# SymbolicML/DynamicExpressions.jl

Hardware: AMD Instinct MI355X
Metric: node-evals/sec (higher is better)
Workload: dtype f32

## Files before the change

dynamicexpressions.jl_amd/api.py:

```python
from __future__ import annotations

import ctypes as C
import os
from dataclasses import dataclass
from typing import Optional, Sequence, Tuple, Union

import numpy as np

from .node import Node, TAPE_DTYPE, count_constant_nodes, flatten_graph, flatten_population, max_feature, preserve_sharing
from .operators import OperatorEnum

_HERE = os.path.dirname(os.path.abspath(__file__))
LIB_PATH = os.environ.get("DE_HIP_LIB") or os.path.join(_HERE, "csrc", "libde_hip.so")

DE_F32, DE_F64, DE_F16, DE_CF32, DE_CF64 = 0, 1, 2, 3, 4
COMPLEX_DTYPES = (np.dtype(np.complex64), np.dtype(np.complex128))
GRAD_VARIABLE, GRAD_CONSTANT, GRAD_BOTH = 0, 1, 2
ABI_VERSION = 3
OPT_EARLY_EXIT, OPT_FUSE_DEG1, OPT_FUSE_DEG2, OPT_BUMPER_CHECKS, OPT_TURBO, OPT_FULL_EVAL, OPT_FORWARD_GRAD, OPT_REVERSE_GRAD = 1, 2, 4, 8, 16, 32, 64, 128

EXPORTS = [
    "de_abi_version", "de_opcode_table_version", "de_opcode_by_name", "de_opcode_name",
    "de_opcode_degree", "de_status_string", "de_ctx_create", "de_ctx_destroy", "de_ctx_set_stream",
    "de_ctx_synchronize", "de_ctx_declare_dataset", "de_ctx_stream", "de_last_error", "de_program_create", "de_program_create_cse",
    "de_program_set_consts", "de_program_update", "de_program_destroy", "de_program_n_trees", "de_program_n_nodes",
    "de_program_n_grad", "de_program_dump", "de_program_verify", "de_program_stream_hash", "de_host_pool_selftest", "de_lower_tape", "de_lower_tape_stage", "de_lower_tape_complex", "de_lower_tape_stage_complex", "de_lower_tape_grad", "de_eval", "de_eval_grad", "de_eval_diff", "de_eval_loss", "de_eval_loss_grad", "de_eval_loss_grad_by_class",
    "de_loss_spec_check", "de_eval_loss_ex", "de_eval_fit_stats", "de_eval_loss_gn", "de_gn_max_rows", "de_eval_loss_grad_ex", "de_eval_loss_grad_by_class_ex",
    "de_eval_pullback_dX", "de_eval_tree_array", "de_eval_plan", "de_prio_tiles_wanted", "de_program_last_live_trees", "de_dist_unique_id", "de_dist_init", "de_dist_destroy", "de_dist_shard_size", "de_dist_world_size",
    "de_dist_broadcast", "de_dist_gather_flags", "de_dist_last_error", "de_ctx_last_kernel_ms", "de_ctx_last_kernel_name",
    "de_ctx_device", "de_ctx_timing_ring", "de_ctx_timing_read", "de_dist_reorder_selftest", "de_eval_sum_certificate",
    "de_dist_set_timeout", "de_ctx_trim", "de_program_set_consts_device", "de_program_get_consts", "de_program_consts_device_path",
]


class DeviceError(RuntimeError):
    """The HIP library/GPU is unavailable or a de_* call failed.  Never swallowed."""


class UncertifiedFlag(DeviceError):
    """EvalContext(strict_flags=True): the device's element-wise validity flag of this tree is not PROVABLY the reference's
    `isfinite(sum(x))` flag (a finite array whose sum may overflow): the caller keeps the CPU path for it."""


class ParamArgs(C.Structure):
    _fields_ = [("params", C.c_void_p), ("ld_params", C.c_int64), ("n_classes", C.c_int64),
                ("classes", C.c_void_p), ("classes_is_i64", C.c_int32), ("class_base", C.c_int32)]


class LossSpec(C.Structure):
    _fields_ = [("kind", C.c_int32), ("reserved", C.c_int32), ("param", C.c_double)]


LOSS_KINDS = {"L2": 0, "L1": 1, "pullback": 2, "huber": 16, "logcosh": 17, "l1_eps": 18, "l2_eps": 19, "quantile": 20, "lp": 21,
              "logit_dist": 22, "logit_margin": 23, "l1_hinge": 24}


def loss_spec(loss: str, loss_param: float = 0.0, with_gradient: bool = True) -> LossSpec:
    if loss == "pullback" and not with_gradient:
        raise KeyError(loss)
    spec = LossSpec(LOSS_KINDS[loss], 0, float(loss_param))
    if library().de_loss_spec_check(C.byref(spec), int(with_gradient)) != 0:
        raise ValueError(f"loss {loss!r}: parameter {loss_param!r} is not finite or outside the kind's range (include/de_hip.h de_loss_kind_t)")
    return spec


class FitStats:

    def __init__(self, mean_p, m2_p, cov, W, mean_y, m2_y):
        self.mean_p, self.m2_p, self.cov = (np.array(v, dtype=np.float64) for v in (mean_p, m2_p, cov))
        if self.mean_p.ndim != 1 or self.m2_p.shape != self.mean_p.shape or self.cov.shape != self.mean_p.shape:
            raise ValueError("mean_p, m2_p and cov are one-dimensional arrays of one length (one entry per tree)")
        self.W, self.mean_y, self.m2_y = float(W), float(mean_y), float(m2_y)

    def __len__(self) -> int:
        return self.mean_p.shape[0]

    def _flat(self):
        return self.m2_p == 0.0

    @property
    def pearson_r(self):
        with np.errstate(divide="ignore", invalid="ignore"):
            r = self.cov / np.sqrt(self.m2_p * self.m2_y)
        return np.where(self._flat(), np.nan, r)
# ... 114 lines not shown
            pass
        lib = C.CDLL(LIB_PATH)
    except OSError as e:
        raise DeviceError(f"cannot load {LIB_PATH}: {e}") from e
    vp, i32, i64, u32 = C.c_void_p, C.c_int32, C.c_int64, C.c_uint32
    lib.de_abi_version.restype = C.c_int
    if lib.de_abi_version() != ABI_VERSION:
        raise DeviceError(f"{LIB_PATH} has ABI version {lib.de_abi_version()}, this module was written for {ABI_VERSION}: rebuild (csrc/build.sh)")
    lib.de_opcode_table_version.restype = C.c_int
    lib.de_opcode_by_name.argtypes = [C.c_char_p, C.c_int]
    lib.de_opcode_name.restype = C.c_char_p
    lib.de_opcode_name.argtypes = [C.c_int]
    lib.de_opcode_degree.argtypes = [C.c_int]
    lib.de_status_string.restype = C.c_char_p
    lib.de_status_string.argtypes = [C.c_int]
    lib.de_ctx_create.argtypes = [C.c_int, vp, C.POINTER(vp)]
    lib.de_ctx_destroy.argtypes = [vp]
    lib.de_ctx_set_stream.argtypes = [vp, vp]
    lib.de_ctx_synchronize.argtypes = [vp]
    lib.de_ctx_declare_dataset.argtypes = [vp, C.c_int, vp, i64, i64, i32]
    lib.de_ctx_stream.restype = vp
    lib.de_ctx_stream.argtypes = [vp]
    lib.de_last_error.restype = C.c_char_p
    lib.de_last_error.argtypes = [vp]
    lib.de_program_create.argtypes = [vp, C.c_int, vp, vp, i64, vp, vp, i32, i32, u32, C.POINTER(vp)]
    lib.de_program_create_cse.argtypes = [vp, C.c_int, vp, vp, vp, vp, i64, vp, vp, i32, i32, u32, C.POINTER(vp)]
    lib.de_program_set_consts.argtypes = [vp, vp]
    lib.de_program_set_consts_device.argtypes = [vp, vp]
    lib.de_program_get_consts.argtypes = [vp, vp]
    lib.de_program_consts_device_path.argtypes = [vp]
    lib.de_program_update.argtypes = [vp, vp, i64, vp, vp, vp, vp, vp, vp]
    lib.de_program_destroy.argtypes = [vp]
    lib.de_program_n_trees.restype = i64
    lib.de_program_n_trees.argtypes = [vp]
    lib.de_program_n_nodes.restype = i64
    lib.de_program_n_nodes.argtypes = [vp]
    lib.de_program_n_grad.restype = i64
    lib.de_program_n_grad.argtypes = [vp, i64, C.c_int]
    lib.de_program_verify.argtypes = [vp]
    lib.de_host_pool_selftest.restype = C.c_int64
    lib.de_host_pool_selftest.argtypes = [C.c_int64, C.POINTER(C.c_int32)]
    lib.de_program_stream_hash.restype = C.c_uint64
    lib.de_program_stream_hash.argtypes = [vp]
    lib.de_program_dump.restype = i64
    lib.de_program_dump.argtypes = [vp, i64, vp, i64, C.c_int]
    lib.de_lower_tape.restype = i64
    lib.de_lower_tape.argtypes = [C.c_int, vp, i64, vp, i64, i32, i32, u32, vp, i64, vp]
    lib.de_lower_tape_stage.restype = i64
    lib.de_lower_tape_stage.argtypes = [C.c_int, vp, i64, vp, i64, i32, i32, u32, C.c_int, vp, i64]
    for fn in (lib.de_lower_tape_complex, lib.de_lower_tape_stage_complex):
        fn.restype = i64
    lib.de_lower_tape_complex.argtypes = lib.de_lower_tape.argtypes
    lib.de_lower_tape_stage_complex.argtypes = lib.de_lower_tape_stage.argtypes
    lib.de_lower_tape_grad.restype = i64
    lib.de_lower_tape_grad.argtypes = [C.c_int, vp, i64, vp, i64, i32, i32, u32, C.c_int, C.c_int, vp, i64, vp]
    lib.de_eval.argtypes = [vp, vp, vp, i64, i64, C.POINTER(ParamArgs), vp, i64, vp]
    lib.de_eval_loss.argtypes = [vp, vp, vp, i64, i64, C.POINTER(ParamArgs), vp, vp, C.c_int32, vp, vp]
    lib.de_eval_loss_grad.argtypes = [vp, vp, vp, i64, i64, C.POINTER(ParamArgs), C.c_int, vp, vp, C.c_int32, vp, vp, vp, vp]
    lib.de_eval_loss_grad_by_class.argtypes = [vp, vp, vp, i64, i64, C.POINTER(ParamArgs), C.c_int, vp, vp, C.c_int32, vp, vp, vp, vp, vp, vp]
    lib.de_loss_spec_check.argtypes = [C.POINTER(LossSpec), C.c_int]
    lib.de_eval_loss_ex.argtypes = [vp, vp, vp, i64, i64, C.POINTER(ParamArgs), vp, vp, C.POINTER(LossSpec), vp, vp]
    lib.de_eval_fit_stats.argtypes = [vp, vp, vp, i64, i64, C.POINTER(ParamArgs), vp, vp, vp, vp, vp]
    lib.de_eval_loss_gn.argtypes = [vp, vp, vp, i64, i64, C.POINTER(ParamArgs), C.c_int, vp, vp, vp, vp, vp, vp, vp, vp]
    lib.de_gn_max_rows.argtypes = []
    lib.de_eval_loss_grad_ex.argtypes = [vp, vp, vp, i64, i64, C.POINTER(ParamArgs), C.c_int, vp, vp, C.POINTER(LossSpec), vp, vp, vp, vp]
    lib.de_eval_loss_grad_by_class_ex.argtypes = [vp, vp, vp, i64, i64, C.POINTER(ParamArgs), C.c_int, vp, vp, C.POINTER(LossSpec), vp, vp, vp, vp, vp, vp]
    lib.de_eval_grad.argtypes = [vp, vp, vp, i64, i64, C.POINTER(ParamArgs), C.c_int, vp, i64, vp, vp, vp]
    lib.de_eval_diff.argtypes = [vp, vp, vp, i64, i64, i32, vp, vp, i64, vp]
    lib.de_eval_pullback_dX.argtypes = [vp, vp, vp, i64, i64, C.POINTER(ParamArgs), vp, vp, vp, vp]
    lib.de_eval_tree_array.argtypes = [vp, C.c_int, vp, i64, vp, i64, vp, i32, i64, u32, vp, vp]
    lib.de_eval_plan.argtypes = [vp, i64, vp]
    lib.de_prio_tiles_wanted.argtypes = [i64, i32, i64]
    lib.de_program_last_live_trees.argtypes = [vp, C.POINTER(i64)]
    lib.de_dist_unique_id.argtypes = [vp]
    lib.de_dist_init.argtypes = [vp, C.c_int, C.c_int, vp, C.POINTER(vp)]
    lib.de_dist_destroy.argtypes = [vp]
    lib.de_dist_set_timeout.argtypes = [vp, i64]
    lib.de_dist_world_size.argtypes = [vp]
    lib.de_dist_shard_size.restype = i64
    lib.de_dist_shard_size.argtypes = [i64, C.c_int, C.c_int]
    lib.de_dist_broadcast.argtypes = [vp, vp, C.c_size_t, C.c_int]
    lib.de_dist_gather_flags.argtypes = [vp, vp, i64, vp]
    lib.de_dist_last_error.restype = C.c_char_p
    lib.de_dist_last_error.argtypes = [vp]
    lib.de_ctx_last_kernel_ms.argtypes = [vp, C.POINTER(C.c_float)]
    lib.de_ctx_last_kernel_name.restype = C.c_char_p
    lib.de_ctx_last_kernel_name.argtypes = [vp]
    lib.de_ctx_device.argtypes = [vp]
    lib.de_ctx_timing_ring.argtypes = [vp, i32]
    lib.de_ctx_timing_read.argtypes = [vp, vp, i32, C.POINTER(i32)]
    lib.de_dist_reorder_selftest.argtypes = [vp, vp, i64, C.c_int, vp, C.POINTER(C.c_float)]
    lib.de_eval_sum_certificate.argtypes = [vp, vp, vp, i64, i64, C.POINTER(ParamArgs), vp, vp, vp]
    _lib = lib
    return lib


def _dtype_code(dtype) -> int:
    dtype = np.dtype(dtype)
    if dtype == np.float32:
        return DE_F32
    if dtype == np.float64:
        return DE_F64
    if dtype == np.float16:
        return DE_F16
    if dtype == np.complex64:
        return DE_CF32
# ... 148 lines not shown
            X = X.to(tdt)
        F, N = X.shape
        if not (X.stride(0) == 1 and (N <= 1 or X.stride(1) >= F)) and X.numel() > 0:
            X = X.t().contiguous().t()
        ld = X.stride(1) if N > 1 else max(F, 1)
        return X.data_ptr(), F, N, ld, X, True
    X = np.asarray(X)
    if X.ndim == 1:
        X = X.reshape(-1, 1)
    Xf = np.asfortranarray(X, dtype=dtype)
    F, N = Xf.shape
    return Xf.ctypes.data, F, N, max(F, 1), Xf, False


def lower_tape(tape, consts, n_features: int, n_params: int = 0, options: int = 7, dtype=np.float32):
    lib = library()
    dtype = np.dtype(dtype)
    tape = np.ascontiguousarray(tape)
    consts = np.ascontiguousarray(consts, dtype=dtype)
    meta = np.zeros(4, dtype=np.int32)
    cp = consts.ctypes.data if consts.size else None
    lower = lib.de_lower_tape_complex if dtype in COMPLEX_DTYPES else lib.de_lower_tape
    n = lower(_dtype_code(dtype), tape.ctypes.data, len(tape), cp, consts.size, n_features,
              n_params, options, None, 0, meta.ctypes.data)
    if n < 0:
        code = int(-n)
        name = lib.de_status_string(code).decode()
        if code == 3:
            from .operators import UnsupportedOperatorError
            raise UnsupportedOperatorError(name)
        raise ValueError(name)
    w = np.zeros(max(int(n), 1), dtype=np.uint32)
    lower(_dtype_code(dtype), tape.ctypes.data, len(tape), cp, consts.size, n_features,
          n_params, options, w.ctypes.data, w.size, meta.ctypes.data)
    return w[:int(n)].reshape(-1, 4), dict(n_slots=int(meta[0]), host_ok_eval=bool(meta[1]),
                                           host_ok_grad=bool(meta[2]), uses_params=bool(meta[3]))


def lower_tape_stage(tape, consts, n_features: int, stage: int, n_params: int = 0, options: int = 7,
                     dtype=np.float32) -> np.ndarray:
    lib = library()
    dtype = np.dtype(dtype)
    tape = np.ascontiguousarray(tape)
    consts = np.ascontiguousarray(consts, dtype=dtype)
    cp = consts.ctypes.data if consts.size else None
    args = (_dtype_code(dtype), tape.ctypes.data, len(tape), cp, consts.size, n_features, n_params, options, stage)
    stage_fn = lib.de_lower_tape_stage_complex if dtype in COMPLEX_DTYPES else lib.de_lower_tape_stage
    n = stage_fn(*args, None, 0)
    if n < 0:
        raise ValueError(lib.de_status_string(int(-n)).decode())
    w = np.zeros(max(int(n), 1), dtype=np.uint32)
    stage_fn(*args, w.ctypes.data, w.size)
    return w[:int(n)].reshape(-1, 4)


def lower_tape_grad(tape, consts, n_features: int, mode: int, form: int, n_params: int = 0, options: int = 7, dtype=np.float32):
    lib = library()
    dtype = np.dtype(dtype)
    tape = np.ascontiguousarray(tape)
    consts = np.ascontiguousarray(consts, dtype=dtype)
    cp = consts.ctypes.data if consts.size else None
    meta = np.zeros(8, dtype=np.int32)
    args = (_dtype_code(dtype), tape.ctypes.data, len(tape), cp, consts.size, n_features, n_params, options, mode, form)
    n = lib.de_lower_tape_grad(*args, None, 0, meta.ctypes.data)
    if n < 0:
        raise ValueError(lib.de_status_string(int(-n)).decode())
    w = np.zeros(max(int(n), 1), dtype=np.uint32)
    lib.de_lower_tape_grad(*args, w.ctypes.data, w.size, meta.ctypes.data)
    return w[:int(n)].reshape(-1, 4), meta


def check_update_ids(indices, n_new: int, n_trees: int) -> np.ndarray:
    ids = np.asarray(list(indices) if not isinstance(indices, np.ndarray) else indices)
    if ids.ndim != 1:
        raise ValueError("update: indices must be one-dimensional")
    if len(ids) != n_new:
        raise ValueError(f"update: {len(ids)} indices for {n_new} trees")
    if len(ids) == 0:
        return np.zeros(0, dtype=np.int64)
    if ids.dtype.kind not in "iu":
        raise ValueError(f"update: indices must be integers, got {ids.dtype}")
    ids = np.ascontiguousarray(ids, dtype=np.int64)
    if ids.min() < 0 or ids.max() >= n_trees:
        raise ValueError(f"update: tree index outside [0, {n_trees})")
    if len(np.unique(ids)) != len(ids):
        raise ValueError("update: a tree index appears twice")
    return ids


class Population:

    def __init__(self, trees: Sequence[Node], operators: OperatorEnum, dtype=np.float32,
                 n_features: Optional[int] = None, n_params: int = 0,
                 eval_context: Optional[EvalContext] = None, ctx: Optional[Context] = None):
        self.ctx = ctx or default_context()
        self.dtype = np.dtype(dtype)
        self.operators = operators
        self.eval_context = eval_context or EvalContext()
        self.n_trees = len(trees)
        nodes, noff, consts, coff = flatten_population(trees, operators, self.dtype)
        if n_features is None:
            n_features = max((max_feature(t) for t in trees), default=0)
        self.n_features, self.n_params = int(n_features), int(n_params)
        self.n_consts = np.diff(coff).astype(np.int64)
        self._classes_checked = set()
        self._h = C.c_void_p()
# ... 131 lines not shown
        return library().de_program_consts_device_path(self._h) == 1

    def verify(self) -> None:
        self.ctx.check(library().de_program_verify(self._h))

    def stream_hash(self) -> int:
        return int(library().de_program_stream_hash(self._h))

    def _combine_rows(self, t: int, g, mode: int):
        if self._occ is None or self._occ[t] is None or mode == GRAD_VARIABLE:
            return g
        o = self._occ[t]
        lead = g.shape[0] - len(o)
        nu = int(o.max()) + 1
        if _is_torch(g):
            import torch
            out = torch.zeros((lead + nu,) + tuple(g.shape[1:]), dtype=g.dtype, device=g.device)
            out[:lead] = g[:lead]
            out.index_add_(0, torch.as_tensor(o + lead, device=g.device), g[lead:])
            return out
        out = np.zeros((lead + nu,) + g.shape[1:], dtype=g.dtype)
        out[:lead] = g[:lead]
        np.add.at(out, o + lead, g[lead:])
        return out

    def plan(self, N: int) -> dict:
        pl = np.zeros(3, dtype=np.int32)
        self.ctx.check(library().de_eval_plan(self._h, N, pl.ctypes.data))
        return dict(tile=int(pl[0]), n_chunks=int(pl[1]), trees_per_chunk=int(pl[2]))

    def last_live_trees(self) -> int:
        n = C.c_int64(-1)
        self.ctx.check(library().de_program_last_live_trees(self._h, C.byref(n)))
        return int(n.value)

    def n_grad(self, tree: int, mode: int) -> int:
        return int(library().de_program_n_grad(self._h, tree, mode))

    def _n_grad_all(self, mode: int) -> np.ndarray:
        cache = self.__dict__.setdefault("_ng_cache", {})
        if mode not in cache:
            lib = library()
            cache[mode] = np.array([lib.de_program_n_grad(self._h, t, mode) for t in range(self.n_trees)], dtype=np.int64)
        return cache[mode]

    def dump(self, tree: int) -> np.ndarray:
        lib = library()
        n = lib.de_program_dump(self._h, tree, None, 0, 0)
        w = np.zeros(max(int(n), 1), dtype=np.uint32)
        got = lib.de_program_dump(self._h, tree, w.ctypes.data, w.size, 0)
        return w[:int(got)].reshape(-1, 4)

    def meta(self, tree: int) -> dict:
        w = np.zeros(5, dtype=np.uint32)
        library().de_program_dump(self._h, tree, w.ctypes.data, 5, 1)
        return dict(n_slots=int(w[0]), host_ok_eval=bool(w[1]), host_ok_grad=bool(w[2]), uses_params=bool(w[3]), waves=int(w[4]))

    def _param_args(self, params, classes, class_base, N, keep):
        if self.n_params == 0 and params is None:
            return None
        if params is None or classes is None:
            raise ValueError("Incorrect call. You must pass the `classes::Vector` argument when calling `eval_tree_array`.")
        pa = ParamArgs()
        if _is_torch(params):
            import torch
            params = params.to(_torch_dtype(self.dtype))
            if params.stride(0) != 1 and params.numel() > 0:
                params = params.t().contiguous().t()
            P, ncls = params.shape
            pa.params, pa.ld_params = params.data_ptr(), (params.stride(1) if ncls > 1 else max(P, 1))
        else:
            params = np.asfortranarray(params, dtype=self.dtype)
            P, ncls = params.shape
            pa.params, pa.ld_params = params.ctypes.data, max(P, 1)
        if P != self.n_params:
            raise ValueError("parameter matrix has the wrong number of rows")
        if _is_torch(classes):
            import torch
            if classes.dtype not in (torch.int32, torch.int64):
                classes = classes.to(torch.int64)
            classes = classes.contiguous()
            n_c = classes.numel()
            key = (classes.data_ptr(), n_c, classes._version, ncls, class_base)
            if n_c and key not in self._classes_checked:
                mn, mx = int(classes.min().item()), int(classes.max().item())
                if mn < class_base or mx - class_base >= ncls:
                    raise ValueError(f"class ids must lie in [{class_base}, {class_base + ncls}): got [{mn}, {mx}] "
                                     "(maximum(classes) <= size(parameters, 2))")
                if len(self._classes_checked) > 64:
                    self._classes_checked.clear()
                self._classes_checked.add(key)
            pa.classes, pa.classes_is_i64 = classes.data_ptr(), int(classes.dtype == torch.int64)
        else:
            classes = np.ascontiguousarray(classes)
            if classes.dtype not in (np.int32, np.int64):
                classes = classes.astype(np.int64)
            n_c = classes.size
            if n_c:
                mn, mx = int(classes.min()), int(classes.max())
                if mn < class_base or mx - class_base >= ncls:
                    raise ValueError(f"class ids must lie in [{class_base}, {class_base + ncls}): got [{mn}, {mx}] "
                                     "(maximum(classes) <= size(parameters, 2))")
            pa.classes, pa.classes_is_i64 = classes.ctypes.data, int(classes.dtype == np.int64)
        if n_c != N:
            raise ValueError(f"length(classes) == size(X, 2) violated: {n_c} class ids for {N} samples")
        pa.n_classes, pa.class_base = ncls, class_base
        keep.extend([params, classes])
        return pa

# ... 580 lines not shown
```

dynamicexpressions.jl_amd/csrc/de_api_eval.cpp:

```cpp
#include "de_api_internal.h"

extern "C" {
int stage_in(de_ctx *c, DevBuf &buf, const void *user, size_t bytes, Staged *s) {
    s->dev = const_cast<void *>(user);
    s->staged = false;
    if (!user || bytes == 0 || is_device_ptr(user)) return DE_OK;
    HIP_TRY(c, buf.reserve(bytes));
    HIP_TRY(c, hipMemcpyAsync(buf.p, user, bytes, hipMemcpyHostToDevice, c->stream));
    s->dev = buf.p;
    s->staged = true;
    return DE_OK;
}
int stage_out(de_ctx *c, DevBuf &buf, void *user, size_t bytes, Staged *s) {
    s->dev = user;
    s->staged = false;
    if (!user || bytes == 0 || is_device_ptr(user)) return DE_OK;
    HIP_TRY(c, buf.reserve(bytes));
    s->dev = buf.p;
    s->staged = true;
    return DE_OK;
}

int check_param_args(de_ctx *c, const de_program *p, const de_param_args_t *pa, int64_t N) {
    if (!p->uses_params) return DE_OK;
// ... 236 lines not shown
    if (ok_dev) {
        sOk.dev = ok;
    } else {
        HIP_TRY(c, c->sOk.reserve((size_t)p->n_trees));
        sOk.dev = c->sOk.p;
        sOk.staged = true;
    }
    if (!p->d_ok_eval) HIP_TRY(c, hipMemcpyAsync(sOk.dev, p->host_ok_eval.data(), (size_t)p->n_trees, hipMemcpyHostToDevice, c->stream));
    if (p->uses_params) {
        rc = stage_in(c, c->sParams, pa->params, (size_t)pa->ld_params * (size_t)pa->n_classes * es, &sPar);
        if (rc) return rc;
        rc = stage_in(c, c->sClasses, pa->classes, (size_t)N * (pa->classes_is_i64 ? 8 : 4), &sCls);
        if (rc) return rc;
    }
    EvalArgs a;
    std::memset(&a, 0, sizeof a);
    a.code = p->d_code;
    a.code_off = p->d_code_off;
    a.n_trees = (int32_t)p->n_trees;
    a.n_slots = p->n_slots + (p->prows ? p->n_params : 0);
    a.prow_base = p->prows ? p->n_features + p->n_slots : 0;
    a.n_prows = p->prows ? p->n_params : 0;
    a.uses_params = p->uses_params;
    a.X = sX.dev;
    a.N = N;
    a.ldX = ldX;
    a.F = p->n_features;
    a.out = sOut.dev;
    a.ld_out = ld_out;
    a.ok = static_cast<uint8_t *>(sOk.dev);
    a.ok_init = p->d_ok_eval;
    if (p->uses_params) {
        a.params = sPar.dev;
        a.ld_params = pa->ld_params;
        a.n_classes = pa->n_classes;
        a.classes = sCls.dev;
        a.classes_is_i64 = pa->classes_is_i64;
        a.class_base = pa->class_base;
    }
    a.early_exit = (p->options & DE_OPT_EARLY_EXIT) != 0;
    a.skip_flagged = a.early_exit && !(p->options & DE_OPT_FULL_EVAL) && tree_skip_enabled();
    a.turbo = (p->options & DE_OPT_TURBO) != 0;
    a.threaded = p->threaded && !direct;
    a.direct = direct;
    a.loss = lr ? &la : nullptr;
    HIP_TRY(c, c->sPrio.reserve((size_t)3 * DE_PRIO_MAX_F * sizeof(unsigned long long)));
    a.prio_keys = c->sPrio.p;
    a.prio_keys_ready = !half && !cplx && !sX.staged && dataset_keys(c, p->dtype, X, N, ldX, p->n_features, &a.prio_keys);
    a.compact_code = p->d_compact_code;
    a.compact_ints = p->d_compact_ints;
    a.waves = p->waves;
    a.wave_slots = p->n_slots;
    a.var_stride = p->var_stride;
    if (cr) {
        a.code = p->d_cert_code;
        a.code_off = p->d_cert_off;
        a.threaded = false;
        a.cert_max = c->sCert.p;
        a.out = nullptr;
        a.prio_keys = nullptr;
        a.compact_code = nullptr;
        a.compact_ints = nullptr;
    }
    HIP_TRY(c, time_begin(c));
    a.compacted = &p->last_compacted;
    p->last_compacted = false;
    if (half || cplx) {
        a.threaded = false;
        a.prio_keys = nullptr;
        a.compact_code = nullptr;
        a.compact_ints = nullptr;
    }
    if (half) HIP_TRY(c, launch_eval_f16(a, c->stream, &c->last_kernel));
    else if (cplx) HIP_TRY(c, launch_eval_complex(p->io, a, p->d_ctab, c->stream, &c->last_kernel));
    else HIP_TRY(c, launch_eval(p->dtype, a, c->stream, &c->last_kernel));
    HIP_TRY(c, time_end(c));
    if (sLoss.staged) HIP_TRY(c, hipMemcpyAsync(lr->loss, sLoss.dev, (size_t)p->n_trees * es, hipMemcpyDeviceToHost, c->stream));
    if (sStats.staged) HIP_TRY(c, hipMemcpyAsync(lr->stats, sStats.dev, (size_t)p->n_trees * 3 * sizeof(double), hipMemcpyDeviceToHost, c->stream));
    if (sYstats.staged) HIP_TRY(c, hipMemcpyAsync(lr->ystats, sYstats.dev, 3 * sizeof(double), hipMemcpyDeviceToHost, c->stream));
    if (sOut.staged) {
        if (ld_out == N)
            HIP_TRY(c, hipMemcpyAsync(out, sOut.dev, (size_t)p->n_trees * (size_t)N * es, hipMemcpyDeviceToHost, c->stream));
        else
            for (int64_t t = 0; t < p->n_trees; t++)
                HIP_TRY(c, hipMemcpyAsync(static_cast<char *>(out) + (size_t)t * (size_t)ld_out * es,
                                          static_cast<char *>(sOut.dev) + (size_t)t * (size_t)ld_out * es,
                                          (size_t)N * es, hipMemcpyDeviceToHost, c->stream));
    }
    if (sOk.staged) HIP_TRY(c, hipMemcpyAsync(ok, sOk.dev, (size_t)p->n_trees, hipMemcpyDeviceToHost, c->stream));
    if (cr) {
        std::vector<unsigned char> mx((size_t)p->n_trees * ces);
        std::vector<uint8_t> okh((size_t)p->n_trees);
        HIP_TRY(c, hipMemcpyAsync(mx.data(), c->sCert.p, mx.size(), hipMemcpyDeviceToHost, c->stream));
        HIP_TRY(c, hipMemcpyAsync(okh.data(), sOk.dev, okh.size(), hipMemcpyDeviceToHost, c->stream));
        HIP_TRY(c, hipStreamSynchronize(c->stream));
        const double top = half ? 65504.0 : p->dtype == DE_F32 ? (double)std::numeric_limits<float>::max() : std::numeric_limits<double>::max();
        double margin = 1.001;
        if (half) {
            const double d = 1024.0 + std::ceil(std::log2(std::max(1.0, (double)N / 1024.0))) + 8.0;
            margin = std::exp(d * std::log1p(std::ldexp(1.0, -11)));
        }
        for (int64_t t = 0; t < p->n_trees; t++) {
            double m = p->dtype == DE_F32 ? (double)reinterpret_cast<float *>(mx.data())[t] : reinterpret_cast<double *>(mx.data())[t];
            m = std::max(m, p->cert_cmax[(size_t)t]);
            if (cr->max_abs) cr->max_abs[t] = m;
            cr->certified[t] = (!okh[(size_t)t] || m * (double)N * margin < top || !(m == m)) ? 1 : 0;
// ... 41 lines not shown
```

dynamicexpressions.jl_amd/csrc/de_api_internal.h:

```cpp
#ifndef DE_API_INTERNAL_H
#define DE_API_INTERNAL_H
#include <hip/hip_runtime.h>
#include <pthread.h>

#include <chrono>
#include <cmath>
#include <cstdarg>
#include <cstdio>
#include <cstring>
#include <condition_variable>
#include <functional>
#include <map>
#include <mutex>
#include <memory>
#include <new>
#include <string>
#include <algorithm>
#include <array>
#include <atomic>
#include <thread>
#include <vector>

#include "../../include/de_hip.h"
#include "de_kernels.h"
// ... 46 lines not shown
    DevBuf sPrioDs;
};

struct de_program {
    de_ctx *ctx = nullptr;
    int dtype = DE_F32;
    int io = DE_F32;
    std::vector<double> consts_im, ctab;
    void *d_ctab = nullptr;
    uint32_t options = 0;
    int32_t n_features = 0, n_params = 0;
    int64_t n_trees = 0, n_nodes = 0;
    int n_slots = 0;
    bool prows = false;
    bool uses_params = false;
    std::vector<Instr> code;
    std::vector<int32_t> code_off;
    std::vector<int64_t> const_off;
    std::vector<int32_t> const_instr;
    std::vector<uint8_t> const_checks;
    std::vector<int32_t> n_consts_tree;
    bool cse_generic = false;
    std::vector<uint8_t> host_ok_eval;
    std::vector<uint8_t> host_ok_grad;
    std::vector<double> consts;
    bool folded = false;
    std::vector<Instr> fcode;
    std::vector<int32_t> fcode_off;
    std::vector<int32_t> fconst_instr;
    struct Fold { int32_t tree, instr; bool tested_always; };
    std::vector<Fold> folds;
    std::vector<int64_t> aux_const_src;
    de_program *aux = nullptr;
    std::vector<uint8_t> fold_ok;
    std::vector<uint8_t> fold_host;
    std::vector<int32_t> kfold;
    std::vector<int64_t> kf_csrc;
    char *d_kf = nullptr;
    size_t kf_o_noff = 0, kf_o_coff = 0, kf_o_cvals = 0, kf_o_out = 0, kf_o_ok = 0, kf_bytes = 0;
    std::vector<de_tape_node_t> fold_nodes;
    std::vector<int64_t> fold_noff, fold_coff;
    std::vector<int32_t> aux_fold;
    std::vector<int64_t> aux_csrc;
    std::vector<BoundInstr> bcode;
    std::vector<BoundInstr> tcode;
    std::vector<BoundInstr> fbcode;
    std::vector<int32_t> tcode_off;
    std::vector<BoundInstr> ccode;
    std::vector<int32_t> ccode_off;
    int waves = 1;
    int waves_choice = 0;
    int64_t var_stride = 0;
    std::vector<BoundInstr> ccode_w;
    uint64_t end_handler = 0;
    uint64_t endv_handler[TOPX_ENDV_COUNT] = {0};
    bool threaded = false;
    bool direct = false;
    uint64_t handler_base = 0;
    std::vector<int32_t> bcode_off;
    BoundInstr *d_code = nullptr;
    int32_t *d_code_off = nullptr;
    bool eval_arena = false;
    BoundInstr *d_compact_code = nullptr;
    int32_t *d_compact_ints = nullptr;
    bool last_compacted = false;
    BoundInstr *d_cert_code = nullptr;
    int32_t *d_cert_off = nullptr;
    size_t cert_cap = 0;
    uint64_t consts_gen = 0;
    uint64_t cert_gen = ~0ull;
    std::vector<double> cert_cmax;
    BoundInstr *d_gcode = nullptr;
    int32_t *d_gcode_off = nullptr;
    std::vector<BoundInstr> gbcode;
    std::vector<int32_t> gbcode_off;
    bool gcode_stale = true;
    std::vector<BoundInstr> gtcode;
    std::vector<int32_t> gtcode_off;
    BoundInstr *d_gtcode = nullptr;
    int32_t *d_gtcode_off = nullptr;
    int32_t *d_gt_ids = nullptr;
    uint8_t *d_ok_eval = nullptr;
    uint8_t *d_ok_grad = nullptr;
    int32_t *d_ng = nullptr;
    int64_t *d_goff = nullptr;
    int tab_mode = -1;
    int64_t tab_N = -1;
    bool tab_ok_stale = true;
    std::vector<int32_t> bsite, tsite, gbsite, gtsite_of_gb;
    struct EvalSite { int32_t src, b, t, c; };
    struct GradSite { int32_t src, gb, gt, rt; };
    std::vector<EvalSite> eval_sites;
    std::vector<GradSite> grad_sites;
    uint64_t site_gen = 1, lists_gen = 0;
    std::vector<BoundInstr> rtcode;
    std::vector<int32_t> rtcode_off, rtcode_mid, rtsite_of_gb;
    BoundInstr *d_rtcode = nullptr;
    int32_t *d_rtcode_off = nullptr, *d_rtcode_mid = nullptr, *d_rt_ids = nullptr;
    int rt_mode = -1, rt_stage_cols = 0, rt_n_groups = 0;
    GradArgs::RevGroup rt_groups[8];
    bool rt_valid = false;
    uint64_t rt_handler_base = 0;
    uint32_t rt_param_off = 0;
    int gt_mode = -1;
    bool gt_valid = false, gt_wide = false;
    bool gt_share = false;
// ... 125 lines not shown
```

dynamicexpressions.jl_amd/csrc/de_api_program.cpp:

```cpp
#include "de_api_internal.h"
#include "de_const_patch.h"

template <typename T>
static bool host_fold_eval(const de_tape_node_t *nd, int64_t n, const double *consts, const int64_t *csrc, T *value, bool half = false) {
    T stack_small[32];
    std::vector<T> stack_big;
    T *st = stack_small;
    if (n > 32) { stack_big.resize((size_t)n); st = stack_big.data(); }
    int sp = 0;
    bool ok = true;
    for (int64_t i = 0; i < n; i++) {
        T v;
        if (nd[i].degree == 0) v = (T)consts[csrc[nd[i].arg]];
        else {
            const T b = st[--sp], a = st[--sp];
            switch (nd[i].op) {
            case DE_B_ADD: v = a + b; break;
            case DE_B_SUB: v = a - b; break;
            case DE_B_MUL: v = a * b; break;
            default: v = a / b; break;
            }
            if (half) v = (T)(_Float16)v;
        }
        ok = ok && std::isfinite(v);
// ... 70 lines not shown
};
static int64_t eval_rows(const de_program *p) { return (int64_t)p->n_features + p->n_slots + (p->prows ? p->n_params : 0); }
static bool same_binding(const de_program *p, const de_program *old) {
    return old->folded == p->folded && old->prows == p->prows && old->n_slots == p->n_slots && old->n_features == p->n_features &&
           old->n_params == p->n_params && old->options == p->options && old->dtype == p->dtype;
}
static void rebind(de_program *p, const Reuse *ru = nullptr) {
    const bool ee = (p->options & DE_OPT_EARLY_EXIT) != 0;
    p->prows = p->uses_params && p->n_params > 0 && p->n_params <= 16 && param_rows_enabled() &&
               ((size_t)p->n_features + (size_t)p->n_slots + (size_t)p->n_params) * 257 * 16 <= 150 * 1024;
    const int prb = p->prows ? p->n_features + p->n_slots : -1;
    const std::vector<Instr> &src = p->folded ? p->fcode : p->code;
    const std::vector<int32_t> &off = p->folded ? p->fcode_off : p->code_off;
    const int nf = p->n_features;
    const de_program *old = ru && ru->old && same_binding(p, ru->old) ? ru->old : nullptr;
    build_stream_by_trees<BoundInstr>(p->n_trees, &p->bcode, &p->bcode_off, [&](int64_t t, std::vector<BoundInstr> *out) {
        if (old && ru->src[(size_t)t] >= 0) {
            const size_t s = (size_t)ru->src[(size_t)t];
            out->insert(out->end(), old->bcode.begin() + old->bcode_off[s], old->bcode.begin() + old->bcode_off[s + 1]);
            return;
        }
        const int32_t i0 = off[(size_t)t], i1 = off[(size_t)t + 1];
        bind_tree(src.data() + i0, (size_t)(i1 - i0), ee, nf, out, prb);
    });
    match_const_sites(src, off, p->bcode, p->bcode_off, p->n_trees, [](const BoundInstr &b) { return bop_is_const_source(b.bop); }, &p->bsite);
    p->tsite.clear();
    p->site_gen++;
}

static void make_chained(de_program *p);
static int choose_waves(const de_program *p) {
    if (TBLK != 64 || (p->uses_params && !p->prows)) return 1;
    if (const char *e = getenv("DE_EVAL_WAVES")) { const int v = atoi(e); return (v == 2 || v == 4 || v == 8) ? v : 1; }
    const size_t rb = trow_bytes(p->dtype), lds_cu = 160u << 10, shared = (size_t)p->n_features + (p->prows ? (size_t)p->n_params : 0);
    auto resident = [&](int W) -> size_t {
        const size_t lds = (shared + (size_t)W * (size_t)p->n_slots) * rb + (size_t)W * 256;
        const size_t by_regs = W >= 4 ? 7 / ((size_t)W / 4) : 28 / (size_t)W;
        return lds > 150u * 1024 ? 0 : std::min<size_t>(lds_cu / lds, by_regs) * (size_t)W;
    };
    int best = 1;
    size_t have = resident(1);
    for (int W : {2, 4, 8}) {
        const size_t w = resident(W);
        if (have >= 20) break;
        if (w * 2 < have * 3) {
            if (W == 2 && have < 12) continue;
            break;
        }
        best = W;
        have = w;
    }
    return best;
}
static int make_threaded(de_ctx *c, de_program *p, const Reuse *ru = nullptr) {
    p->threaded = false;
    p->waves = 1;
    p->var_stride = 0;
    p->ccode_w.clear();
    dbg_lap(nullptr);
    p->direct = (size_t)eval_rows(p) * FLAT_ROW_BYTES > 150 * 1024;
    if (p->io == DE_F16) return DE_OK;
    if (is_complex_io(p->io)) {
        p->direct = (size_t)eval_rows(p) * complex_row_bytes(p->io) > 64 * 1024;
        return DE_OK;
    }
    if ((p->direct && ((size_t)eval_rows(p) + 3 * (size_t)p->n_slots) * trow_bytes(p->dtype) + 4 * 256 > 150 * 1024) || !eval_uses_threaded()) return DE_OK;
    if (eval_rows(p) > 4000) return DE_OK;
    uint64_t table[TOPX_TABLE];
    hipError_t st = eval_handler_table(p->dtype, (p->options & DE_OPT_TURBO) != 0, table);
    if (st != hipSuccess) return fail(c, DE_ERR_HIP, "handler table: %s", hipGetErrorString(st));
    dbg_lap("handler table");
    uint64_t base = table[0];
    for (int i = 0; i < (int)TOPX_TABLE; i++) base = std::min<uint64_t>(base, table[i]);
    for (int i = 0; i < (int)TOPX_TABLE; i++) {
        if (table[i] - base > 0xFFFFFFFFull) return DE_OK;
        if (p->dtype != DE_F32 && (table[i] >> 32) != (table[0] >> 32)) return DE_OK;
    }
    const bool hot_unary = !getenv("DE_NO_CONST_UNARY_HOT");
    const uint32_t row_bytes = (uint32_t)trow_bytes(p->dtype);
    const char *nf = getenv("DE_NO_FUSE");
    const bool fuse = !(nf && *nf == '1');
    if (p->waves_choice == 0) p->waves_choice = choose_waves(p);
    const int W = fuse ? p->waves_choice : 1;
    const int wave_prows = p->prows ? p->n_params : 0;
    const FuseRows rows0{(uint32_t)p->n_features, (uint32_t)(p->n_features + p->n_slots), 0, W > 1 ? wave_prows + (W - 1) * p->n_slots : 0};
    const de_program *old = ru && ru->old && ru->old->threaded && ru->old->waves_choice == p->waves_choice && same_binding(p, ru->old) ? ru->old : nullptr;
    build_stream_by_trees<BoundInstr>(p->n_trees, &p->fbcode, &p->tcode_off, [&](int64_t t, std::vector<BoundInstr> *out) {
        if (old && ru->src[(size_t)t] >= 0) {
            const size_t s = (size_t)ru->src[(size_t)t];
            out->insert(out->end(), old->fbcode.begin() + old->tcode_off[s], old->fbcode.begin() + old->tcode_off[s + 1]);
            return;
        }
        const int32_t b0 = p->bcode_off[(size_t)t], b1 = p->bcode_off[(size_t)t + 1];
        if (fuse) fuse_tree(p->bcode.data() + b0, (size_t)(b1 - b0), out, W > 1 && p->n_slots > 0 ? &rows0 : nullptr);
        else out->insert(out->end(), p->bcode.begin() + b0, p->bcode.begin() + b1);
    });
    dbg_lap("fuse_tree");
    p->tcode.resize(p->fbcode.size());
    auto threaded_words = [p, &table, base, hot_unary, row_bytes](const BoundInstr &b) {
        BoundInstr t = b;
        t.bop = (uint32_t)(table[b.bop] - base);
        if (hot_unary && (b.bop == BOP_GEN_ROW || b.bop == BOP_GEN_ACC)) {
            const int k = gun_index((int)(b.arg >> 24), DE_U_COS, DE_U_EXP, DE_U_SIN, DE_U_NEG, DE_U_SQUARE, DE_U_CUBE, DE_U_ABS, DE_U_LOG, DE_U_SAFE_LOG,
                                    DE_U_SQRT, DE_U_SAFE_SQRT, DE_U_TANH, DE_U_RELU);
            if (k >= 3) t.bop = (uint32_t)(table[TOPX_UN_BASE + (uint32_t)(k - 3) * 2 + (b.bop == BOP_GEN_ACC ? 1 : 0)] - base);
        }
        if (hot_unary && (b.bop == BOP_GEN_ROW || b.bop == BOP_GEN_CONST) && ((b.arg >> 24) == (uint32_t)DE_B_MAX || (b.arg >> 24) == (uint32_t)DE_B_MIN))
            t.bop = (uint32_t)(table[TOPX_BIN_BASE + ((b.arg >> 24) == (uint32_t)DE_B_MAX ? 0u : 2u) + (b.bop == BOP_GEN_CONST ? 1u : 0u)] - base);
        if (b.bop < BOP_COUNT && bop_is_const_source(b.bop)) {
            t.arg = b.arg & 0xFF000000u;
        } else if (b.bop == BOP_GEN_PARAM) {
// ... 32 lines not shown
        const bool ee = (p->options & DE_OPT_EARLY_EXIT) != 0, f32 = p->dtype == DE_F32;
        const std::vector<Instr> &src = p->folded ? p->fcode : p->code;
        const std::vector<int32_t> &off = p->folded ? p->fcode_off : p->code_off;
        const int prb = p->prows ? p->n_features + p->n_slots : -1, n_prows = wave_prows;
        const size_t n_rec = p->ccode.size();
        p->ccode_w.resize(n_rec * (size_t)(W - 1));
        std::atomic<bool> same{true};
        const bool wold = old && old->waves == W && old->var_stride != 0 && old->ccode_w.size() == old->ccode.size() * (size_t)(W - 1);
        for (int w = 1; w < W; w++) {
            BoundInstr *cw = p->ccode_w.data() + n_rec * (size_t)(w - 1);
            const int shift = n_prows + w * p->n_slots;
            const FuseRows rows_w{(uint32_t)(p->n_features + shift), (uint32_t)(p->n_features + shift + p->n_slots), shift, rows0.headroom};
            parallel_tree_ranges(p->n_trees, [&](int, int64_t tb, int64_t te) {
                std::vector<BoundInstr> b, f;
                const size_t r0 = (size_t)p->ccode_off[(size_t)tb] - 1, r1 = te < p->n_trees ? (size_t)p->ccode_off[(size_t)te] - 1 : n_rec;
                std::copy(p->ccode.begin() + (long)r0, p->ccode.begin() + (long)r1, cw + r0);
                for (int64_t t = tb; t < te; t++) {
                    if (wold && ru->src[(size_t)t] >= 0) {
                        const size_t s = (size_t)ru->src[(size_t)t], h = (size_t)p->ccode_off[(size_t)t], ho = (size_t)old->ccode_off[s];
                        const BoundInstr *ow = old->ccode_w.data() + old->ccode.size() * (size_t)(w - 1);
                        for (int32_t i = 0; i < p->tcode_off[(size_t)t + 1] - p->tcode_off[(size_t)t]; i++) {
                            BoundInstr &r = cw[h + (size_t)i];
                            const BoundInstr &o = ow[ho + (size_t)i];
                            r.bop = o.bop;
                            if (f32) r.arg = o.arg;
                            else { r.lo = o.lo; r.hi = o.hi; }
                        }
                        continue;
                    }
                    b.clear();
                    f.clear();
                    bind_tree(src.data() + off[(size_t)t], (size_t)(off[(size_t)t + 1] - off[(size_t)t]), ee, p->n_features, &b, prb, shift);
                    fuse_tree(b.data(), b.size(), &f, &rows_w);
                    const int32_t i0 = p->tcode_off[(size_t)t], i1 = p->tcode_off[(size_t)t + 1];
                    if ((int32_t)f.size() != i1 - i0) { same = false; return; }
                    const size_t h = (size_t)p->ccode_off[(size_t)t];
                    for (int32_t i = i0; i < i1; i++) {
                        if (f[(size_t)(i - i0)].bop != p->fbcode[(size_t)i].bop) { same = false; return; }
                        const BoundInstr tw = threaded_words(f[(size_t)(i - i0)]);
                        BoundInstr &r = cw[h + (size_t)(i - i0)];
                        r.bop = tw.arg;
                        if (f32) r.arg = tw.lo;
                        else { r.lo = tw.lo; r.hi = tw.hi; }
                    }
                }
            });
        }
        if (same) {
            p->waves = W;
            p->var_stride = (int64_t)(p->bcode.size() + (size_t)p->n_trees + 2);
        } else p->ccode_w.clear();
        dbg_lap("wave-group stream variants");
    } else if (W > 1 && fuse) p->waves = W;
    return DE_OK;
}

static void make_chained(de_program *p) {
    const bool f32 = p->dtype == DE_F32;
    p->ccode.assign(p->tcode.size() + (size_t)p->n_trees + 1, BoundInstr{0u, 0u, 0u, 0u});
    p->ccode_off.assign((size_t)p->n_trees + 1, 0);
    auto put = [&](BoundInstr &r, uint32_t la, uint32_t lo, uint32_t hi) {
        r.bop = la;
        if (f32) r.arg = lo;
        else { r.lo = lo; r.hi = hi; }
    };
    auto name_next = [&](BoundInstr &r, uint64_t handler) {
        if (f32) { r.lo = (uint32_t)handler; r.hi = (uint32_t)(handler >> 32); }
        else r.arg = (uint32_t)handler;
    };
    auto ev_of = [&](int64_t t) -> int {
        const int32_t i0 = p->tcode_off[(size_t)t], i1 = p->tcode_off[(size_t)t + 1];
        return i1 - i0 >= 2 ? topx_endv_of(p->fbcode[(size_t)i1 - 1].bop) : -1;
    };
    auto handler_of = [&](int32_t i, int32_t i1, int ev) -> uint64_t {
        return (i == i1 - 1 && ev >= 0) ? p->endv_handler[ev] : p->handler_base + p->tcode[(size_t)i].bop;
    };
    parallel_tree_ranges(p->n_trees, [&](int, int64_t tb, int64_t te) {
        for (int64_t t = tb; t < te; t++) {
            const int32_t i0 = p->tcode_off[(size_t)t], i1 = p->tcode_off[(size_t)t + 1];
            const size_t h = (size_t)i0 + (size_t)t + 1;
            p->ccode_off[(size_t)t] = (int32_t)h;
            const int ev = ev_of(t);
            for (int32_t i = i0; i < i1; i++) {
                const BoundInstr &s = p->tcode[(size_t)i];
                put(p->ccode[h + (size_t)(i - i0)], s.arg, s.lo, s.hi);
                if (i > i0) name_next(p->ccode[h + (size_t)(i - i0) - 1], handler_of(i, i1, ev));
            }
            put(p->ccode[h + (size_t)(i1 - i0)], (uint32_t)t, 0u, 0u);
            if (i1 > i0) name_next(p->ccode[h + (size_t)(i1 - i0) - 1], p->end_handler);
        }
    });
    for (int64_t t = 0; t < p->n_trees; t++) {
        const int32_t i0 = p->tcode_off[(size_t)t], i1 = p->tcode_off[(size_t)t + 1];
        const size_t h = (size_t)p->ccode_off[(size_t)t];
        const int ev = ev_of(t);
        if (i1 > i0) {
            const uint64_t first = handler_of(i0, i1, ev);
            name_next(p->ccode[h - 1], first);
            if (t > 0 && ev_of(t - 1) >= 0) name_next(p->ccode[h - 2], first);
        } else name_next(p->ccode[h - 1], p->end_handler);
        put(p->ccode[h - 1], t == 0 ? 0u : (uint32_t)(t - 1), (uint32_t)(i1 - i0) | (ev >= 0 ? DE_HDR_FUSED_END : 0u), 0u);
    }
    if (p->n_trees > 0) name_next(p->ccode.back(), p->end_handler);
    p->ccode_off[(size_t)p->n_trees] = (int32_t)p->ccode.size();
}
static inline void patch_chained_imm(de_program *p, int32_t c, uint32_t lo, uint32_t hi) {
    if (p->dtype == DE_F32) p->ccode[(size_t)c].arg = lo;
    else { p->ccode[(size_t)c].lo = lo; p->ccode[(size_t)c].hi = hi; }
    for (size_t w = 0; w * p->ccode.size() < p->ccode_w.size(); w++) {
        BoundInstr &r = p->ccode_w[w * p->ccode.size() + (size_t)c];
        if (p->dtype == DE_F32) r.arg = lo;
        else { r.lo = lo; r.hi = hi; }
    }
}
static hipError_t upload_wave_variants(de_program *p) {
    for (size_t w = 0; p->var_stride && w * p->ccode.size() < p->ccode_w.size(); w++) {
        const hipError_t st = hipMemcpy(p->d_code + (w + 1) * (size_t)p->var_stride, p->ccode_w.data() + w * p->ccode.size(),
                                        p->ccode.size() * sizeof(BoundInstr), hipMemcpyHostToDevice);
        if (st != hipSuccess) return st;
    }
    return hipSuccess;
}

static void recompute_host_ok(de_program *p) {
    const bool ee = (p->options & DE_OPT_EARLY_EXIT) != 0;
    parallel_for_trees(p->n_trees, [&](int64_t t) {
        bool ok_eval = true, ok_grad = true;
        for (int64_t k = p->const_off[t]; k < p->const_off[t + 1]; k++) {
            const bool fin = finite_in(p->dtype, p->consts[k]) && (p->consts_im.empty() || finite_in(p->dtype, p->consts_im[k]));
            ok_grad = ok_grad && fin;
            const uint8_t ch = p->const_checks[k];
            if (!fin && ((ch & CONST_CHECK_ALWAYS) || (ee && (ch & CONST_CHECK_EE)))) ok_eval = false;
        }
        p->host_ok_eval[t] = ok_eval;
        p->host_ok_grad[t] = ok_grad;
    }, 1024);
    for (size_t j = 0; j < p->folds.size() && j < p->fold_ok.size(); j++)
        if (!p->fold_ok[j] && (p->folds[j].tested_always || ee)) p->host_ok_eval[(size_t)p->folds[j].tree] = 0;
}

static int create_impl(de_ctx_t *ctx, int dtype, const de_tape_node_t *nodes, const int64_t *node_offsets,
                       int64_t n_trees, const void *consts, const int64_t *const_offsets, int32_t n_features,
                       int32_t n_params, uint32_t options, bool allow_fold, de_program_t **out_program,
                       const de_tape_node_t *cse_nodes = nullptr, const int64_t *cse_offsets = nullptr, const Reuse *reuse = nullptr,
                       bool keep_input = true);

static int upload_ok_eval(de_ctx *c, de_program *p) {
    p->tab_ok_stale = true;
    if (p->n_trees == 0) return DE_OK;
    if (!p->d_ok_eval) HIP_TRY(c, hipMalloc(reinterpret_cast<void **>(&p->d_ok_eval), (size_t)std::max<int64_t>(p->n_trees, 1)));
    HIP_TRY(c, hipStreamSynchronize(c->stream));
    HIP_TRY(c, hipMemcpy(p->d_ok_eval, p->host_ok_eval.data(), (size_t)p->n_trees, hipMemcpyHostToDevice));
    return DE_OK;
}

static int refresh_folds(de_ctx *c, de_program *p, bool aux_current = false) {
    if (!p->folded || p->folds.empty()) return DE_OK;
    const size_t es = p->dtype == DE_F32 ? 4 : 8;
    const size_t ies = dtype_bytes(p->io);
    const size_t nf = p->folds.size();
    p->fold_ok.assign(nf, 0);
    parallel_for_trees((int64_t)nf, [&](int64_t j) {
        if (p->fold_host[(size_t)j] != 1) return;
        const de_tape_node_t *nd = p->fold_nodes.data() + p->fold_noff[(size_t)j];
        const int64_t n = p->fold_noff[(size_t)j + 1] - p->fold_noff[(size_t)j];
        const int64_t *csrc = p->aux_const_src.data() + p->fold_coff[(size_t)j];
// ... 562 lines not shown
                        std::vector<int32_t> oaux(o->folds.size(), -1);
                        for (size_t a = 0; a < o->aux_fold.size(); a++) oaux[(size_t)o->aux_fold[a]] = (int32_t)a;
                        aru.old = o->aux;
                        aru.src.assign(p->aux_fold.size(), -1);
                        for (size_t a = 0; a < p->aux_fold.size(); a++) {
                            const size_t j = (size_t)p->aux_fold[a];
                            const int64_t t = p->folds[j].tree;
                            if (!reuse->reuse(t)) continue;
                            const size_t s = (size_t)reuse->src[(size_t)t];
                            aru.src[a] = oaux[(size_t)(reuse->fold0[s] + ((int64_t)j - fold0[(size_t)t]))];
                        }
                        aru.fold0.assign((size_t)o->aux->n_trees + 1, 0);
                        for (const de_program::Fold &f : o->aux->folds) aru.fold0[(size_t)f.tree + 1]++;
                        for (size_t q = 0; q < (size_t)o->aux->n_trees; q++) aru.fold0[q + 1] += aru.fold0[q];
                    }
                    int rc = create_impl(ctx, io, xnodes.data(), xnoff.data(), (int64_t)p->aux_fold.size(), ac.data(),
                                         xcoff.data(), n_features, 0, options, false, &p->aux, nullptr, nullptr, aru.old ? &aru : nullptr,
                                         false);
                    if (rc != DE_OK) return rc;
                    lap("aux program (create)");
                }
                int rc = refresh_folds(ctx, p.get(), true);
                if (rc != DE_OK) return rc;
                lap("folds (evaluate: host + kernel + aux)");
            } else if (any_cse) {
                p->folded = true;
            } else {
                p->fcode.clear();
                p->fcode_off.clear();
            }
        }
        if (!allow_fold) parallel_for_trees(n_trees, [&](int64_t t) { Lowered done; std::swap(done, low[(size_t)t]); });
        lap("release lowerings");
        if (cplx) fill_ctab_consts(p.get());
        recompute_host_ok(p.get());
        rebind(p.get(), reuse);
        lap("bind");
    } catch (const std::bad_alloc &) {
        return fail(ctx, DE_ERR_HIP, "out of host memory");
    }
    HIP_TRY(ctx, hipSetDevice(ctx->device));
    {
        int rc = DE_OK;
        try { rc = make_threaded(ctx, p.get(), reuse); } catch (const std::bad_alloc &) { rc = fail(ctx, DE_ERR_HIP, "out of host memory"); }
        if (rc != DE_OK) return rc;
    }
    lap("threaded + chained records");
    if (cplx) {
        const int rc = upload_ctab(ctx, p.get());
        if (rc != DE_OK) return rc;
    }
    const size_t cbytes = (p->bcode.size() + (size_t)p->n_trees + 2) * sizeof(BoundInstr);
    {
        const size_t nvar = p->threaded && p->var_stride ? (size_t)p->waves : 1;
        if (nvar > 1 && (size_t)p->var_stride * sizeof(BoundInstr) != cbytes) return fail(ctx, DE_ERR_HIP, "wave-group stream variants: stride and arena disagree");
        const size_t abytes = p->threaded ? 2 * nvar * cbytes : cbytes;
        auto al = [](size_t x) { return (x + 255) & ~(size_t)255; };
        const size_t off_bytes = p->bcode_off.size() * sizeof(int32_t);
        const size_t ints_bytes = p->threaded ? ((size_t)2 * (size_t)p->n_trees + 5) * sizeof(int32_t) : 0;
        const size_t o_off = al(abytes), o_ints = o_off + al(off_bytes), o_ok = o_ints + al(ints_bytes);
        const size_t total = o_ok + al((size_t)std::max<int64_t>(p->n_trees, 1));
        const hipError_t ast = prog_malloc(ctx, reinterpret_cast<void **>(&p->d_code), total);
        if (ast != hipSuccess) return fail(ctx, DE_ERR_HIP, "hipMalloc failed: %s", hipGetErrorString(ast));
        if (!in_one_window(p->d_code, abytes)) return fail(ctx, DE_ERR_HIP, "instruction stream straddles a 4 GiB boundary");
        char *base = reinterpret_cast<char *>(p->d_code);
        p->eval_arena = true;
        p->d_code_off = reinterpret_cast<int32_t *>(base + o_off);
        p->d_ok_eval = reinterpret_cast<uint8_t *>(base + o_ok);
        if (p->threaded) {
            p->d_compact_code = p->d_code + nvar * cbytes / sizeof(BoundInstr);
            p->d_compact_ints = reinterpret_cast<int32_t *>(base + o_ints);
        }
        lap("hipMalloc (arena)");
        const std::vector<BoundInstr> &stream = p->threaded ? p->ccode : p->bcode;
        const std::vector<int32_t> &offs = p->threaded ? p->ccode_off : p->bcode_off;
        hipError_t st = hipSuccess;
        if (total <= (size_t)(128u << 10)) {
            std::vector<unsigned char> img(total, 0);
            if (!stream.empty()) std::memcpy(img.data(), stream.data(), stream.size() * sizeof(BoundInstr));
            for (size_t w = 1; w < nvar; w++)
                std::memcpy(img.data() + w * cbytes, p->ccode_w.data() + (w - 1) * p->ccode.size(), p->ccode.size() * sizeof(BoundInstr));
            std::memcpy(img.data() + o_off, offs.data(), off_bytes);
            if (p->n_trees > 0) std::memcpy(img.data() + o_ok, p->host_ok_eval.data(), (size_t)p->n_trees);
            st = hipMemcpy(base, img.data(), total, hipMemcpyHostToDevice);
        } else {
            st = hipMemset(p->d_code, 0, nvar * cbytes);
            if (st == hipSuccess && !stream.empty()) st = hipMemcpy(p->d_code, stream.data(), stream.size() * sizeof(BoundInstr), hipMemcpyHostToDevice);
            if (st == hipSuccess) st = upload_wave_variants(p.get());
            if (st == hipSuccess) st = hipMemcpy(p->d_code_off, offs.data(), off_bytes, hipMemcpyHostToDevice);
            if (st == hipSuccess && p->n_trees > 0) st = hipMemcpy(p->d_ok_eval, p->host_ok_eval.data(), (size_t)p->n_trees, hipMemcpyHostToDevice);
        }
        if (st != hipSuccess) {
            prog_free(ctx, p->d_code);
            p->d_code = nullptr;
            return fail(ctx, DE_ERR_HIP, "program upload failed: %s", hipGetErrorString(st));
        }
    }
    lap("memset + upload (stream, offsets, flags)");
    if (getenv("DE_VERIFY") && *getenv("DE_VERIFY") == '1') {
        const int rc = de_program_verify(p.get());
        if (rc != DE_OK) return rc;
    }
    *out_program = p.release();
    return DE_OK;
}

static void refresh_site_lists(de_program *p) {
// ... 61 lines not shown
    HIP_TRY(ctx, hipSetDevice(ctx->device));
    {
        const int rc = upload_ok_eval(ctx, p);
        if (rc != DE_OK) return rc;
    }
    const auto t3 = now();
    if (cplx) return upload_ctab(ctx, p);
    const char *nopatch = getenv("DE_NO_CONST_PATCH");
    if (!(nopatch && *nopatch == '1') && p->threaded && !p->tsite.empty() && !p->bsite.empty()) {
        const std::vector<Instr> &src = p->folded ? p->fcode : p->code;
        const bool gpatch = p->d_gcode && !p->gcode_stale && !p->gbsite.empty();
        const bool tpatch = gpatch && p->gt_valid && !p->gtsite_of_gb.empty();
        const bool rpatch = gpatch && p->rt_valid && !p->rtsite_of_gb.empty();
        refresh_site_lists(p);
        try {
        parallel_tree_ranges((int64_t)p->eval_sites.size(), [&](int, int64_t sb, int64_t se) {
            for (size_t q = (size_t)sb; q < (size_t)se; q++) {
                const de_program::EvalSite &e = p->eval_sites[q];
                const uint32_t lo = src[(size_t)e.src].imm.u32[0], hi = src[(size_t)e.src].imm.u32[1];
                p->bcode[(size_t)e.b].lo = lo;
                p->bcode[(size_t)e.b].hi = hi;
                p->tcode[(size_t)e.t].lo = lo;
                p->tcode[(size_t)e.t].hi = hi;
                p->fbcode[(size_t)e.t].lo = lo;
                p->fbcode[(size_t)e.t].hi = hi;
                patch_chained_imm(p, e.c, lo, hi);
            }
        }, 4096);
        if (gpatch)
            parallel_tree_ranges((int64_t)p->grad_sites.size(), [&](int, int64_t sb, int64_t se) {
                for (size_t q = (size_t)sb; q < (size_t)se; q++) {
                    const de_program::GradSite &g = p->grad_sites[q];
                    const uint32_t lo = p->code[(size_t)g.src].imm.u32[0], hi = p->code[(size_t)g.src].imm.u32[1];
                    p->gbcode[(size_t)g.gb].lo = lo;
                    p->gbcode[(size_t)g.gb].hi = hi;
                    if (tpatch && g.gt >= 0) {
                        for (int64_t w = 0; w < (p->gt_share ? 4 : 1); w++) {
                            p->gtcode[(size_t)(g.gt + w * p->gt_stride)].lo = lo;
                            p->gtcode[(size_t)(g.gt + w * p->gt_stride)].hi = hi;
                        }
                    }
                    if (rpatch && g.rt >= 0) {
                        p->rtcode[(size_t)g.rt].lo = lo;
                        p->rtcode[(size_t)g.rt].hi = hi;
                    }
                }
            }, 4096);
        } catch (const std::bad_alloc &) { return fail(ctx, DE_ERR_HIP, "out of host memory"); }
        if (gpatch) {
            if (!tpatch) p->gt_valid = false;
            if (!rpatch) p->rt_valid = false;
        } else {
            p->gcode_stale = true;
        }
        const auto t4 = now();
        HIP_TRY(ctx, hipStreamSynchronize(ctx->stream));
        if (!p->ccode.empty())
            HIP_TRY(ctx, hipMemcpy(p->d_code, p->ccode.data(), p->ccode.size() * sizeof(BoundInstr), hipMemcpyHostToDevice));
        HIP_TRY(ctx, upload_wave_variants(p));
        if (gpatch) {
            if (!p->gbcode.empty())
                HIP_TRY(ctx, hipMemcpy(p->d_gcode, p->gbcode.data(), p->gbcode.size() * sizeof(BoundInstr), hipMemcpyHostToDevice));
            if (p->gt_valid && !p->gtcode.empty())
                HIP_TRY(ctx, hipMemcpy(p->d_gtcode, p->gtcode.data(), p->gtcode.size() * sizeof(BoundInstr), hipMemcpyHostToDevice));
            if (p->rt_valid && !p->rtcode.empty())
                HIP_TRY(ctx, hipMemcpy(p->d_rtcode, p->rtcode.data(), p->rtcode.size() * sizeof(BoundInstr), hipMemcpyHostToDevice));
        }
        if (timing)
            fprintf(stderr, "set_consts us: write %ld, refresh_folds %ld, flags %ld, patch %ld, upload %ld\n", us(t0, t1), us(t1, t2), us(t2, t3),
                    us(t3, t4), us(t4, now()));
        return DE_OK;
    }
    p->gcode_stale = true;
    try {
        rebind(p);
    } catch (const std::bad_alloc &) {
        return fail(ctx, DE_ERR_HIP, "out of host memory");
    }
    {
        int rc = DE_OK;
        try { rc = make_threaded(ctx, p); } catch (const std::bad_alloc &) { rc = fail(ctx, DE_ERR_HIP, "out of host memory"); }
        if (rc != DE_OK) return rc;
    }
    HIP_TRY(ctx, hipStreamSynchronize(ctx->stream));
    if (!p->bcode.empty())
        HIP_TRY(ctx, hipMemcpy(p->d_code, (p->threaded ? p->ccode : p->bcode).data(),
                               (p->threaded ? p->ccode : p->bcode).size() * sizeof(BoundInstr), hipMemcpyHostToDevice));
    if (p->threaded) HIP_TRY(ctx, upload_wave_variants(p));
    return DE_OK;
}

int consts_materialise(de_program *p) {
    if (!p || !p->consts_dev_ahead) return DE_OK;
    de_ctx *c = p->ctx;
    const size_t es = p->dtype == DE_F32 ? 4 : 8;
    try {
        std::vector<unsigned char> h(std::max<size_t>(p->consts.size(), 1) * es);
        HIP_TRY(c, hipSetDevice(c->device));
        HIP_TRY(c, hipMemcpyAsync(h.data(), p->d_cp_vals, p->consts.size() * es, hipMemcpyDeviceToHost, c->stream));
        HIP_TRY(c, hipStreamSynchronize(c->stream));
        p->consts_dev_ahead = false;
        const int rc = set_consts_nothrow(p, h.data());
        if (rc != DE_OK) p->consts_dev_ahead = true;
        return rc;
    } catch (const std::bad_alloc &) { return fail(c, DE_ERR_HIP, "out of host memory"); }
}
// ... 152 lines not shown
            const size_t nt = (size_t)p->n_trees;
            HIP_TRY(c, hipMalloc(reinterpret_cast<void **>(&p->d_ok_grad), nt));
            HIP_TRY(c, hipMalloc(reinterpret_cast<void **>(&p->d_ng), nt * sizeof(int32_t)));
            HIP_TRY(c, hipMalloc(reinterpret_cast<void **>(&p->d_goff), nt * sizeof(int64_t)));
            p->tab_mode = -1;
        }
        de_program::ConstPatchKey key;
        key.site_gen = p->site_gen;
        key.code = p->d_code;
        key.gcode = gpatch ? p->d_gcode : nullptr;
        key.gtcode = tpatch ? p->d_gtcode : nullptr;
        key.rtcode = rpatch ? p->d_rtcode : nullptr;
        key.ok_grad = p->d_ok_grad;
        key.gt_stride = tpatch ? p->gt_stride : 0;
        key.gt_variants = tpatch ? (p->gt_share ? 4 : 1) : 0;
        if (!p->d_cp || !(key == p->cp_key)) {
            const int rc = build_const_patch_tables(c, p, key, gpatch, tpatch, rpatch);
            if (rc < 0) return -rc;
            if (rc == 0) { p->cp_eligible = 0; device = false; }
        }
        if (device) {
            char *vals = p->d_cp_vals;
            uint8_t *fok = reinterpret_cast<uint8_t *>(vals + p->cp_o_fok);
            const int64_t *gidx = reinterpret_cast<const int64_t *>(p->d_cp + p->cp_o_gidx);
            if (!c->nested) HIP_TRY(c, time_begin(c));
            HIP_TRY(c, hipMemcpyAsync(vals, d_consts, nc * es, hipMemcpyDeviceToDevice, c->stream));
            HIP_TRY(c, launch_const_gather(p->dtype, vals, gidx, p->cp_nkc, p->d_kf ? p->d_kf + p->kf_o_cvals : nullptr, p->cp_nhc,
                                           p->d_cp + p->cp_o_hcvals, c->stream));
            if (p->cp_nk > 0)
                HIP_TRY(c, launch_fold(p->dtype, p->d_kf, reinterpret_cast<const int64_t *>(p->d_kf + p->kf_o_noff),
                                       reinterpret_cast<const int64_t *>(p->d_kf + p->kf_o_coff), p->d_kf + p->kf_o_cvals, p->cp_nk, vals + nc * es, fok,
                                       c->stream));
            if (p->cp_nh > 0)
                HIP_TRY(c, launch_fold(p->dtype, p->d_cp + p->cp_o_hnodes, reinterpret_cast<const int64_t *>(p->d_cp + p->cp_o_hnoff),
                                       reinterpret_cast<const int64_t *>(p->d_cp + p->cp_o_hcoff), p->d_cp + p->cp_o_hcvals, p->cp_nh,
                                       vals + (nc + (size_t)p->cp_nk) * es, fok + p->cp_nk, c->stream));
            HIP_TRY(c, launch_const_scatter(p->dtype, vals, reinterpret_cast<const uint64_t *>(p->d_cp + p->cp_o_addr),
                                            reinterpret_cast<const uint32_t *>(p->d_cp + p->cp_o_src), p->cp_n_sites, c->stream));
            HIP_TRY(c, launch_const_flags(p->dtype, vals, reinterpret_cast<const int64_t *>(p->d_cp + p->cp_o_coff),
                                          reinterpret_cast<const uint8_t *>(p->d_cp + p->cp_o_checks), reinterpret_cast<const int32_t *>(p->d_cp + p->cp_o_tfoff),
                                          reinterpret_cast<const uint32_t *>(p->d_cp + p->cp_o_tfold), fok, p->n_trees, (p->options & DE_OPT_EARLY_EXIT) != 0,
                                          p->d_ok_eval, p->d_ok_grad, c->stream));
            if (!c->nested) HIP_TRY(c, time_end(c));
            p->consts_gen++;
            if (gpatch) {
                if (!tpatch) p->gt_valid = false;
                if (!rpatch) p->rt_valid = false;
            } else {
                p->gcode_stale = true;
            }
            p->tab_ok_stale = false;
            p->consts_dev_ahead = true;
            p->consts_dev_path = true;
            return DE_OK;
        }
    }
    std::vector<unsigned char> h(nc * dtype_bytes(p->io));
    HIP_TRY(c, hipMemcpyAsync(h.data(), d_consts, h.size(), hipMemcpyDeviceToHost, c->stream));
    HIP_TRY(c, hipStreamSynchronize(c->stream));
    return de_program_set_consts(p, h.data());
}
int de_program_set_consts_device(de_program_t *p, const void *d_consts) {
    if (!p) return DE_ERR_INVALID_ARG;
    int rc = DE_OK;
    try { rc = set_consts_device_impl(p, d_consts); }
    catch (const std::bad_alloc &) { return fail(p->ctx, DE_ERR_HIP, "out of host memory"); }
    catch (const std::exception &e) { return fail(p->ctx, DE_ERR_HIP, "internal error: %s", e.what()); }
    catch (...) { return fail(p->ctx, DE_ERR_HIP, "internal error (unknown exception)"); }
    if (rc == DE_OK && p->consts_dev_ahead && getenv("DE_VERIFY") && *getenv("DE_VERIFY") == '1') return de_program_verify(p);
    return rc;
}
int de_program_consts_device_path(const de_program_t *p) { return p ? (p->consts_dev_path ? 1 : 0) : -1; }

static int get_consts_impl(de_program_t *p, void *out) {
    de_ctx *c = p->ctx;
    const size_t nc = p->consts.size();
    if (nc == 0) return DE_OK;
    if (!out) return fail(c, DE_ERR_INVALID_ARG, "out is null");
    HIP_TRY(c, hipSetDevice(c->device));
    const size_t ies = dtype_bytes(p->io);
    const bool dev = is_device_ptr(out);
    if (dev && p->consts_dev_ahead) {
        HIP_TRY(c, hipMemcpyAsync(out, p->d_cp_vals, nc * ies, hipMemcpyDeviceToDevice, c->stream));
        return DE_OK;
    }
    const int rc = consts_materialise(p);
    if (rc != DE_OK) return rc;
    std::vector<unsigned char> h;
    unsigned char *dst = static_cast<unsigned char *>(out);
    if (dev) { h.resize(nc * ies); dst = h.data(); }
    for (size_t k = 0; k < nc; k++) store_elem(p->io, dst, k, p->consts[k], p->consts_im.empty() ? 0.0 : p->consts_im[k]);
    if (dev) {
        HIP_TRY(c, hipMemcpyAsync(out, h.data(), h.size(), hipMemcpyHostToDevice, c->stream));
        HIP_TRY(c, hipStreamSynchronize(c->stream));
    }
    return DE_OK;
}
int de_program_get_consts(de_program_t *p, void *out) {
    if (!p) return DE_ERR_INVALID_ARG;
    DE_NOTHROW(p->ctx, get_consts_impl(p, out));
}

int de_program_destroy(de_program_t *p) {
    if (!p) return DE_OK;
    (void)hipSetDevice(p->ctx->device);
    dbg_lap(nullptr);
// ... 196 lines not shown
                                    fb.bop == BOP_GEN_PARAM || (fb.bop >= BOP_UN_BASE && fb.bop < BOP_UN_END && !((fb.bop - BOP_UN_BASE) & 2)) ||
                                    (fb.bop >= TOPX_UN_BASE && fb.bop < TOPX_BIN_BASE && ((fb.bop - TOPX_UN_BASE) & 1)) ||
                                    (fb.bop >= TOPX_BIN_BASE && ((fb.bop - TOPX_BIN_BASE) & 1));
                if (!no_row) {
                    const uint64_t off = r.bop & 0xFFFFFFu;
                    if (off % trow_bytes(p->dtype) != 0 || off + trow_bytes(p->dtype) > lds_bytes) return bad("LDS operand offset outside the launch's allocation", t, i - i0, r.bop);
                    const bool pushes = (fb.bop >= TOP_LOADROW_BASE && fb.bop < TOP_LOADCONST_PUSH && ((fb.bop - TOP_LOADROW_BASE) & 2)) ||
                                        (fb.bop >= TOP_UNROW_BASE && fb.bop < TOP_BINROWC_BASE && ((fb.bop - TOP_UNROW_BASE) & 2)) ||
                                        (fb.bop >= TOP_BIN2_BASE && fb.bop < TOP_COUNT && ((fb.bop - TOP_BIN2_BASE) & 1));
                    if (pushes) {
                        const int64_t prow = (int64_t)(off / trow_bytes(p->dtype)) + (int8_t)(r.bop >> 24);
                        if (prow < p->n_features || prow >= spill_end) return bad("push row of a superinstruction outside the spill slots", t, i - i0, r.bop);
                    }
                    if (fb.bop >= TOP_BIN2_BASE && fb.bop < TOP_COUNT && !(((fb.bop - TOP_BIN2_BASE) >> 2) & 1)) {
                        const int64_t second = (int64_t)off + (int32_t)(f32 ? r.arg : r.lo);
                        if (second < 0 || second % (int64_t)trow_bytes(p->dtype) != 0 || (uint64_t)second + trow_bytes(p->dtype) > lds_bytes) return bad("second operand row of a two-operand form", t, i - i0, (uint64_t)second);
                    }
                }
                if (fb.bop == BOP_GEN_PARAM && (f32 ? r.arg : r.lo) != (uint32_t)rows * (uint32_t)trow_bytes(p->dtype)) return bad("class-row offset of a parameter operand", t, i - i0, r.arg);
            }
        }
        if (p->waves > 1 && p->ccode_w.size() != (p->var_stride ? p->ccode.size() * (size_t)(p->waves - 1) : 0)) return bad("stream variants of the wave group", -1, p->waves, p->ccode_w.size());
        const uint64_t rb = trow_bytes(p->dtype);
        for (size_t w = 1; p->var_stride && w < (size_t)p->waves; w++) {
            const BoundInstr *cw = p->ccode_w.data() + (w - 1) * p->ccode.size();
            const int64_t shift = (p->prows ? p->n_params : 0) + (int64_t)w * p->n_slots, rows_all = rows + (int64_t)(p->waves - 1) * p->n_slots;
            auto moved = [&](int64_t row0, int64_t roww) { return roww == (row0 >= p->n_features && row0 < spill_end ? row0 + shift : row0) && roww < rows_all; };
            for (int64_t t = 0; t < p->n_trees; t++) {
                const int32_t i0 = p->tcode_off[(size_t)t], i1 = p->tcode_off[(size_t)t + 1], h = p->ccode_off[(size_t)t];
                for (int32_t i = i0 - 1; i <= i1; i++) {
                    const BoundInstr &r0 = p->ccode[(size_t)(h + (i - i0))], &r = cw[(size_t)(h + (i - i0))];
                    const bool same_next = f32 ? (r.lo == r0.lo && r.hi == r0.hi) : r.arg == r0.arg;
                    if (!same_next) return bad("stream variant names another handler", t, i - i0, w);
                    if (i < i0 || i == i1) { if (std::memcmp(&r, &r0, sizeof r)) return bad("stream variant: header / end record differs", t, i - i0, w); continue; }
                    const BoundInstr &fb = p->fbcode[(size_t)i];
                    if (fb.bop == BOP_GEN_PARAM) { if (std::memcmp(&r, &r0, sizeof r)) return bad("stream variant: a gathered-parameter record differs", t, i - i0, w); continue; }
                    const uint64_t off0 = r0.bop & 0xFFFFFFu, off = r.bop & 0xFFFFFFu;
                    if (off0 % rb != 0 || off % rb != 0) { if (off != off0) return bad("stream variant: operand word", t, i - i0, r.bop); }
                    else if (!moved((int64_t)(off0 / rb), (int64_t)(off / rb))) return bad("stream variant: operand row", t, i - i0, r.bop);
                    const bool pushes = (fb.bop >= TOP_LOADROW_BASE && fb.bop < TOP_LOADCONST_PUSH && ((fb.bop - TOP_LOADROW_BASE) & 2)) ||
                                        (fb.bop >= TOP_UNROW_BASE && fb.bop < TOP_BINROWC_BASE && ((fb.bop - TOP_UNROW_BASE) & 2)) ||
                                        (fb.bop >= TOP_BIN2_BASE && fb.bop < TOP_COUNT && ((fb.bop - TOP_BIN2_BASE) & 1));
                    if (pushes ? !moved((int64_t)(off0 / rb) + (int8_t)(r0.bop >> 24), (int64_t)(off / rb) + (int8_t)(r.bop >> 24)) : (r.bop >> 24) != (r0.bop >> 24))
                        return bad("stream variant: push row / aux byte", t, i - i0, r.bop);
                    const bool row_row = fb.bop >= TOP_BIN2_BASE && fb.bop < TOP_COUNT && !(((fb.bop - TOP_BIN2_BASE) >> 2) & 1);
                    if (row_row || fb.bop == BOP_TERN) {
                        const int64_t s0 = (int64_t)off0 + (int32_t)(f32 ? r0.arg : r0.lo), s1 = (int64_t)off + (int32_t)(f32 ? r.arg : r.lo);
                        if (s1 < 0 || s1 % (int64_t)rb != 0 || !moved(s0 / (int64_t)rb, s1 / (int64_t)rb)) return bad("stream variant: second operand row", t, i - i0, (uint64_t)s1);
                    } else if (f32 ? r.arg != r0.arg : (r.lo != r0.lo || r.hi != r0.hi))
                        return bad("stream variant: immediate differs", t, i - i0, w);
                }
            }
        }
    }
    return DE_OK;
}

int64_t de_program_dump(const de_program_t *p, int64_t tree, uint32_t *words, int64_t cap, int which) {
    if (!p || tree < 0 || tree >= p->n_trees) return -DE_ERR_INVALID_ARG;
    if (const int mrc = consts_materialise(const_cast<de_program_t *>(p))) return -mrc;
    if (which == 1) {
        if (cap < 4) return -DE_ERR_INVALID_ARG;
        words[0] = (uint32_t)p->n_slots;
        words[1] = p->host_ok_eval[(size_t)tree];
        words[2] = p->host_ok_grad[(size_t)tree];
        words[3] = p->uses_params;
        if (cap < 5) return 4;
        words[4] = (uint32_t)(p->threaded ? p->waves : 1);
        return 5;
    }
    if (which == 2) {
        const int32_t b0 = p->bcode_off[(size_t)tree], b1 = p->bcode_off[(size_t)tree + 1];
        const int64_t nb = (int64_t)(b1 - b0) * 4;
        if (!words || cap < nb) return nb;
        std::memcpy(words, p->bcode.data() + b0, (size_t)nb * 4);
        return nb;
    }
    if (which == 3) {
        if (!p->threaded) return 0;
        const int32_t b0 = p->tcode_off[(size_t)tree], b1 = p->tcode_off[(size_t)tree + 1];
        const int64_t nb = (int64_t)(b1 - b0) * 4;
        if (!words || cap < nb) return nb;
        std::memcpy(words, p->fbcode.data() + b0, (size_t)nb * 4);
        return nb;
    }
    const int32_t i0 = p->code_off[(size_t)tree], i1 = p->code_off[(size_t)tree + 1];
    const int64_t nw = (int64_t)(i1 - i0) * 4;
    if (!words || cap < nw) return nw;
    std::memcpy(words, p->code.data() + i0, (size_t)nw * 4);
    return nw;
}

static int64_t lower_tape_impl(int dtype, const de_tape_node_t *nodes, int64_t n_nodes, const void *consts, int64_t n_consts,
                               int32_t n_features, int32_t n_params, uint32_t options, uint32_t *words, int64_t cap, int32_t *meta);
static int64_t lower_tape_stage_impl(int dtype, const de_tape_node_t *nodes, int64_t n_nodes, const void *consts, int64_t n_consts,
                                     int32_t n_features, int32_t n_params, uint32_t options, int stage, uint32_t *words, int64_t cap);
int64_t de_lower_tape(int dtype, const de_tape_node_t *nodes, int64_t n_nodes, const void *consts,
                      int64_t n_consts, int32_t n_features, int32_t n_params, uint32_t options, uint32_t *words,
                      int64_t cap, int32_t *meta) {
    if (is_complex_io(dtype)) return -DE_ERR_INVALID_ARG;
    return lower_tape_impl(dtype, nodes, n_nodes, consts, n_consts, n_features, n_params, options, words, cap, meta);
}
int64_t de_lower_tape_complex(int dtype, const de_tape_node_t *nodes, int64_t n_nodes, const void *consts,
                              int64_t n_consts, int32_t n_features, int32_t n_params, uint32_t options, uint32_t *words,
                              int64_t cap, int32_t *meta) {
    if (!is_complex_io(dtype)) return -DE_ERR_INVALID_ARG;
    return lower_tape_impl(dtype, nodes, n_nodes, consts, n_consts, n_features, n_params, options, words, cap, meta);
}
int64_t de_lower_tape_stage(int dtype, const de_tape_node_t *nodes, int64_t n_nodes, const void *consts,
                            int64_t n_consts, int32_t n_features, int32_t n_params, uint32_t options, int stage,
                            uint32_t *words, int64_t cap) {
    if (is_complex_io(dtype)) return -DE_ERR_INVALID_ARG;
    return lower_tape_stage_impl(dtype, nodes, n_nodes, consts, n_consts, n_features, n_params, options, stage, words, cap);
}
int64_t de_lower_tape_stage_complex(int dtype, const de_tape_node_t *nodes, int64_t n_nodes, const void *consts,
                                    int64_t n_consts, int32_t n_features, int32_t n_params, uint32_t options, int stage,
                                    uint32_t *words, int64_t cap) {
    if (!is_complex_io(dtype)) return -DE_ERR_INVALID_ARG;
    return lower_tape_stage_impl(dtype, nodes, n_nodes, consts, n_consts, n_features, n_params, options, stage, words, cap);
}
static int64_t lower_tape_impl(int dtype, const de_tape_node_t *nodes, int64_t n_nodes, const void *consts, int64_t n_consts,
                               int32_t n_features, int32_t n_params, uint32_t options, uint32_t *words, int64_t cap, int32_t *meta) {
    if (!nodes || (dtype != DE_F32 && dtype != DE_F64 && dtype != DE_F16 && !is_complex_io(dtype)) || (n_consts > 0 && !consts)) return -DE_ERR_INVALID_ARG;
    const int io = dtype;
    const bool cplx = is_complex_io(io);
    if (dtype == DE_F16 || dtype == DE_CF32) dtype = DE_F32;
    else if (dtype == DE_CF64) dtype = DE_F64;
    if (cplx && complex_refused_op(nodes, n_nodes) >= 0) return -DE_ERR_UNSUPPORTED_OP;
    if (cplx && n_params > 0) return -DE_ERR_UNSUPPORTED;
    try {
        LowerOptions lo;
        lo.early_exit = (options & DE_OPT_EARLY_EXIT) != 0;
        lo.fuse1 = (options & DE_OPT_FUSE_DEG1) != 0;
        lo.fuse2 = (options & DE_OPT_FUSE_DEG2) != 0;
        lo.bumper = (options & DE_OPT_BUMPER_CHECKS) != 0;
        lo.n_features = n_features;
        lo.n_params = n_params;
        lo.dtype = dtype;
        for (int64_t i = 0; i < n_nodes; i++)
            if ((nodes[i].degree == 1 && nodes[i].op == DE_OP_SHARE) || (nodes[i].degree == 0 && nodes[i].op == DE_LEAF_SHARED)) lo.cse = true;
        TreeProgram tp;
        std::string why;
        int rc = lower_tree(nodes, n_nodes, n_consts, lo, &tp, &why);
        if (rc != DE_OK) return -rc;
        bool ok_eval = true, ok_grad = true;
        for (int64_t k = 0; k < n_consts; k++) {
            const double v = load_elem(io, consts, (size_t)k);
            if (tp.const_instr[(size_t)k] >= 0) {
                if (cplx) write_cidx(tp.code[(size_t)tp.const_instr[(size_t)k]], (size_t)k);
                else write_imm(tp.code[(size_t)tp.const_instr[(size_t)k]], dtype, v);
            }
            const bool fin = finite_in(dtype, v) && finite_in(dtype, load_elem_im(io, consts, (size_t)k));
            ok_grad = ok_grad && fin;
            const uint8_t ch = tp.const_checks[(size_t)k];
            if (!fin && ((ch & CONST_CHECK_ALWAYS) || (lo.early_exit && (ch & CONST_CHECK_EE)))) ok_eval = false;
        }
        if (meta) {
            meta[0] = tp.n_slots;
            meta[1] = ok_eval;
            meta[2] = ok_grad;
            meta[3] = tp.uses_params;
        }
        const int64_t nw = (int64_t)tp.code.size() * 4;
        if (!words || cap < nw) return nw;
        std::memcpy(words, tp.code.data(), (size_t)nw * 4);
        return nw;
    } catch (...) {
        return -DE_ERR_HIP;
    }
}

static int64_t lower_tape_stage_impl(int dtype, const de_tape_node_t *nodes, int64_t n_nodes, const void *consts, int64_t n_consts,
                                     int32_t n_features, int32_t n_params, uint32_t options, int stage, uint32_t *words, int64_t cap) {
    if (stage != 2 && stage != 3) return -DE_ERR_INVALID_ARG;
    std::vector<uint32_t> g;
    int64_t nw = lower_tape_impl(dtype, nodes, n_nodes, consts, n_consts, n_features, n_params, options, nullptr, 0, nullptr);
    if (nw < 0) return nw;
    try {
        g.resize((size_t)nw);
        nw = lower_tape_impl(dtype, nodes, n_nodes, consts, n_consts, n_features, n_params, options, g.data(), nw, nullptr);
        if (nw < 0) return nw;
        std::vector<BoundInstr> b, f;
        bind_tree(reinterpret_cast<const Instr *>(g.data()), (size_t)nw / 4, (options & DE_OPT_EARLY_EXIT) != 0, n_features, &b);
        if (stage == 3 && dtype != DE_F16 && !is_complex_io(dtype)) fuse_tree(b.data(), b.size(), &f);
        const std::vector<BoundInstr> &o = stage == 3 ? f : b;
        const int64_t n = (int64_t)o.size() * 4;
        if (!words || cap < n) return n;
        std::memcpy(words, o.data(), (size_t)n * 4);
        return n;
    } catch (...) {
        return -DE_ERR_HIP;
    }
}

}
```

dynamicexpressions.jl_amd/csrc/de_bind.cpp:

```cpp
#include "de_bind.h"

#include "../../include/de_opcodes.h"

namespace de {
namespace {

int hot_binary_index(uint32_t op) {
    switch (op) {
    case DE_B_ADD: return 0;
    case DE_B_SUB: return 1;
    case DOP_RSUB: return 2;
    case DE_B_MUL: return 3;
    case DE_B_DIV: return 4;
    case DOP_RDIV: return 5;
    default: return -1;
    }
}
int hot_unary_index(uint32_t op) {
    switch (op) {
    case DE_U_COS: return 0;
    case DE_U_EXP: return 1;
    case DE_U_SIN: return 2;
    default: return -1;
    }
}
BoundInstr mk(uint32_t bop, uint32_t arg, uint32_t lo = 0, uint32_t hi = 0) {
    BoundInstr b;
    b.bop = bop;
    b.arg = arg;
    b.lo = lo;
    b.hi = hi;
    return b;
}

}

void bind_tree(const Instr *code, size_t n, bool ee, int n_features, std::vector<BoundInstr> *out, int param_row_base, int slot_shift) {
    const uint32_t slot0 = (uint32_t)n_features + (uint32_t)slot_shift;
    for (size_t i = 0; i < n; i++) {
        const Instr &ins = code[i];
        const uint32_t hdr = ins.hdr;
        const uint32_t op = hdr & H_OP_MASK;
        uint32_t src = (hdr >> H_SRC_SHIFT) & H_SRC_MASK;
        uint32_t row = ins.feat & 0xFFFFu;
        if (src == SRC_PARAM && param_row_base >= 0) {
            src = SRC_ROW;
            row += (uint32_t)param_row_base;
        } else if (src == SRC_ROW && row >= (uint32_t)n_features) row += (uint32_t)slot_shift;
        const uint32_t lo = ins.imm.u32[0], hi = ins.imm.u32[1];
        if (hdr & H_PUSH) out->push_back(mk(BOP_PUSH, slot0 + ((hdr >> H_PUSH_SHIFT) & H_SLOT_MASK)));
        const bool check_b = ee && (hdr & H_CHECK_B);
        if (check_b && src == SRC_ROW) out->push_back(mk(BOP_CHECK_ROW, row));
        const bool check_out = op != DOP_LOAD && (hdr & (ee ? H_CHECK_OUT : H_CHECK_ALWAYS));
// ... 115 lines not shown
                f.arg = push_row;
                out->push_back(f);
                i = j + 1;
                continue;
            }
            if (m.bop >= BOP_UN_BASE && m.bop < BOP_UN_END && ((m.bop - BOP_UN_BASE) & 2) && (!chk || chk_row == row) &&
                (!push || delta_ok(row, push_row, fr))) {
                const uint32_t v = m.bop - BOP_UN_BASE;
                BoundInstr f = m;
                f.bop = top_unrow((int)(v >> 2), (v & 1) != 0, push, chk);
                f.arg = with_delta(row, push, push_row);
                out->push_back(f);
                i = j + 1;
                continue;
            }
            if (!push && chk && hot_bin_of(m, &hb) && !hb.cst && chk_row == row) {
                BoundInstr f = m;
                f.bop = top_binrowc(hb.k, hb.out);
                f.arg = row;
                out->push_back(f);
                i = j + 1;
                continue;
            }
        } else if (j < n) {
            const BoundInstr &m = b[j];
            HotBin hb;
            if (j + 1 < n && hot_bin_of(b[j + 1], &hb)) {
                const BoundInstr &nb = b[j + 1];
                if (m.bop == BOP_LOAD_ROW && (hb.cst || delta_ok(m.arg & 0xFFFFFFu, nb.arg & 0xFFFFFFu, fr))) {
                    const uint32_t row = m.arg & 0xFFFFFFu;
                    BoundInstr f = nb;
                    f.bop = top_bin2(hb.k, hb.cst, hb.out, false);
                    f.arg = row;
                    if (!hb.cst) { f.lo = (uint32_t)((int32_t)(nb.arg & 0xFFFFFFu) - (int32_t)row); f.hi = 0; }
                    out->push_back(f);
                    i = j + 2;
                    continue;
                }
                if (m.bop == BOP_LOAD_CONST && !hb.cst) {
                    BoundInstr f = m;
                    f.bop = top_bin2(mirrored(hb.k), true, hb.out, false);
                    f.arg = nb.arg & 0xFFFFFFu;
                    out->push_back(f);
                    i = j + 2;
                    continue;
                }
            }
        }
        out->push_back(b[i]);
        i++;
    }
}

}
```

dynamicexpressions.jl_amd/csrc/de_bind.h:

```cpp
#pragma once
#include <stdint.h>

#include <vector>

#include "de_program.h"

namespace de {

enum BoundOp : uint32_t {
    BOP_LOAD_ROW = 0,
    BOP_LOAD_CONST,
    BOP_PUSH,
    BOP_CHECK_ROW,
    BOP_CHECK_ACC,
    BOP_BIN_BASE,
    BOP_BIN_END = BOP_BIN_BASE + 24,
    BOP_UN_BASE = BOP_BIN_END,
    BOP_UN_END = BOP_UN_BASE + 12,
    BOP_GEN_ROW = BOP_UN_END,
    BOP_GEN_CONST,
    BOP_GEN_ACC,
    BOP_GEN_PARAM,
    BOP_TERN,
    BOP_INJ_ACC,
// ... 48 lines not shown
    if (bop == BOP_LOAD_CONST || bop == BOP_GEN_CONST) return true;
    return bop >= BOP_BIN_BASE && bop < BOP_BIN_END && ((bop - BOP_BIN_BASE) & 2);
}

enum ThreadedOp : uint32_t {
    TOP_LOADROW_BASE = BOP_COUNT,
    TOP_LOADCONST_PUSH = TOP_LOADROW_BASE + 4,
    TOP_UNROW_BASE = TOP_LOADCONST_PUSH + 1,
    TOP_BINROWC_BASE = TOP_UNROW_BASE + 24,
    TOP_BIN2_BASE = TOP_BINROWC_BASE + 12,
    TOP_COUNT = TOP_BIN2_BASE + 48
};
constexpr uint32_t top_loadrow(bool push, bool chk) { return TOP_LOADROW_BASE + 2 * push + chk; }
constexpr uint32_t top_unrow(int k, bool out, bool push, bool chk) { return TOP_UNROW_BASE + ((k * 2 + out) * 2 + push) * 2 + chk; }
constexpr uint32_t top_binrowc(int k, bool out) { return TOP_BINROWC_BASE + k * 2 + out; }
constexpr uint32_t top_bin2(int k, bool cst, bool out, bool push) { return TOP_BIN2_BASE + ((k * 2 + cst) * 2 + out) * 2 + push; }

constexpr int GOP_MAX = 760;
constexpr int GBIN_K = 8;
constexpr int GUN_K = 13;
static_assert(ROP_GEN_BASE - ROP_UN_BASE == 4 * GUN_K, "RevOp layout and GUN_K disagree");
static_assert(ROP_UN_BASE - ROP_BIN_BASE == 6 * GBIN_K, "RevOp layout and GBIN_K disagree");
constexpr int gun_index(int op, int u_cos, int u_exp, int u_sin, int u_neg, int u_square, int u_cube, int u_abs, int u_log,
                        int u_safe_log, int u_sqrt, int u_safe_sqrt, int u_tanh, int u_relu) {
    return op == u_cos ? 0 : op == u_exp ? 1 : op == u_sin ? 2 : op == u_neg ? 3 : op == u_square ? 4 : op == u_cube ? 5 : op == u_abs ? 6 :
           op == u_log ? 7 : op == u_safe_log ? 8 : op == u_sqrt ? 9 : op == u_safe_sqrt ? 10 : op == u_tanh ? 11 : op == u_relu ? 12 : -1;
}
enum { GSRC_LEAF = 0, GSRC_SLOT = 1, GSRC_CONST = 2, GSRC_ACC = 3 };
constexpr uint32_t gop_ns(int GC) { return (uint32_t)GC + 2; }
constexpr uint32_t gop_load(int GC, int src, int sv) {
    return src == GSRC_LEAF ? (uint32_t)sv : (src == GSRC_SLOT ? gop_ns(GC) : gop_ns(GC) + 1 + (uint32_t)sv);
}
constexpr uint32_t gop_push(int GC) { return 2 * gop_ns(GC) + 1; }
constexpr uint32_t gop_check_acc(int GC) { return gop_push(GC) + 1; }
constexpr uint32_t gop_bin_base(int GC) { return gop_check_acc(GC) + 1; }
constexpr uint32_t gop_bin(int GC, int k, int src, int sv, bool chk) {
    return gop_bin_base(GC) + (uint32_t)(k * 2 + chk) * (2 * gop_ns(GC) + 1) + gop_load(GC, src, sv);
}
constexpr uint32_t gop_un_base(int GC) { return gop_bin_base(GC) + 2 * GBIN_K * (2 * gop_ns(GC) + 1); }
constexpr uint32_t gop_un(int GC, int k, int src, int sv, bool chk) {
    return gop_un_base(GC) + (uint32_t)(k * 2 + chk) * (gop_ns(GC) + 2) +
           (src == GSRC_LEAF ? (uint32_t)sv : (src == GSRC_SLOT ? gop_ns(GC) : gop_ns(GC) + 1));
}
constexpr uint32_t gop_gen_base(int GC) { return gop_un_base(GC) + 2 * GUN_K * (gop_ns(GC) + 2); }
constexpr uint32_t gop_gen(int GC, int src) { return gop_gen_base(GC) + (uint32_t)src; }
constexpr uint32_t gop_param(int GC) { return gop_gen_base(GC) + 4; }
constexpr uint32_t gop_tern(int GC) { return gop_gen_base(GC) + 5; }
constexpr uint32_t gop_pushload(int GC, int src, int sv) { return gop_gen_base(GC) + 6 + (src == GSRC_LEAF ? 0u : gop_ns(GC)) + (uint32_t)sv; }
constexpr uint32_t gop_count(int GC) { return gop_gen_base(GC) + 6 + 2 * gop_ns(GC); }
static_assert(gop_count(8) <= GOP_MAX, "GOP_MAX too small");

constexpr uint32_t TOPX_UN_BASE = TOP_COUNT;
constexpr uint32_t TOPX_BIN_BASE = TOPX_UN_BASE + 2 * (GUN_K - 3);
constexpr uint32_t TOPX_COUNT = TOPX_BIN_BASE + 4;
constexpr uint32_t TOPX_END = TOPX_COUNT;
constexpr uint32_t TOPX_ENDV_BASE = TOPX_END + 1;
constexpr uint32_t TOPX_ENDV_COUNT = 15;
constexpr uint32_t TOPX_AUX_BASE = TOPX_ENDV_BASE + TOPX_ENDV_COUNT;
constexpr uint32_t TOPX_TABLE = TOPX_AUX_BASE + 2;
constexpr uint32_t DE_HDR_FUSED_END = 0x80000000u;
constexpr int topx_endv_of(uint32_t id) {
    return (id >= BOP_BIN_BASE && id < BOP_BIN_END && ((id - BOP_BIN_BASE) & 1)) ? (int)(((id - BOP_BIN_BASE) >> 2) * 2 + (((id - BOP_BIN_BASE) >> 1) & 1))
         : (id >= BOP_UN_BASE && id < BOP_UN_END && ((id - BOP_UN_BASE) & 3) == 1) ? 12 + (int)((id - BOP_UN_BASE) >> 2) : -1;
}

inline bool top_reads_acc(uint32_t top, int generic_degree) {
    if (top == BOP_LOAD_ROW || top == BOP_LOAD_CONST || top == BOP_CHECK_ROW || top == BOP_INJ_ROW) return false;
    if (top == BOP_GEN_ROW || top == BOP_GEN_CONST || top == BOP_GEN_PARAM) return generic_degree != 1 && generic_degree != 0;
    if (top >= BOP_UN_BASE && top < BOP_UN_END) return ((top - BOP_UN_BASE) & 2u) == 0;
    if (top < BOP_COUNT) return true;
    if (top >= TOP_LOADROW_BASE && top < TOP_LOADCONST_PUSH) return ((top - TOP_LOADROW_BASE) & 2u) != 0;
    if (top == TOP_LOADCONST_PUSH) return true;
    if (top >= TOP_UNROW_BASE && top < TOP_BINROWC_BASE) return ((top - TOP_UNROW_BASE) & 2u) != 0;
    if (top >= TOP_BINROWC_BASE && top < TOP_BIN2_BASE) return true;
    if (top >= TOP_BIN2_BASE && top < TOP_COUNT) return ((top - TOP_BIN2_BASE) & 1u) != 0;
    if (top >= TOPX_UN_BASE && top < TOPX_BIN_BASE) return ((top - TOPX_UN_BASE) & 1u) != 0;
    return true;
}

inline bool bop_reads_row(uint32_t bop) {
    if (bop == BOP_LOAD_ROW || bop == BOP_GEN_ROW) return true;
    if (bop >= BOP_BIN_BASE && bop < BOP_BIN_END) return ((bop - BOP_BIN_BASE) & 2u) == 0;
    return bop >= BOP_UN_BASE && bop < BOP_UN_END && ((bop - BOP_UN_BASE) & 2u) != 0;
}

inline bool top_carries_const(uint32_t top) {
    if (top < BOP_COUNT) return bop_is_const_source(top);
    if (top == TOP_LOADCONST_PUSH) return true;
    if (top >= TOP_BIN2_BASE && top < TOP_COUNT) return (((top - TOP_BIN2_BASE) >> 2) & 1u) != 0;
    return false;
}

struct FuseRows { uint32_t slot_lo, slot_hi; int32_t shift, headroom; };
void fuse_tree(const BoundInstr *b, size_t n, std::vector<BoundInstr> *out, const FuseRows *rows = nullptr);
bool top_is_const_source(uint32_t top);

void bind_tree(const Instr *code, size_t n, bool early_exit, int n_features, std::vector<BoundInstr> *out, int param_row_base = -1, int slot_shift = 0);

}
```

dynamicexpressions.jl_amd/csrc/de_kernels.h:

```cpp
#pragma once
#include <hip/hip_runtime.h>
#include <stdint.h>

#include "../../include/de_hip.h"
#include "de_bind.h"
#include "de_program.h"

namespace de {

constexpr int BLOCK = 256;
#ifndef DE_TBLK
#define DE_TBLK 64
#endif
constexpr int TBLK = DE_TBLK, TWAVES = DE_TBLK / 64;
#ifndef DE_TG
#define DE_TG 1
#endif
constexpr int TG_F32 = DE_TG, TG_F64 = 1;
constexpr int tg_planes(int dtype) { return dtype == DE_F32 ? TG_F32 : TG_F64; }
constexpr int ttile_samples(int dtype) { return TBLK * tg_planes(dtype) * (dtype == DE_F32 ? 4 : 2); }
constexpr size_t trow_bytes(int dtype) { return (size_t)(TBLK * tg_planes(dtype) + 1) * 16; }
constexpr int flat_tile_samples(int io) { return io == DE_F32 || io == DE_F16 ? 1024 : (io == DE_CF64 ? 256 : 512); }
constexpr size_t FLAT_ROW_BYTES = 257 * 16;

struct LossArgs {
    const void *y;
    const void *w;
    int32_t kind;
    double param;
    void *partial;
    void *seg_sum;
    void *loss;
    double *stats;
    double *ystats;
};
constexpr int32_t FIT_STATS_KIND = 25;
constexpr int FIT_STATS_VALUES = 4;

struct EvalArgs {
    const BoundInstr *code;
    const int32_t *code_off;
    int32_t n_trees;
    int32_t n_slots;
    int32_t prow_base, n_prows;
    bool uses_params;
    const void *X;
    int64_t N, ldX;
    int32_t F;
    void *out;
    int64_t ld_out;
    uint8_t *ok;
    const uint8_t *ok_init;
    const void *params;
    int64_t ld_params;
    int64_t n_classes;
    const void *classes;
    int32_t classes_is_i64, class_base;
    bool early_exit;
    bool skip_flagged;
    bool turbo;
    bool threaded;
    bool direct;
    const LossArgs *loss;
    void *prio_keys;
    bool prio_keys_ready;
    void *compact_code;
    int32_t *compact_ints;
    bool *compacted;
    int32_t waves, wave_slots;
    int64_t var_stride;
    void *cert_max;
};
constexpr int DE_PRIO_MAX_F = 8;
constexpr int DE_PRIO_UNIT = 64;
#define DE_FOLD_STACK 16
hipError_t launch_fold(int dtype, const void *nodes, const int64_t *noff, const int64_t *coff, const void *cvals, int64_t n_folds, void *out,
                       uint8_t *ok, hipStream_t stream);
hipError_t launch_dist_pack(uint8_t *send, const uint8_t *ok_local_dev, int64_t mine, int64_t per, hipStream_t stream);
hipError_t launch_dist_unpack(uint8_t *ok_global_dev, const uint8_t *recv, int64_t per, int32_t world, int64_t n_trees, hipStream_t stream);
hipError_t launch_tile_extremes(int dtype, const void *X, int64_t N, int64_t ldX, int F, void *keys, hipStream_t stream, const uint8_t *ok_init = nullptr,
                                uint8_t *ok = nullptr, int32_t n_ok = 0);
bool prio_tiles_wanted(int64_t N, int F, int64_t n_trees);

constexpr int DE_GN_MAX_ROWS = 8;
struct GradArgs {
    EvalArgs e;
    const BoundInstr *generic_code;
    int32_t mode;
    int32_t P;
    void *grad;
    const int64_t *grad_off;
    const int32_t *n_grad;
    int32_t max_grad;
    int32_t diff_direction;
    const LossArgs *loss;
    const int64_t *col_off;
    int64_t n_cols;
    void *dloss;
    const int64_t *dloss_off;
    bool gn;
    void *jtj;
    const int64_t *jtj_off;
    const BoundInstr *threaded_code;
    const BoundInstr *rev_code;
    const int32_t *rev_code_off, *rev_code_mid;
    const int32_t *rev_ids;
    int32_t rev_n_groups;
    const int64_t *rev_tile_range;
    int64_t rev_n_tiles;
    struct RevGroup { int32_t first, n, rows; } rev_groups[8];
    int32_t rev_stage_cols;
    uint64_t rev_handler_base;
    uint32_t rev_param_off;
    bool prio_ready;
    bool gt_share;
    int64_t gt_var_stride;
    int32_t n_buckets;
    struct Bucket {
        int32_t GC, VS;
        int32_t windows, max_grad;
        int32_t n_slots;
        const int32_t *ids;
        int32_t n;
// ... 52 lines not shown
```

dynamicexpressions.jl_amd/csrc/de_kernels.hip:

```cpp
#include <hip/hip_runtime.h>
#include <algorithm>
#include <map>
#include <mutex>
#include <type_traits>
#include <vector>

#include <cstdlib>
#include <cstring>

#include "de_bind.h"
#include "de_device_ops.h"
#include "de_kernels.h"
#include "de_loss_kinds.h"
#include "de_plan.h"
#include "de_real_vec.h"

namespace de {


template <typename T> struct KArgs {
    const BoundInstr *code;
    const int32_t *code_off;
    const T *X;
    T *out;
    uint8_t *ok;
    const T *params;
    const void *classes;
    int64_t N, ldX, ld_out, ld_params, n_tiles, n_classes;
    int32_t F, n_trees, trees_per_chunk, n_chunks, n_slots, xstride;
    int32_t prow_base, n_prows;
    const unsigned long long *prio;
    uint32_t n_prio_blocks, n_prio, prio_shift;
    int32_t classes_is_i64, class_base, vec_store;
    const T *y;
    const T *w;
    T *partial;
    int32_t loss_kind;
    uint32_t cls_row_off;
    int32_t x_vec;
    int32_t skip_flagged;
    uint32_t f_magic;
    const int32_t *live_idx;
    const int32_t *ctrl;
    int32_t map_group;
    void *cert_max;
    int32_t tail_split;
    int64_t var_stride;
    uint32_t list_off;
    T loss_param;
    const double *fit_ystats;
};


__device__ __forceinline__ TileMap map_block_grouped(uint32_t bid, int32_t n_chunks, int64_t n_tiles, uint32_t grp) {
    TileMap m;
    const uint32_t xcd = bid & 7u, idx = bid >> 3;
    const uint32_t per = grp * (uint32_t)n_chunks;
    const uint32_t g = idx / per, r = idx - g * per;
    m.chunk = (int32_t)(r / grp);
    m.tile = ((int64_t)g * grp + (r - (uint32_t)m.chunk * grp)) * 8 + xcd;
    m.valid = m.tile < n_tiles;
    return m;
}

template <typename T>
__device__ __forceinline__ void stage_param_rows(const KArgs<T> &a, T *__restrict__ rows, int row_elems, int64_t base, int tile, int tid, int blk) {
    const int64_t last = a.N - 1;
    for (int j = tid; j < tile; j += blk) {
        int64_t jj = base + j;
        jj = jj < last ? jj : last;
        const int64_t cl = clamp_class((a.classes_is_i64 ? reinterpret_cast<const int64_t *>(a.classes)[jj]
                                                         : (int64_t) reinterpret_cast<const int32_t *>(a.classes)[jj]) - a.class_base, a.n_classes);
        const T *__restrict__ col = a.params + a.ld_params * cl;
        for (int p = 0; p < a.n_prows; p++) rows[(size_t)(a.prow_base + p) * row_elems + j] = col[p];
    }
}

template <typename T> struct PoisonOf { typedef T type; };
template <> struct PoisonOf<float> { typedef float type __attribute__((ext_vector_type(2))); };
template <typename T> struct TG { static constexpr int G = sizeof(T) == 4 ? DE_TG : 1; };
static_assert(DE_TG == TG_F32, "de_kernels.h TG_F32 and DE_TG disagree");
#define DE_PLANE_BYTES (DE_TBLK * 16u)
#if DE_TG == 1
#define FOR_PLANES if (constexpr int g = 0; true)
#else
#define FOR_PLANES DE_UNROLL for (int g = 0; g < TG<T>::G; g++)
#endif
template <typename T> struct __attribute__((packed, aligned(8))) HState {
    typename VecOf<T>::type acc[TG<T>::G];
    typename PoisonOf<T>::type poison;
};
template <typename T> struct __attribute__((packed, aligned(8))) BState {
    typename VecOf<T>::type acc;
    typename PoisonOf<T>::type poison;
};
template <typename T> struct HLoss { typename VecOf<T>::type v[2]; };
template <typename T> struct ImmBits;
template <> struct ImmBits<float> { typedef uint32_t type; };
template <> struct ImmBits<double> { typedef uint64_t type; };
template <typename T> __device__ __forceinline__ T imm_from(typename ImmBits<T>::type b);
template <> __device__ __forceinline__ float imm_from<float>(uint32_t b) { return __uint_as_float(b); }
template <> __device__ __forceinline__ double imm_from<double>(uint64_t b) { return __longlong_as_double((long long)b); }
#define HARGS BState<T> st, uint32_t la, typename ImmBits<T>::type imm
#define LDSP(T, addr) (reinterpret_cast<__attribute__((address_space(3))) typename VecOf<T>::type *>((uintptr_t)(addr)))
// ... 525 lines not shown
    typedef VecOf<float>::type V;
    if constexpr (K == 1 || TB || G == 1) {
        DE_UNROLL for (int g = 0; g < G; g++) out[g] = un_finish<K, TB>(x[g], p[g]);
    } else {
        constexpr bool SIN = K == 2;
        DeF2 sa[G], sb[G];
        DE_UNROLL for (int g = 0; g < G; g++) {
            sa[g] = trig_poly_f32x2<SIN, TB>(DeF2{x[g][0], x[g][1]}, p[g].ta);
            sb[g] = trig_poly_f32x2<SIN, TB>(DeF2{x[g][2], x[g][3]}, p[g].tb);
        }
#ifndef DE_TRIG_NO_EXTREMUM_FIX
        DeF2 ra[G], rb[G];
        bool near = false;
        DE_UNROLL for (int g = 0; g < G; g++) {
            ra[g] = trig_reduced_f32x2<SIN, TB>(DeF2{x[g][0], x[g][1]}, p[g].ta);
            rb[g] = trig_reduced_f32x2<SIN, TB>(DeF2{x[g][2], x[g][3]}, p[g].tb);
            const DeF2 za = ra[g] * ra[g], zb = rb[g] * rb[g];
            near |= __builtin_fmaxf(__builtin_fmaxf(__builtin_fmaxf(za[0], za[1]), zb[0]), zb[1]) > (0x1.3bd3ccp+1f - 8.0e-4f);
        }
        if (__builtin_expect(__ballot(near) != 0ull, 0)) {
            asm volatile("" ::: "memory");
            DE_UNROLL for (int g = 0; g < G; g++) {
                sa[g][0] = trig_extremum_fix(ra[g][0], sa[g][0]); sa[g][1] = trig_extremum_fix(ra[g][1], sa[g][1]);
                sb[g][0] = trig_extremum_fix(rb[g][0], sb[g][0]); sb[g][1] = trig_extremum_fix(rb[g][1], sb[g][1]);
            }
        }
#endif
        DE_UNROLL for (int g = 0; g < G; g++) {
            const DeF2 ya = fast_trig_sign_f32x2(sa[g], p[g].ka), yb = fast_trig_sign_f32x2(sb[g], p[g].kb);
            out[g] = V{ya[0], ya[1], yb[0], yb[1]};
        }
    }
}
#if DE_NO_LOSS
#define HFAST_LOSS_C
#elif DE_TG == 1
#define HFAST_LOSS_C VecOf<float>::type ly0, VecOf<float>::type lw0,
#else
#define HFAST_LOSS_C VecOf<float>::type ly0, VecOf<float>::type ly1, VecOf<float>::type lw0, VecOf<float>::type lw1,
#endif
#define HFAST_ARGS HState<float> st, HFAST_LOSS_C uint32_t lds0, ConstU4Ptr code, uint64_t outp, uint32_t la, uint32_t w1, uint64_t w23, uint64_t okp, uint64_t ldo, \
                   uint64_t skip, uint32_t left, uint32_t flags
#define HFAST_PASS st, HL_PASS_C lds0, code, outp, la, w1, w23, okp, ldo, skip, left, flags
#define HFAST_NEXT(W) [[clang::musttail]] return arg_next<float>(w1, w23)(st, HL_PASS_C lds0, code_at(code, 1), outp, (W).x, (W).y, ((uint64_t)(W).w << 32) | (W).z, okp, ldo, skip, left, flags)
#define HFAST_END_TAIL()                                                                                                    \
    {                                                                                                                       \
        const U32x4 wn = code[1];                                                                                           \
        const uint32_t tree = *reinterpret_cast<const DE_CONSTANT uint32_t *>(code);       \
        const GPtr row = reinterpret_cast<GPtr>(outp + (uint64_t)tree * (uint64_t)(uint32_t)ldo);                                               \
        FOR_PLANES DE_OUT_STORE(VecOf<float>::type, row + lds0 + (uint32_t)g * DE_PLANE_BYTES, st.acc[g]); \
        HTREE_END_TAIL(wn, code_at(code, 2), code);                                                                                     \
    }
#define PLANE_ADDR(A, g) ((A) + (uint32_t)(g) * DE_PLANE_BYTES)
template <int K, int VAR, bool TB> __device__ __noinline__ HState<float> h_un_fast(HFAST_ARGS) {
    typedef float T;
    constexpr int G = TG<T>::G;
    const U32x4 w = *code;
    VecOf<float>::type x[G];
    FOR_PLANES x[g] = (VAR & 2) ? *LDSP(T, PLANE_ADDR(lds0 + la, g)) : st.acc[g];
    UnPre p[G];
    bool slow = false;
    FOR_PLANES slow |= un_pretest<K, TB>(x[g], p[g]);
    if (__builtin_expect(__ballot(slow) != 0ull, 0)) [[clang::musttail]] return h_chain<T, &b_un<T, K, VAR, TB>>(HFAST_PASS);
#if DE_TG == 1
    FOR_PLANES {
        st.acc[g] = un_finish<K, TB>(x[g], p[g]);
        if constexpr (VAR & 1) hpoison<T>(st.poison, st.acc[g]);
    }
#else
    un_finish_planes<K, TB, G>(st.acc, x, p);
    if constexpr (VAR & 1) FOR_PLANES hpoison<T>(st.poison, st.acc[g]);
#endif
    HFAST_NEXT(w);
}
template <int K, bool TB> __device__ __noinline__ HState<float> h_un_end_fast(HFAST_ARGS) {
    typedef float T;
    constexpr int G = TG<T>::G;
    UnPre p[G];
    bool slow = false;
    FOR_PLANES slow |= un_pretest<K, TB>(st.acc[g], p[g]);
    if (__builtin_expect((int32_t)flags < 0, 0)) [[clang::musttail]] return h_chain_end<T, &b_un<T, K, 1, TB>>(HFAST_PASS);
    if (__builtin_expect(wave_any(slow), 0)) [[clang::musttail]] return h_chain_end<T, &b_un<T, K, 1, TB>>(HFAST_PASS);
#if DE_TG == 1
    FOR_PLANES {
        st.acc[g] = un_finish<K, TB>(st.acc[g], p[g]);
        hpoison<T>(st.poison, st.acc[g]);
    }
#else
    un_finish_planes<K, TB, G>(st.acc, st.acc, p);
    FOR_PLANES hpoison<T>(st.poison, st.acc[g]);
#endif
    HFAST_END_TAIL()
}
template <int K, bool OUT, bool PUSH, bool CHK, bool TB> __device__ __noinline__ HState<float> h_unrow_fast(HFAST_ARGS) {
    typedef float T;
    constexpr int G = TG<T>::G;
    const U32x4 w = *code;
    const uint32_t a = lds0 + la;
    VecOf<float>::type x[G];
    FOR_PLANES {
        if constexpr (PUSH) *LDSP(T, push_addr<T>(PLANE_ADDR(a, g))) = st.acc[g];
        x[g] = *LDSP(T, PUSH ? row_a(PLANE_ADDR(a, g)) : PLANE_ADDR(a, g));
    }
    UnPre p[G];
    bool slow = false;
    FOR_PLANES slow |= un_pretest<K, TB>(x[g], p[g]);
    if (__builtin_expect(__ballot(slow) != 0ull, 0)) [[clang::musttail]] return h_chain<T, &b_unrow_f<T, K, OUT, PUSH, CHK, TB>>(HFAST_PASS);
#if DE_TG == 1
    FOR_PLANES {
        if constexpr (CHK) hpoison<T>(st.poison, x[g]);
        st.acc[g] = un_finish<K, TB>(x[g], p[g]);
        if constexpr (OUT) hpoison<T>(st.poison, st.acc[g]);
    }
#else
    if constexpr (CHK) FOR_PLANES hpoison<T>(st.poison, x[g]);
    un_finish_planes<K, TB, G>(st.acc, x, p);
    if constexpr (OUT) FOR_PLANES hpoison<T>(st.poison, st.acc[g]);
#endif
    HFAST_NEXT(w);
}
template <int K, int VAR> __device__ __noinline__ HState<float> h_div_fast(HFAST_ARGS) {
    typedef float T;
    typedef VecOf<float>::type V;
    constexpr int G = TG<T>::G;
    const U32x4 w = *code;
    if constexpr (VAR & 2) {
        bool unsafe = false;
        FOR_PLANES unsafe |= !div_samples_safe(st.acc[g]);
        if (__builtin_expect(!div_const_in_range(w1), 0)) [[clang::musttail]] return h_chain<T, &b_bin<T, K, VAR, false>>(HFAST_PASS);
        if (__builtin_expect(wave_any(unsafe), 0)) [[clang::musttail]] return h_chain<T, &b_bin<T, K, VAR, false>>(HFAST_PASS);
        FOR_PLANES st.acc[g] = div_const<K>(st.acc[g], w1);
    } else {
        V num[G], den[G];
        bool unsafe = false;
        FOR_PLANES {
            const V b = *LDSP(T, PLANE_ADDR(lds0 + la, g));
            num[g] = K == 4 ? st.acc[g] : b;
            den[g] = K == 4 ? b : st.acc[g];
            unsafe |= !div_operands_safe(num[g], den[g]);
        }
        if (__builtin_expect(__ballot(unsafe) != 0ull, 0)) [[clang::musttail]] return h_chain<T, &b_bin<T, K, VAR, false>>(HFAST_PASS);
        FOR_PLANES st.acc[g] = div_safe(num[g], den[g]);
    }
    if constexpr (VAR & 1) FOR_PLANES hpoison<T>(st.poison, st.acc[g]);
    HFAST_NEXT(w);
}
template <int K, bool CST> __device__ __noinline__ HState<float> h_div_end_fast(HFAST_ARGS) {
    typedef float T;
    typedef VecOf<float>::type V;
    constexpr int G = TG<T>::G;
    if constexpr (CST) {
        bool unsafe = false;
        FOR_PLANES unsafe |= !div_samples_safe(st.acc[g]);
        if (__builtin_expect(((int32_t)flags < 0) | !div_const_in_range(w1), 0)) [[clang::musttail]] return h_chain_end<T, &b_bin<T, K, 3, false>>(HFAST_PASS);
        if (__builtin_expect(wave_any(unsafe), 0)) [[clang::musttail]] return h_chain_end<T, &b_bin<T, K, 3, false>>(HFAST_PASS);
        FOR_PLANES st.acc[g] = div_const<K>(st.acc[g], w1);
    } else {
        V num[G], den[G];
        bool unsafe = false;
        FOR_PLANES {
            const V b = *LDSP(T, PLANE_ADDR(lds0 + la, g));
            num[g] = K == 4 ? st.acc[g] : b;
            den[g] = K == 4 ? b : st.acc[g];
            unsafe |= !div_operands_safe(num[g], den[g]);
        }
        if (__builtin_expect((int32_t)flags < 0, 0)) [[clang::musttail]] return h_chain_end<T, &b_bin<T, K, 1, false>>(HFAST_PASS);
        if (__builtin_expect(wave_any(unsafe), 0)) [[clang::musttail]] return h_chain_end<T, &b_bin<T, K, 1, false>>(HFAST_PASS);
        FOR_PLANES st.acc[g] = div_safe(num[g], den[g]);
    }
    FOR_PLANES hpoison<T>(st.poison, st.acc[g]);
    HFAST_END_TAIL()
}
template <int K, bool OUT> __device__ __noinline__ HState<float> h_divrowc_fast(HFAST_ARGS) {
    typedef float T;
    typedef VecOf<float>::type V;
    constexpr int G = TG<T>::G;
    const U32x4 w = *code;
    V b[G], num[G], den[G];
    bool unsafe = false;
    FOR_PLANES {
        b[g] = *LDSP(T, PLANE_ADDR(lds0 + la, g));
        num[g] = K == 4 ? st.acc[g] : b[g];
        den[g] = K == 4 ? b[g] : st.acc[g];
        unsafe |= !div_operands_safe(num[g], den[g]);
    }
    if (__builtin_expect(__ballot(unsafe) != 0ull, 0)) [[clang::musttail]] return h_chain<T, &b_binrowc<T, K, OUT, false>>(HFAST_PASS);
    FOR_PLANES {
        hpoison<T>(st.poison, b[g]);
        st.acc[g] = div_safe(num[g], den[g]);
        if constexpr (OUT) hpoison<T>(st.poison, st.acc[g]);
    }
    HFAST_NEXT(w);
}
template <int K, bool CST, bool OUT, bool PUSH> __device__ __noinline__ HState<float> h_div2_fast(HFAST_ARGS) {
// ... 122 lines not shown
#define TBK(K) (TB && (K) >= 4)
#define HB(K) t[BOP_BIN_BASE + 4 * K + 0] = (uint64_t)&h_chain<T, &b_bin<T, K, 0, TBK(K)>>; t[BOP_BIN_BASE + 4 * K + 1] = (uint64_t)&h_chain<T, &b_bin<T, K, 1, TBK(K)>>; \
              t[BOP_BIN_BASE + 4 * K + 2] = (uint64_t)&h_chain<T, &b_bin<T, K, 2, TBK(K)>>; t[BOP_BIN_BASE + 4 * K + 3] = (uint64_t)&h_chain<T, &b_bin<T, K, 3, TBK(K)>>;
#define HU(K) t[BOP_UN_BASE + 4 * K + 0] = (uint64_t)&h_chain<T, &b_un<T, K, 0, TB>>; t[BOP_UN_BASE + 4 * K + 1] = (uint64_t)&h_chain<T, &b_un<T, K, 1, TB>>; \
              t[BOP_UN_BASE + 4 * K + 2] = (uint64_t)&h_chain<T, &b_un<T, K, 2, TB>>; t[BOP_UN_BASE + 4 * K + 3] = (uint64_t)&h_chain<T, &b_un<T, K, 3, TB>>;
    t[BOP_LOAD_ROW] = (uint64_t)&h_chain<T, &b_load_row<T>>;
    t[BOP_LOAD_CONST] = (uint64_t)&h_chain<T, &b_load_const<T>>;
    t[BOP_PUSH] = (uint64_t)&h_chain<T, &b_push<T>>;
    t[BOP_CHECK_ROW] = (uint64_t)&h_chain<T, &b_check_row<T>>;
    t[BOP_CHECK_ACC] = (uint64_t)&h_chain<T, &b_check_acc<T>>;
    HB(0) HB(1) HB(2) HB(3) HB(4) HB(5)
    HU(0) HU(1) HU(2)
    t[BOP_GEN_ROW] = (uint64_t)&h_chain<T, &b_gen<T, 0, false>>;
    t[BOP_GEN_CONST] = (uint64_t)&h_chain<T, &b_gen<T, 1, false>>;
    t[BOP_GEN_ACC] = (uint64_t)&h_chain<T, &b_gen<T, 2, false>>;
    t[BOP_GEN_PARAM] = (uint64_t)&h_param<T, TB>;
    t[TOPX_END] = (uint64_t)&h_tree_end<T>;
    t[TOPX_AUX_BASE + 0] = (uint64_t)&h_tree_end_slow<T>;
    t[TOPX_AUX_BASE + 1] = (uint64_t)&h_tree_skip<T>;
#define HEB(K) t[TOPX_ENDV_BASE + K * 2] = (uint64_t)&h_chain_end<T, &b_bin<T, K, 1, TBK(K)>>; t[TOPX_ENDV_BASE + K * 2 + 1] = (uint64_t)&h_chain_end<T, &b_bin<T, K, 3, TBK(K)>>;
    HEB(0) HEB(1) HEB(2) HEB(3) HEB(4) HEB(5)
#undef HEB
    t[TOPX_ENDV_BASE + 12] = (uint64_t)&h_chain_end<T, &b_un<T, 0, 1, TB>>;
    t[TOPX_ENDV_BASE + 13] = (uint64_t)&h_chain_end<T, &b_un<T, 1, 1, TB>>;
    t[TOPX_ENDV_BASE + 14] = (uint64_t)&h_chain_end<T, &b_un<T, 2, 1, TB>>;
    t[BOP_TERN] = (uint64_t)&h_chain<T, &b_tern<T>>;
    t[BOP_INJ_ACC] = (uint64_t)&h_chain<T, &b_gen<T, 2, true>>;
    t[BOP_INJ_ROW] = (uint64_t)&h_chain<T, &b_gen<T, 0, true>>;
#define HX(K) t[TOPX_UN_BASE + (K - 3) * 2] = (uint64_t)&h_chain<T, &b_un2<T, K, 0>>; t[TOPX_UN_BASE + (K - 3) * 2 + 1] = (uint64_t)&h_chain<T, &b_un2<T, K, 1>>;
    HX(3) HX(4) HX(5) HX(6) HX(7) HX(8) HX(9) HX(10) HX(11) HX(12)
#undef HX
    t[TOPX_BIN_BASE + 0] = (uint64_t)&h_chain<T, &b_maxmin<T, 6, 0>>; t[TOPX_BIN_BASE + 1] = (uint64_t)&h_chain<T, &b_maxmin<T, 6, 1>>;
    t[TOPX_BIN_BASE + 2] = (uint64_t)&h_chain<T, &b_maxmin<T, 7, 0>>; t[TOPX_BIN_BASE + 3] = (uint64_t)&h_chain<T, &b_maxmin<T, 7, 1>>;
#undef HB
#undef HU
    t[top_loadrow(false, false)] = (uint64_t)&h_chain<T, &b_load_row<T>>;
    t[top_loadrow(false, true)] = (uint64_t)&h_chain<T, &b_loadrow_f<T, false, true>>;
    t[top_loadrow(true, false)] = (uint64_t)&h_chain<T, &b_loadrow_f<T, true, false>>;
    t[top_loadrow(true, true)] = (uint64_t)&h_chain<T, &b_loadrow_f<T, true, true>>;
    t[TOP_LOADCONST_PUSH] = (uint64_t)&h_chain<T, &b_loadconst_push<T>>;
#define TU1(K, O, P) t[top_unrow(K, O, P, false)] = (uint64_t)&h_chain<T, &b_unrow_f<T, K, O, P, false, TB>>; t[top_unrow(K, O, P, true)] = (uint64_t)&h_chain<T, &b_unrow_f<T, K, O, P, true, TB>>;
#define TU(K) TU1(K, false, false) TU1(K, false, true) TU1(K, true, false) TU1(K, true, true)
    TU(0) TU(1) TU(2)
#define TBC(K) t[top_binrowc(K, false)] = (uint64_t)&h_chain<T, &b_binrowc<T, K, false, TBK(K)>>; t[top_binrowc(K, true)] = (uint64_t)&h_chain<T, &b_binrowc<T, K, true, TBK(K)>>;
    TBC(0) TBC(1) TBC(2) TBC(3) TBC(4) TBC(5)
#define TB1(K, C, O) t[top_bin2(K, C, O, false)] = (uint64_t)&h_chain<T, &b_bin2<T, K, C, O, false, TBK(K)>>; t[top_bin2(K, C, O, true)] = (uint64_t)&h_chain<T, &b_bin2<T, K, C, O, true, TBK(K)>>;
#define TBF(K) TB1(K, false, false) TB1(K, false, true) TB1(K, true, false) TB1(K, true, true)
    TBF(0) TBF(1) TBF(2) TBF(3) TBF(4) TBF(5)
#undef TU1
#undef TU
#undef TBC
#undef TB1
#undef TBF
    if constexpr (sizeof(T) == 4) {
#define HUF(K) t[BOP_UN_BASE + 4 * K + 0] = (uint64_t)&h_un_fast<K, 0, TB>; t[BOP_UN_BASE + 4 * K + 1] = (uint64_t)&h_un_fast<K, 1, TB>; \
               t[BOP_UN_BASE + 4 * K + 2] = (uint64_t)&h_un_fast<K, 2, TB>; t[BOP_UN_BASE + 4 * K + 3] = (uint64_t)&h_un_fast<K, 3, TB>; \
               t[TOPX_ENDV_BASE + 12 + K] = (uint64_t)&h_un_end_fast<K, TB>;
#define HURF1(K, O, P) t[top_unrow(K, O, P, false)] = (uint64_t)&h_unrow_fast<K, O, P, false, TB>; t[top_unrow(K, O, P, true)] = (uint64_t)&h_unrow_fast<K, O, P, true, TB>;
#define HURF(K) HURF1(K, false, false) HURF1(K, false, true) HURF1(K, true, false) HURF1(K, true, true)
        HUF(0) HUF(2) HURF(0) HURF(2)
        if constexpr (!TB) {
            HUF(1) HURF(1)
#define HDF(K) t[BOP_BIN_BASE + 4 * K + 0] = (uint64_t)&h_div_fast<K, 0>; t[BOP_BIN_BASE + 4 * K + 1] = (uint64_t)&h_div_fast<K, 1>; \
               t[BOP_BIN_BASE + 4 * K + 2] = (uint64_t)&h_div_fast<K, 2>; t[BOP_BIN_BASE + 4 * K + 3] = (uint64_t)&h_div_fast<K, 3>; \
               t[TOPX_ENDV_BASE + K * 2] = (uint64_t)&h_div_end_fast<K, false>; t[TOPX_ENDV_BASE + K * 2 + 1] = (uint64_t)&h_div_end_fast<K, true>; \
               t[top_binrowc(K, false)] = (uint64_t)&h_divrowc_fast<K, false>; t[top_binrowc(K, true)] = (uint64_t)&h_divrowc_fast<K, true>;
#define HD2(K, C, O) t[top_bin2(K, C, O, false)] = (uint64_t)&h_div2_fast<K, C, O, false>; t[top_bin2(K, C, O, true)] = (uint64_t)&h_div2_fast<K, C, O, true>;
#define HD2K(K) HD2(K, false, false) HD2(K, false, true) HD2(K, true, false) HD2(K, true, true)
            HDF(4) HDF(5) HD2K(4) HD2K(5)
#undef HD2K
#undef HD2
#undef HDF
        }
#undef HURF
#undef HURF1
#undef HUF
    }
#undef TBK
}

__device__ __forceinline__ uint32_t orderable_f32(float v) {
    const uint32_t b = __float_as_uint(v);
    return (b & 0x80000000u) ? ~b : (b | 0x80000000u);
}
template <typename T, int FMAX>
__global__ void __launch_bounds__(256) de_tile_extremes_kernel(const T *__restrict__ X, int64_t N, int64_t ldX, int F, int tile_shift,
                                                               unsigned long long *__restrict__ keys, const uint8_t *__restrict__ ok_init,
                                                               uint8_t *__restrict__ ok, int32_t n_ok) {
    for (int32_t i = (int32_t)(blockIdx.x * 256 + threadIdx.x); i < n_ok; i += (int32_t)(gridDim.x * 256)) ok[i] = ok_init[i];
    const float inf = __builtin_inff();
    float v[3][FMAX];
    uint32_t at[3][FMAX];
    DE_UNROLL for (int f = 0; f < FMAX; f++) DE_UNROLL for (int k = 0; k < 3; k++) { v[k][f] = -inf; at[k][f] = 0u; }
    for (int64_t j = (int64_t)blockIdx.x * 256 + threadIdx.x; j < N; j += (int64_t)gridDim.x * 256) {
        const uint32_t tile = (uint32_t)(j >> tile_shift);
        DE_UNROLL for (int f = 0; f < FMAX; f++) {
            if (f < F) {
                const float x = (float)X[f + ldX * j];
                const bool fin = __builtin_fabsf(x) < inf;
                const float c[3] = {fin ? x : inf, fin ? -x : inf, fin ? -__builtin_fabsf(x) : inf};
                DE_UNROLL for (int k = 0; k < 3; k++)
                    if (c[k] > v[k][f]) { v[k][f] = c[k]; at[k][f] = tile; }
            }
        }
    }
    __shared__ unsigned long long best[4][3 * FMAX];
    DE_UNROLL for (int f = 0; f < FMAX; f++) {
        if (f < F) {
            DE_UNROLL for (int k = 0; k < 3; k++) {
                unsigned long long key = ((unsigned long long)orderable_f32(v[k][f]) << 32) | (unsigned long long)at[k][f];
                DE_UNROLL for (int m = 32; m >= 1; m >>= 1) {
                    const unsigned long long o = __shfl_xor(key, m, 64);
                    key = o > key ? o : key;
                }
                if ((threadIdx.x & 63) == 0) best[threadIdx.x >> 6][3 * f + k] = key;
            }
        }
    }
    __syncthreads();
    if ((int)threadIdx.x < 3 * F) {
        unsigned long long key = best[0][threadIdx.x];
        DE_UNROLL for (int w = 1; w < 4; w++) key = best[w][threadIdx.x] > key ? best[w][threadIdx.x] : key;
// ... 96 lines not shown
template <typename T, bool PARAMS, bool LOSS = false, int WW = 1>
__global__ void __launch_bounds__(DE_TBLK * WW) de_eval_threaded_kernel(const KArgs<T> a) {
    typedef typename VecOf<T>::type V;
    constexpr int VW = VecOf<T>::W;
    constexpr int BLK = DE_TBLK, G = TG<T>::G, PLANE = BLK * VW, TILE = PLANE * G, ROWV = BLK * G + 1;
    static_assert(WW == 1 || DE_TBLK == 64, "a wave group shares one 64-lane tile");
    constexpr int SBLK = BLK * WW;
    extern __shared__ __align__(16) unsigned char smem_base[];
    unsigned char *const smem_raw = smem_base + DE_SKIPLIST_BYTES;
    T *__restrict__ rows = reinterpret_cast<T *>(smem_raw);

    TileMap tm;
    int flag_protocol = a.skip_flagged;
    int32_t n_trees = a.n_trees, n_chunks = a.n_chunks, tpc = a.trees_per_chunk;
    if (a.ctrl) {
        const ConstI32Ptr ct = (ConstI32Ptr)(uintptr_t)a.ctrl;
        n_trees = ct[0];
        n_chunks = ct[1];
        tpc = ct[2];
        if (n_trees <= 0) return;
    }
    const int32_t host_groups = WW > 1 ? (a.n_chunks + WW - 1) / WW : a.n_chunks, groups = WW > 1 ? (n_chunks + WW - 1) / WW : n_chunks + a.tail_split - 1;
    if (blockIdx.x < a.n_prio_blocks) {
        const uint32_t k = blockIdx.x / (uint32_t)host_groups;
        if (k >= a.n_prio) return;
        tm.tile = (int64_t)((uint32_t)a.prio[k] >> a.prio_shift);
        tm.chunk = (int32_t)(blockIdx.x % (uint32_t)host_groups);
        tm.valid = tm.tile < a.n_tiles;
        flag_protocol = 1;
    } else tm = a.map_group > 0 ? map_block_grouped(blockIdx.x - a.n_prio_blocks, groups, a.n_tiles, (uint32_t)a.map_group)
                                : map_block(blockIdx.x - a.n_prio_blocks, groups, a.n_tiles);
    if (!tm.valid) return;
    const int stid = threadIdx.x;
    const int tid = WW > 1 ? (int)(threadIdx.x & 63u) : (int)threadIdx.x;
    const int wave = WW > 1 ? __builtin_amdgcn_readfirstlane((int)(threadIdx.x >> 6)) : 0;
    const int64_t base = tm.tile * TILE;
    const int64_t last = a.N - 1;
    if constexpr (WW > 1) tm.chunk = tm.chunk * WW + wave;
    int tA = tm.chunk * tpc;
    int tB = (tA + tpc < n_trees) ? tA + tpc : n_trees;
    if (WW > 1 && tm.chunk >= n_chunks) tA = tB = 0;
    if (WW == 1 && a.tail_split > 1 && tm.chunk >= n_chunks - 1) {
        const int b0 = (n_chunks - 1) * tpc, rem = n_trees - b0;
        const int sub = (rem + a.tail_split - 1) / a.tail_split;
        tA = b0 + (tm.chunk - (n_chunks - 1)) * sub;
        tB = tA + sub < n_trees ? tA + sub : n_trees;
        if (tA >= tB) return;
    }
    uint8_t f_first = 1;
    if (a.skip_flagged && (WW > 1 || tid < 64) && tA + tid < tB) f_first = skip_flag_load(a.ok + (a.live_idx ? a.live_idx[tA + tid] : tA + tid), flag_protocol, tm.tile);
    uint64_t *const mask_slot = reinterpret_cast<uint64_t *>(smem_raw + (size_t)BLK * G * 16);
    int32_t co_first = 0;
    if (a.skip_flagged && tA + (tid & 63) < tB) co_first = a.code_off[tA + (tid & 63)];
    {
        const uint32_t F = (uint32_t)a.F;
        const uint32_t total = (uint32_t)TILE * F;
        if (a.x_vec && base + TILE <= a.N) {
            const V *__restrict__ src = reinterpret_cast<const V *>(a.X + base * (int64_t)F);
            const uint32_t GF = (uint32_t)G * F;
            if constexpr (WW > 1) {
                const uint32_t nv = (uint32_t)BLK * GF;
                for (uint32_t i0 = 0; i0 * SBLK < nv; i0 += 8) {
                    V buf[8];
                    DE_UNROLL for (uint32_t u = 0; u < 8; u++)
                        if (stid + (i0 + u) * SBLK < nv) buf[u] = src[stid + (i0 + u) * SBLK];
                    DE_UNROLL for (uint32_t u = 0; u < 8; u++) {
                        if (stid + (i0 + u) * SBLK < nv) {
                            const uint32_t e = (stid + (i0 + u) * SBLK) * VW;
                            uint32_t j = a.f_magic ? __umulhi(e, a.f_magic) : e;
                            uint32_t f = e - j * F;
                            DE_UNROLL for (int c = 0; c < VW; c++) {
                                rows[f * (ROWV * VW) + j] = buf[u][c];
                                ++f;
                                if (f == F) { f = 0; ++j; }
                            }
                        }
                    }
                }
            } else
            for (uint32_t i0 = 0; i0 < GF; i0 += 8) {
                V buf[8];
                DE_UNROLL for (uint32_t u = 0; u < 8; u++)
                    if (i0 + u < GF) buf[u] = src[tid + (i0 + u) * BLK];
                DE_UNROLL for (uint32_t u = 0; u < 8; u++) {
                    if (i0 + u < GF) {
                        const uint32_t e = (tid + (i0 + u) * BLK) * VW;
                        uint32_t j = a.f_magic ? __umulhi(e, a.f_magic) : e;
                        uint32_t f = e - j * F;
                        DE_UNROLL for (int c = 0; c < VW; c++) {
                            rows[f * (ROWV * VW) + j] = buf[u][c];
                            ++f;
                            if (f == F) { f = 0; ++j; }
                        }
                    }
                }
            }
        } else if (a.ldX == (int64_t)F && base + TILE <= a.N) {
            const T *__restrict__ src = a.X + base * (int64_t)F;
            for (uint32_t e = stid; e < total; e += SBLK) {
                const uint32_t j = e / F, f = e - j * F;
                rows[f * (ROWV * VW) + j] = src[e];
            }
        } else {
            for (uint32_t e = stid; e < total; e += SBLK) {
                const uint32_t j = e / F, f = e - j * F;
                int64_t jj = base + j;
                jj = jj < last ? jj : last;
                rows[f * (ROWV * VW) + j] = a.X[f + a.ldX * jj];
            }
        }
    }
    if (PARAMS && a.n_prows > 0) {
        stage_param_rows<T>(a, rows, ROWV * VW, base, TILE, stid, SBLK);
    } else if (PARAMS && WW == 1) {
        DE_UNROLL for (int g = 0; g < G; g++) {
            uint32_t cv[4] = {0u, 0u, 0u, 0u};
            DE_UNROLL for (int i = 0; i < VW; i++) {
                int64_t jj = base + g * PLANE + tid * VW + i;
                jj = jj < last ? jj : last;
                cv[i] = (uint32_t)((uint64_t)a.ld_params * sizeof(T) *
                                   (uint64_t)clamp_class((a.classes_is_i64 ? reinterpret_cast<const int64_t *>(a.classes)[jj]
                                                                           : (int64_t) reinterpret_cast<const int32_t *>(a.classes)[jj]) - a.class_base,
                                                         a.n_classes));
            }
            const uint64_t tab = (uint64_t)(uintptr_t)a.params;
            unsigned char *crow = smem_raw + a.cls_row_off + g * DE_PLANE_BYTES + tid * 16;
            if constexpr (sizeof(T) == 4) {
                *reinterpret_cast<U32x4 *>(crow) = U32x4{cv[0], cv[1], cv[2], cv[3]};
                *reinterpret_cast<U32x4 *>(crow + RowOf<T>::BYTES) = U32x4{(uint32_t)tab, (uint32_t)(tab >> 32), 0u, 0u};
            } else {
                *reinterpret_cast<U32x4 *>(crow) = U32x4{cv[0], cv[1], (uint32_t)tab, (uint32_t)(tab >> 32)};
            }
        }
    }
    if constexpr (LOSS) {
        if (a.loss_kind >= DE_LOSS_HUBER && stid == 0) *reinterpret_cast<T *>(smem_base + LossParamLds<T>::ADDR) = a.loss_param;
    }
    uint64_t m_first = 0ull;
    if constexpr (WW > 1) {
        if (a.skip_flagged) m_first = __ballot(f_first == 0);
    } else if (a.skip_flagged && tid < 64) {
        const uint64_t m0 = __ballot(f_first == 0);
        if (tid == 0) *mask_slot = m0;
    }
    __syncthreads();

    const ConstU4Ptr code = (ConstU4Ptr)(uintptr_t)(a.code + (WW > 1 ? (int64_t)wave * a.var_stride : (int64_t)0));
    const uint32_t list_at = (WW > 1 && wave > 0) ? a.list_off + (uint32_t)(wave - 1) * DE_SKIPLIST_BYTES : 0u;
    const ConstI32Ptr code_off = (ConstI32Ptr)(uintptr_t)a.code_off;
    const bool full = base + TILE <= a.N;
    const uint32_t lds0 = (uint32_t)(uintptr_t)smem_raw + tid * 16;
    HLoss<T> yv, wv;
    DE_UNROLL for (int g = 0; g < 2; g++) { yv.v[g] = V{}; wv.v[g] = V{}; }
    if constexpr (LOSS) {
        DE_UNROLL for (int g = 0; g < G; g++) DE_UNROLL for (int i = 0; i < VW; i++) {
            const int64_t j = base + g * PLANE + tid * VW + i;
            const int64_t jj = j < last ? j : last;
            yv.v[g][i] = a.y[jj];
            wv.v[g][i] = j <= last ? (a.w ? a.w[jj] : T(1)) : T(0);
        }
        if (a.loss_kind == FIT_STATS_KIND) {
            const T ym = (T)a.fit_ystats[1];
            DE_UNROLL for (int g = 0; g < G; g++) DE_UNROLL for (int i = 0; i < VW; i++) yv.v[g][i] = yv.v[g][i] - ym;
        }
    }

    if (tA >= tB) return;
    const uint64_t ldo = (uint64_t)a.ld_out * sizeof(T);
    const int sub = 63;
    for (int t0 = tA; t0 < tB; t0 += sub) {
    const int t1 = t0 + sub < tB ? t0 + sub : tB;
    uint64_t skip = 0ull;
    if (a.skip_flagged) {
        if constexpr (WW > 1) {
            if (t0 != tA) break;
            skip = ((uint64_t)(uint32_t)__builtin_amdgcn_readfirstlane((int)(uint32_t)(m_first >> 32)) << 32) | (uint64_t)(uint32_t)__builtin_amdgcn_readfirstlane((int)(uint32_t)m_first);
            skip &= (1ull << (t1 - t0)) - 1ull;
        } else {
        if (t0 != tA) {
            __syncthreads();
            if (tid < 64) {
                const int i = t0 + tid;
                const uint8_t f = i >= t1 ? (uint8_t)1 : skip_flag_load(a.ok + (a.live_idx ? a.live_idx[i] : i), flag_protocol, tm.tile);
                const uint64_t m0 = __ballot(f == 0);
                if (tid == 0) *mask_slot = m0;
            }
            __syncthreads();
        }
        {
            const uint64_t m = *mask_slot;
            skip = ((uint64_t)(uint32_t)__builtin_amdgcn_readfirstlane((int)(uint32_t)(m >> 32)) << 32) | (uint64_t)(uint32_t)__builtin_amdgcn_readfirstlane((int)(uint32_t)m);
            skip &= (1ull << (t1 - t0)) - 1ull;
        }
        }
        {
            const int i = t0 + (tid & 63);
            if (i < t1 && !((skip >> (tid & 63)) & 1ull)) {
                const uint32_t r = (uint32_t)__builtin_popcountll((~skip & ((1ull << (t1 - t0)) - 1ull)) >> 1 >> (tid & 63));
                const uint64_t hdr = (uint64_t)(uintptr_t)(code + (t0 == tA ? co_first : a.code_off[i]) - 1);
                reinterpret_cast<uint32_t *>(smem_base + list_at)[r] = (uint32_t)hdr;
// ... 352 lines not shown
#define DE_TEV(FF) case FF: hipLaunchKernelGGL((de_tile_extremes_vec_kernel<FF>), gv, dim3(256), 0, stream, x, N, shift, k, ok_init, ok, n_ok); break;
            DE_TEV(1) DE_TEV(2) DE_TEV(3) DE_TEV(4) DE_TEV(5) DE_TEV(6) DE_TEV(7) DE_TEV(8)
#undef DE_TEV
            default: return hipErrorInvalidValue;
        }
        return hipGetLastError();
    }
    if (dtype == DE_F32)
        hipLaunchKernelGGL((de_tile_extremes_kernel<float, DE_PRIO_MAX_F>), grid, dim3(256), 0, stream, static_cast<const float *>(X), N, ldX, F, shift,
                           static_cast<unsigned long long *>(keys), ok_init, ok, n_ok);
    else
        hipLaunchKernelGGL((de_tile_extremes_kernel<double, DE_PRIO_MAX_F>), grid, dim3(256), 0, stream, static_cast<const double *>(X), N, ldX, F, shift,
                           static_cast<unsigned long long *>(keys), ok_init, ok, n_ok);
    return hipGetLastError();
}
bool prio_tiles_wanted(int64_t N, int F, int64_t n_trees) {
    return F >= 1 && F <= DE_PRIO_MAX_F && n_trees >= env_int("DE_PRIO_MIN_TREES", 96) && (N + 255) / 256 >= env_int("DE_PRIO_MIN_TILES", 512) &&
           !env_int("DE_NO_PRIO_TILES", 0);
}

template <typename T>
static hipError_t launch_threaded_t(const EvalArgs &e, hipStream_t stream, const char **kname) {
    constexpr int VW = VecOf<T>::W;
    constexpr int TILE = TBLK * VW * TG<T>::G;
    KArgs<T> a;
    a.code = e.code;
    a.code_off = e.code_off;
    a.X = static_cast<const T *>(e.X);
    a.out = static_cast<T *>(e.out);
    a.ok = e.ok;
    a.params = static_cast<const T *>(e.params);
    a.classes = e.classes;
    a.N = e.N;
    a.ldX = e.ldX;
    a.ld_out = e.ld_out;
    a.ld_params = e.ld_params;
    a.prow_base = e.prow_base;
    a.n_prows = e.n_prows;
    a.n_tiles = (e.N + TILE - 1) / TILE;
    a.F = e.F;
    a.n_trees = e.n_trees;
    a.n_slots = e.n_slots;
    a.xstride = 0;
    a.classes_is_i64 = e.classes_is_i64;
    a.class_base = e.class_base;
    a.n_classes = e.n_classes > 0 ? e.n_classes : 1;
    a.vec_store = (reinterpret_cast<uintptr_t>(e.out) % 16 == 0 && (e.ld_out * sizeof(T)) % 16 == 0 && (uint64_t)e.ld_out * sizeof(T) < (1ull << 32)) ? 1 : 0;
    a.x_vec = (e.F >= 1 && e.ldX == e.F && reinterpret_cast<uintptr_t>(e.X) % 16 == 0 && (int64_t)TILE * e.F < 0x10000000LL) ? 1 : 0;
    a.f_magic = e.F > 1 ? (uint32_t)((0x100000000ull + (uint64_t)e.F - 1) / (uint64_t)e.F) : 0u;
    if (!env_int("DE_X_VEC", 1)) { a.x_vec = 0; a.f_magic = 0; }
    if (env_int("DE_DEBUG_NO_STORE", 0)) a.vec_store = 2;
    const int WW = (TBLK == 64 && (e.waves == 2 || e.waves == 4 || e.waves == 8) && (!e.uses_params || e.n_prows > 0)) ? e.waves : 1;
    a.var_stride = WW > 1 ? e.var_stride : 0;
    int32_t tpc, nch, nc0;
    plan_chunks(e.n_trees, a.n_tiles, &nch, &tpc, &nc0, WW);
    a.trees_per_chunk = tpc;
    a.n_chunks = nch;
    a.live_idx = a.ctrl = nullptr;
    a.cert_max = nullptr;
    a.skip_flagged = (e.early_exit && e.skip_flagged && a.F + a.n_slots >= 1) ? 1 : 0;
    if (a.skip_flagged) { const int pr = env_int("DE_SKIP_PROTOCOL", (e.loss && tpc >= 8) ? 1 : 2); a.skip_flagged = pr >= 1 && pr <= 3 ? pr : 2; }
    const int64_t tiles8 = (a.n_tiles + 7) / 8;
    a.map_group = 0;
    if (a.n_tiles >= 64 && a.n_chunks > 1) {
        const int64_t g = env_int("DE_MAP_GROUP", (int64_t)a.F * 8 <= (int64_t)a.trees_per_chunk * WW ? (int)(tiles8 > 0x3fffffff ? 0x3fffffff : tiles8) : 0);
        a.map_group = (int32_t)(g <= 0 ? 0 : (g > tiles8 ? tiles8 : g));
    }
    const int64_t tiles8g = a.map_group > 0 ? (tiles8 + a.map_group - 1) / a.map_group * a.map_group : tiles8;
    a.tail_split = 1;
    const int64_t fills = (a.n_tiles * (int64_t)a.n_chunks) / ((int64_t)(cu_count() > 0 ? cu_count() : 256) * 21);
    if (TBLK == 64 && WW == 1 && a.map_group > 0 && a.n_chunks > 1 && fills <= env_int("DE_TAIL_SPLIT_FILLS", 24)) {
        const int ts = env_int("DE_TAIL_SPLIT", 4);
        const int most = tpc / 8;
        a.tail_split = ts < 1 ? 1 : (ts > most ? (most < 1 ? 1 : most) : ts);
    }
    auto groups_of = [&](int64_t chunks) { return WW > 1 ? (chunks + WW - 1) / WW : chunks + a.tail_split - 1; };
    int64_t blocks = tiles8g * 8 * groups_of(a.n_chunks);
    if (blocks <= 0 || blocks > 0x7fffffffLL) return hipErrorInvalidValue;
    a.prio = nullptr;
    a.n_prio_blocks = a.n_prio = 0;
    bool ok_set = !e.ok_init;
    if (TBLK == 64 && a.skip_flagged && e.prio_keys && a.F >= 1 && prio_tiles_wanted(a.N, a.F, a.n_trees)) {
        const int np = 3 * a.F;
        hipError_t ps = e.prio_keys_ready ? hipSuccess
                                          : launch_tile_extremes(sizeof(T) == 4 ? DE_F32 : DE_F64, a.X, a.N, a.ldX, a.F, e.prio_keys, stream, e.ok_init, e.ok, e.n_trees);
        if (ps != hipSuccess) return ps;
        ok_set = !e.prio_keys_ready;
        const int tile_samples = TILE;
        a.prio_shift = 0;
        while ((DE_PRIO_UNIT << a.prio_shift) < tile_samples) ++a.prio_shift;
        a.prio = static_cast<const unsigned long long *>(e.prio_keys);
        a.n_prio = (uint32_t)np;
        a.n_prio_blocks = (uint32_t)(((int64_t)np * (WW > 1 ? groups_of(a.n_chunks) : (int64_t)a.n_chunks) + 7) / 8 * 8);
        if (!env_int("DE_PRIO_PROBE", 1)) {
            a.tail_split = 1;
            blocks = tiles8g * 8 * groups_of(a.n_chunks);
        }
        blocks += a.n_prio_blocks;
        if (blocks > 0x7fffffffLL) return hipErrorInvalidValue;
    }
    if (!ok_set) {
        const hipError_t cs = hipMemcpyAsync(e.ok, e.ok_init, (size_t)e.n_trees, hipMemcpyDeviceToDevice, stream);
        if (cs != hipSuccess) return cs;
    }
    a.cls_row_off = (uint32_t)((size_t)(a.F + a.n_slots) * RowOf<T>::BYTES);
    const int prm_rows = (e.uses_params && e.n_prows == 0) ? (sizeof(T) == 4 ? 2 : 1) : 0;
// ... 21 lines not shown
            if (WW == 8) kern = e.uses_params ? de_eval_threaded_kernel<T, true, true, 8> : de_eval_threaded_kernel<T, false, true, 8>;
        }
        a.y = static_cast<const T *>(e.loss->y);
        a.w = static_cast<const T *>(e.loss->w);
        a.partial = static_cast<T *>(e.loss->partial);
        a.loss_kind = e.loss->kind;
        a.loss_param = (T)e.loss->param;
        if (a.loss_kind >= DE_LOSS_HUBER && ((uint32_t)a.loss_kind & ~(uint32_t)HF_LOSS_KIND_MASK)) return hipErrorInvalidValue;
    }
    const bool fit = e.loss && e.loss->kind == FIT_STATS_KIND;
    a.fit_ystats = nullptr;
    if (fit) {
        if (TWAVES != 1 || !e.loss->stats || !e.loss->ystats) return hipErrorInvalidValue;
        a.fit_ystats = e.loss->ystats;
        const hipError_t fs = launch_fit_prepass<T>(*e.loss, e.n_trees, a.N, a.n_tiles, TILE, stream);
        if (fs != hipSuccess) return fs;
    }
    if (kname) *kname = "de_eval_threaded_kernel";
    if (lds > 64 * 1024) {
        hipError_t st = hipFuncSetAttribute(reinterpret_cast<const void *>(kern), hipFuncAttributeMaxDynamicSharedMemorySize, (int)lds);
        if (st != hipSuccess) return st;
    }
    if (a.n_prio && env_int("DE_PRIO_PROBE", 1)) {
        KArgs<T> pa = a;
        pa.tail_split = 1;
        pa.trees_per_chunk = env_int("DE_PRIO_PROBE_TPC", 8);
        pa.trees_per_chunk = pa.trees_per_chunk < 1 ? 1 : (pa.trees_per_chunk > 64 ? 64 : pa.trees_per_chunk);
        pa.n_chunks = (a.n_trees + pa.trees_per_chunk - 1) / pa.trees_per_chunk;
        pa.n_prio_blocks = (uint32_t)(((int64_t)pa.n_prio * (WW > 1 ? ((int64_t)pa.n_chunks + WW - 1) / WW : (int64_t)pa.n_chunks) + 7) / 8 * 8);
        hipLaunchKernelGGL(kern, dim3(pa.n_prio_blocks), dim3(TBLK * WW), lds, stream, pa);
        const hipError_t ps = hipGetLastError();
        if (ps != hipSuccess) return ps;
        blocks -= a.n_prio_blocks;
        a.n_prio_blocks = a.n_prio = 0;
        a.prio = nullptr;
        if (e.compact_code && e.compact_ints && tpc <= 64 && env_int("DE_COMPACT", 1)) {
            int32_t *coff = e.compact_ints, *live_idx = coff + (size_t)e.n_trees + 1, *ctrl = live_idx + e.n_trees;
            const int64_t want_blocks = (int64_t)cu_count() * 4 * 8;
            const int32_t tpc_max = plan_tpc_max(WW);
            LossEnds le;
            std::memset(&le, 0, sizeof le);
            if (e.loss && env_int("DE_LOSS_PLAIN_ENDS", 1)) {
                uint64_t table[TOPX_TABLE];
                const hipError_t ts = eval_handler_table(sizeof(T) == 4 ? DE_F32 : DE_F64, e.turbo, table);
                if (ts != hipSuccess) return ts;
                le.end = table[TOPX_END];
                le.slow_end = table[TOPX_AUX_BASE + 0];
                for (uint32_t k = 0; k < TOPX_ENDV_COUNT; k++) {
                    le.endv[k] = table[TOPX_ENDV_BASE + k];
                    le.plain[k] = k < 12 ? table[BOP_BIN_BASE + 4 * (k / 2) + ((k & 1) ? 3 : 1)] : table[BOP_UN_BASE + 4 * (k - 12) + 1];
                }
            }
            if (sizeof(T) == 4)
                hipLaunchKernelGGL(de_compact_live_kernel<true>, dim3(a.var_stride ? WW : 1), dim3(1024), 0, stream, reinterpret_cast<const U32x4 *>(e.code), e.code_off, e.ok,
                                   e.n_trees, reinterpret_cast<U32x4 *>(e.compact_code), coff, live_idx, ctrl, a.n_tiles, want_blocks, tpc_max, le, a.var_stride);
            else
                hipLaunchKernelGGL(de_compact_live_kernel<false>, dim3(a.var_stride ? WW : 1), dim3(1024), 0, stream, reinterpret_cast<const U32x4 *>(e.code), e.code_off, e.ok,
                                   e.n_trees, reinterpret_cast<U32x4 *>(e.compact_code), coff, live_idx, ctrl, a.n_tiles, want_blocks, tpc_max, le, a.var_stride);
            const hipError_t cs = hipGetLastError();
            if (cs != hipSuccess) return cs;
            a.code = static_cast<const BoundInstr *>(e.compact_code);
            a.code_off = coff;
            a.live_idx = live_idx;
            a.ctrl = ctrl;
            if (e.compacted) *e.compacted = true;
            blocks = tiles8g * 8 * groups_of(nc0);
            if (blocks > 0x7fffffffLL) return hipErrorInvalidValue;
        }
    }
    hipLaunchKernelGGL(kern, dim3((unsigned)blocks), dim3(TBLK * WW), lds, stream, a);
    hipError_t st = hipGetLastError();
    if (st != hipSuccess || !e.loss) return st;
    if (fit) return launch_fit_reduce<T>(*e.loss, e.n_trees, a.n_tiles, e.ok, stream);
    int32_t n_segs = 1;
    st = launch_loss_reduce_tiles(sizeof(T) == 4 ? DE_F32 : DE_F64, a.partial, (int64_t)e.n_trees * TWAVES, a.n_tiles, e.loss->seg_sum, &n_segs, stream);
    if (st != hipSuccess) return st;
    hipLaunchKernelGGL(de_loss_finish_kernel<T>, dim3((unsigned)((e.n_trees + 255) / 256)), dim3(256), 0, stream,
                       static_cast<const double *>(e.loss->seg_sum), (int64_t)e.n_trees, n_segs, e.ok, static_cast<T *>(e.loss->loss));
    return hipGetLastError();
}

hipError_t launch_loss_reduce_tiles(int dtype, const void *partial, int64_t n_cols, int64_t n_tiles, void *seg_sum,
                                    int32_t *n_segs_out, hipStream_t stream) {
    const int32_t n_segs = loss_segments(n_tiles);
    const int64_t tps = (n_tiles + n_segs - 1) / n_segs;
    const dim3 grid((unsigned)((n_cols + 255) / 256), (unsigned)n_segs);
    if (dtype == DE_F32)
        hipLaunchKernelGGL(de_loss_reduce_tiles_kernel<float>, grid, dim3(256), 0, stream, static_cast<const float *>(partial), n_cols,
                           n_tiles, tps, static_cast<double *>(seg_sum));
    else
        hipLaunchKernelGGL(de_loss_reduce_tiles_kernel<double>, grid, dim3(256), 0, stream, static_cast<const double *>(partial), n_cols,
                           n_tiles, tps, static_cast<double *>(seg_sum));
    *n_segs_out = n_segs;
    return hipGetLastError();
}

int32_t loss_segments(int64_t n_tiles) { return (int32_t)(n_tiles < 64 ? (n_tiles < 1 ? 1 : n_tiles) : 64); }
void loss_scratch_bytes(int dtype, int64_t n_trees, int64_t N, size_t *partial_bytes, size_t *seg_bytes) {
    const int64_t tile = ttile_samples(dtype);
    const int64_t n_tiles = (N + tile - 1) / tile;
    *partial_bytes = (size_t)n_tiles * (size_t)n_trees * TWAVES * (dtype == DE_F32 ? 4 : 8);
    *seg_bytes = (size_t)loss_segments(n_tiles) * (size_t)n_trees * TWAVES * sizeof(double);
}

void fit_stats_scratch_bytes(int dtype, int64_t n_trees, int64_t N, size_t *partial_bytes, size_t *seg_bytes) {
    const int64_t tile = ttile_samples(dtype);
    const int64_t n_tiles = (N + tile - 1) / tile;
    *partial_bytes = (size_t)n_tiles * (size_t)n_trees * FIT_STATS_VALUES * (dtype == DE_F32 ? 4 : 8);
    *seg_bytes = (3 * (size_t)n_tiles + 3 * (size_t)loss_segments(n_tiles) * (size_t)n_trees) * sizeof(double);
}
// ... 97 lines not shown
```

include/de_hip.h:

```cpp
#ifndef DE_HIP_H
#define DE_HIP_H

#include <stddef.h>
#include <stdint.h>

#include "de_opcodes.h"

#ifdef __cplusplus
extern "C" {
#endif

#define DE_HIP_ABI_VERSION 3

typedef enum de_status {
    DE_OK = 0,
    DE_ERR_INVALID_ARG = 1,
    DE_ERR_BAD_TAPE = 2,
    DE_ERR_UNSUPPORTED_OP = 3,
    DE_ERR_HIP = 4,
    DE_ERR_NO_DEVICE = 5,
    DE_ERR_OUT_OF_RANGE = 6,
    DE_ERR_UNSUPPORTED = 7,
    DE_ERR_RCCL = 8
} de_status_t;
// ... 31 lines not shown
int de_opcode_table_version(void);
int de_opcode_by_name(const char *name, int degree);
const char *de_opcode_name(int opcode);
int de_opcode_degree(int opcode);
const char *de_status_string(int status);

#define DE_STREAM_NULL ((void *)(intptr_t)-1)
int de_ctx_create(int device, void *stream, de_ctx_t **out_ctx);
int de_ctx_destroy(de_ctx_t *ctx);
int de_ctx_set_stream(de_ctx_t *ctx, void *stream);
int de_ctx_synchronize(de_ctx_t *ctx);
int de_ctx_trim(de_ctx_t *ctx);
int de_ctx_declare_dataset(de_ctx_t *ctx, int dtype, const void *X, int64_t N, int64_t ldX, int32_t n_features);
void *de_ctx_stream(de_ctx_t *ctx);
int de_ctx_device(de_ctx_t *ctx);
const char *de_last_error(de_ctx_t *ctx);

int de_program_create(de_ctx_t *ctx, int dtype, const de_tape_node_t *nodes,
                      const int64_t *node_offsets, int64_t n_trees, const void *consts,
                      const int64_t *const_offsets, int32_t n_features, int32_t n_params,
                      uint32_t options, de_program_t **out_program);
int de_program_create_cse(de_ctx_t *ctx, int dtype, const de_tape_node_t *nodes, const int64_t *node_offsets,
                          const de_tape_node_t *cse_nodes, const int64_t *cse_offsets, int64_t n_trees,
                          const void *consts, const int64_t *const_offsets, int32_t n_features,
                          int32_t n_params, uint32_t options, de_program_t **out_program);
int de_program_set_consts(de_program_t *prog, const void *consts);
int de_program_set_consts_device(de_program_t *prog, const void *d_consts);
int de_program_get_consts(de_program_t *prog, void *out);
int de_program_consts_device_path(const de_program_t *prog);
int de_program_update(de_program_t *prog, const int64_t *tree_ids, int64_t n_update,
                      const de_tape_node_t *nodes, const int64_t *node_offsets,
                      const de_tape_node_t *cse_nodes, const int64_t *cse_offsets,
                      const void *consts, const int64_t *const_offsets);
int de_program_destroy(de_program_t *prog);
int64_t de_program_n_trees(const de_program_t *prog);
int64_t de_program_n_nodes(const de_program_t *prog);
int64_t de_program_n_grad(const de_program_t *prog, int64_t tree, int mode);
int64_t de_program_dump(const de_program_t *prog, int64_t tree, uint32_t *words, int64_t cap,
                        int which);

int de_program_verify(const de_program_t *prog);

uint64_t de_program_stream_hash(const de_program_t *prog);

int64_t de_host_pool_selftest(int64_t n, int32_t *n_ranges);

int64_t de_lower_tape(int dtype, const de_tape_node_t *nodes, int64_t n_nodes, const void *consts,
                      int64_t n_consts, int32_t n_features, int32_t n_params, uint32_t options,
                      uint32_t *words, int64_t cap, int32_t *meta);
int64_t de_lower_tape_stage(int dtype, const de_tape_node_t *nodes, int64_t n_nodes,
                            const void *consts, int64_t n_consts, int32_t n_features,
                            int32_t n_params, uint32_t options, int stage, uint32_t *words,
                            int64_t cap);
int64_t de_lower_tape_complex(int dtype, const de_tape_node_t *nodes, int64_t n_nodes, const void *consts,
                              int64_t n_consts, int32_t n_features, int32_t n_params, uint32_t options,
                              uint32_t *words, int64_t cap, int32_t *meta);
int64_t de_lower_tape_stage_complex(int dtype, const de_tape_node_t *nodes, int64_t n_nodes,
                                    const void *consts, int64_t n_consts, int32_t n_features,
                                    int32_t n_params, uint32_t options, int stage, uint32_t *words,
                                    int64_t cap);
int64_t de_lower_tape_grad(int dtype, const de_tape_node_t *nodes, int64_t n_nodes, const void *consts, int64_t n_consts,
                           int32_t n_features, int32_t n_params, uint32_t options, int mode, int form, uint32_t *words,
                           int64_t cap, int32_t *meta);

typedef struct de_param_args {
    const void *params;
    int64_t ld_params;
    int64_t n_classes;
    const void *classes;
    int32_t classes_is_i64;
    int32_t class_base;
} de_param_args_t;

int de_eval(de_ctx_t *ctx, de_program_t *prog, const void *X, int64_t N, int64_t ldX,
            const de_param_args_t *pargs, void *out, int64_t ld_out, uint8_t *ok);

int de_eval_sum_certificate(de_ctx_t *ctx, de_program_t *prog, const void *X, int64_t N, int64_t ldX,
                            const de_param_args_t *pargs, uint8_t *ok, uint8_t *certified, double *max_abs);

int de_eval_grad(de_ctx_t *ctx, de_program_t *prog, const void *X, int64_t N, int64_t ldX,
                 const de_param_args_t *pargs, int mode, void *out, int64_t ld_out, void *grad,
                 const int64_t *grad_offsets, uint8_t *ok);

int de_eval_diff(de_ctx_t *ctx, de_program_t *prog, const void *X, int64_t N, int64_t ldX,
                 int32_t direction, void *out, void *dout, int64_t ld_out, uint8_t *ok);

typedef enum de_loss_kind {
    DE_LOSS_L2 = 0,
    DE_LOSS_L1 = 1,
    DE_LOSS_PULLBACK = 2,
    DE_LOSS_HUBER = 16,
    DE_LOSS_LOGCOSH = 17,
    DE_LOSS_L1_EPS = 18,
    DE_LOSS_L2_EPS = 19,
    DE_LOSS_QUANTILE = 20,
    DE_LOSS_LP = 21,
    DE_LOSS_LOGIT_DIST = 22,
    DE_LOSS_LOGIT_MARGIN = 23,
    DE_LOSS_L1_HINGE = 24
} de_loss_kind_t;
typedef struct de_loss_spec {
    int32_t kind;
    int32_t reserved;
    double param;
} de_loss_spec_t;
int de_loss_spec_check(const de_loss_spec_t *spec, int with_gradient);
// ... 69 lines not shown
```

Before: 14270 billion.

## Add range-assured handler stream that drops per-sample safety checks on bounded inputs

Runs a host-side interval analysis per tree, assuming every input magnitude is at most xmax, and builds a second threaded code stream whose handlers skip the runtime domain and division safety ballots wherever the analysis proves them unnecessary. At load time the kernel checks that every X value in the tile is within xmax and selects the assured stream only for tiles that pass. The cost targeted is the per-instruction safety checks and ballots on the hot path. In exchange it adds a per-element check during load, a second stream variant to upload and compact, and relinking work when constants change.

```diff
diff --git a/dynamicexpressions.jl_amd/api.py b/dynamicexpressions.jl_amd/api.py
--- a/dynamicexpressions.jl_amd/api.py
+++ b/dynamicexpressions.jl_amd/api.py
@@ -30,6 +30,7 @@
     "de_dist_broadcast", "de_dist_gather_flags", "de_dist_last_error", "de_ctx_last_kernel_ms", "de_ctx_last_kernel_name",
     "de_ctx_device", "de_ctx_timing_ring", "de_ctx_timing_read", "de_dist_reorder_selftest", "de_eval_sum_certificate",
     "de_dist_set_timeout", "de_ctx_trim", "de_program_set_consts_device", "de_program_get_consts", "de_program_consts_device_path",
+    "de_lower_tape_assured",
 ]
 
 
@@ -250,6 +251,9 @@
         fn.restype = i64
     lib.de_lower_tape_complex.argtypes = lib.de_lower_tape.argtypes
     lib.de_lower_tape_stage_complex.argtypes = lib.de_lower_tape_stage.argtypes
+    if hasattr(lib, "de_lower_tape_assured"):
+        lib.de_lower_tape_assured.restype = i64
+        lib.de_lower_tape_assured.argtypes = [vp, i64, vp, i64, i32, u32, C.c_double, vp, i64]
     lib.de_lower_tape_grad.restype = i64
     lib.de_lower_tape_grad.argtypes = [C.c_int, vp, i64, vp, i64, i32, i32, u32, C.c_int, C.c_int, vp, i64, vp]
     lib.de_eval.argtypes = [vp, vp, vp, i64, i64, C.POINTER(ParamArgs), vp, i64, vp]
@@ -504,6 +508,20 @@
     w = np.zeros(max(int(n), 1), dtype=np.uint32)
     stage_fn(*args, w.ctypes.data, w.size)
     return w[:int(n)].reshape(-1, 4)
+
+
+def lower_tape_assured(tape, consts, n_features: int, xmax: float = 64.0, options: int = 7) -> np.ndarray:
+    lib = library()
+    tape = np.ascontiguousarray(tape)
+    consts = np.ascontiguousarray(consts, dtype=np.float32)
+    cp = consts.ctypes.data if consts.size else None
+    args = (tape.ctypes.data, len(tape), cp, consts.size, n_features, options, float(xmax))
+    n = lib.de_lower_tape_assured(*args, None, 0)
+    if n < 0:
+        raise ValueError(lib.de_status_string(int(-n)).decode())
+    w = np.zeros(max(int(n), 1), dtype=np.float64)
+    lib.de_lower_tape_assured(*args, w.ctypes.data, w.size)
+    return w[:int(n)].reshape(-1, 6)
 
 
 def lower_tape_grad(tape, consts, n_features: int, mode: int, form: int, n_params: int = 0, options: int = 7, dtype=np.float32):
@@ -741,9 +759,17 @@
         return w[:int(got)].reshape(-1, 4)
 
     def meta(self, tree: int) -> dict:
-        w = np.zeros(5, dtype=np.uint32)
-        library().de_program_dump(self._h, tree, w.ctypes.data, 5, 1)
-        return dict(n_slots=int(w[0]), host_ok_eval=bool(w[1]), host_ok_grad=bool(w[2]), uses_params=bool(w[3]), waves=int(w[4]))
+        w = np.zeros(7, dtype=np.uint32)
+        library().de_program_dump(self._h, tree, w.ctypes.data, 7, 1)
+        return dict(n_slots=int(w[0]), host_ok_eval=bool(w[1]), host_ok_grad=bool(w[2]), uses_params=bool(w[3]), waves=int(w[4]),
+                    assured=bool(w[5]), assured_valid=bool(w[6]))
+
+    def dump_stage(self, tree: int, which: int) -> np.ndarray:
+        lib = library()
+        n = lib.de_program_dump(self._h, tree, None, 0, which)
+        w = np.zeros(max(int(n), 1), dtype=np.uint32)
+        got = lib.de_program_dump(self._h, tree, w.ctypes.data, w.size, which)
+        return w[:int(got)].reshape(-1, 4)
 
     def _param_args(self, params, classes, class_base, N, keep):
         if self.n_params == 0 and params is None:
diff --git a/dynamicexpressions.jl_amd/csrc/de_api_eval.cpp b/dynamicexpressions.jl_amd/csrc/de_api_eval.cpp
--- a/dynamicexpressions.jl_amd/csrc/de_api_eval.cpp
+++ b/dynamicexpressions.jl_amd/csrc/de_api_eval.cpp
@@ -312,6 +312,8 @@
     a.waves = p->waves;
     a.wave_slots = p->n_slots;
     a.var_stride = p->var_stride;
+    a.assured = p->assured && p->assured_valid && p->var_stride != 0;
+    a.assured_xmax = (float)p->assured_xmax;
     if (cr) {
         a.code = p->d_cert_code;
         a.code_off = p->d_cert_off;
diff --git a/dynamicexpressions.jl_amd/csrc/de_api_internal.h b/dynamicexpressions.jl_amd/csrc/de_api_internal.h
--- a/dynamicexpressions.jl_amd/csrc/de_api_internal.h
+++ b/dynamicexpressions.jl_amd/csrc/de_api_internal.h
@@ -122,6 +122,11 @@
     int waves_choice = 0;
     int64_t var_stride = 0;
     std::vector<BoundInstr> ccode_w;
+    bool assured = false, assured_valid = false;
+    int assured_cfg = 0;
+    double assured_xmax = 64.0;
+    uint32_t assured_parts = 0;
+    std::vector<uint32_t> aids;
     uint64_t end_handler = 0;
     uint64_t endv_handler[TOPX_ENDV_COUNT] = {0};
     bool threaded = false;
diff --git a/dynamicexpressions.jl_amd/csrc/de_api_program.cpp b/dynamicexpressions.jl_amd/csrc/de_api_program.cpp
--- a/dynamicexpressions.jl_amd/csrc/de_api_program.cpp
+++ b/dynamicexpressions.jl_amd/csrc/de_api_program.cpp
@@ -146,11 +146,36 @@
     }
     return best;
 }
+static void make_assured(de_program *p, const uint64_t *table);
+static double assured_xmax_env() {
+    const char *ax = getenv("DE_ASSURED_XMAX");
+    const double xm = ax ? (double)(float)atof(ax) : 64.0;
+    return (xm >= 0x1p-40 && xm <= 0x1p100) ? xm : 64.0;
+}
+static uint32_t assured_parts_env() {
+    const char *ap = getenv("DE_ASSURED_PARTS");
+    const int v = ap && *ap ? atoi(ap) : (int)ASSURED_PARTS_SHIPPED;
+    return (uint32_t)v & ASSURED_PARTS_ALL;
+}
 static int make_threaded(de_ctx *c, de_program *p, const Reuse *ru = nullptr) {
     p->threaded = false;
     p->waves = 1;
     p->var_stride = 0;
     p->ccode_w.clear();
+    p->assured = p->assured_valid = false;
+    p->aids.clear();
+    if (p->assured_cfg == 0) {
+        if (ru && ru->old && ru->old->assured_cfg != 0) {
+            p->assured_cfg = ru->old->assured_cfg;
+            p->assured_xmax = ru->old->assured_xmax;
+            p->assured_parts = ru->old->assured_parts;
+        } else {
+            const char *as = getenv("DE_ASSURED");
+            p->assured_parts = assured_parts_env();
+            p->assured_cfg = ((as && *as == '0') || p->assured_parts == 0) ? -1 : 1;
+            p->assured_xmax = assured_xmax_env();
+        }
+    }
     dbg_lap(nullptr);
     p->direct = (size_t)eval_rows(p) * FLAT_ROW_BYTES > 150 * 1024;
     if (p->io == DE_F16) return DE_OK;
@@ -289,6 +314,11 @@
         } else p->ccode_w.clear();
         dbg_lap("wave-group stream variants");
     } else if (W > 1 && fuse) p->waves = W;
+    if (p->assured_cfg > 0 && p->waves == 1 && p->var_stride == 0 && p->io == DE_F32 && p->dtype == DE_F32 && !p->uses_params &&
+        !(p->options & DE_OPT_TURBO) && p->n_trees >= 8 && p->allow_fold) {
+        make_assured(p, table);
+        dbg_lap("assured stream");
+    }
     return DE_OK;
 }
 
@@ -349,6 +379,42 @@
         if (p->dtype == DE_F32) r.arg = lo;
         else { r.lo = lo; r.hi = hi; }
     }
+}
+static void assured_link_trees(de_program *p, const uint64_t *table, int64_t tb, int64_t te, bool touched_only = false) {
+    BoundInstr *cw = p->ccode_w.data();
+    std::vector<AssuredInstr> info;
+    auto name_next = [](BoundInstr &r, uint64_t handler) { r.lo = (uint32_t)handler; r.hi = (uint32_t)(handler >> 32); };
+    auto ev_of = [&](int64_t t) -> int {
+        const int32_t i0 = p->tcode_off[(size_t)t], i1 = p->tcode_off[(size_t)t + 1];
+        return i1 - i0 >= 2 ? topx_endv_of(p->fbcode[(size_t)i1 - 1].bop) : -1;
+    };
+    for (int64_t t = tb; t < te; t++) {
+        const int32_t i0 = p->tcode_off[(size_t)t], i1 = p->tcode_off[(size_t)t + 1];
+        if (i1 <= i0) continue;
+        if (touched_only && p->const_off[(size_t)t + 1] == p->const_off[(size_t)t]) continue;
+        info.resize((size_t)(i1 - i0));
+        assure_tree(p->fbcode.data() + i0, (size_t)(i1 - i0), p->n_features, p->assured_xmax, info.data(), p->assured_parts);
+        const size_t h = (size_t)p->ccode_off[(size_t)t];
+        const int ev = ev_of(t);
+        for (int32_t i = i0; i < i1; i++) {
+            const uint32_t id = info[(size_t)(i - i0)].id;
+            p->aids[(size_t)i] = id;
+            if (i == i1 - 1 && ev >= 0) continue;
+            const uint64_t handler = id == p->fbcode[(size_t)i].bop ? p->handler_base + p->tcode[(size_t)i].bop : table[id];
+            if (i > i0) name_next(cw[h + (size_t)(i - i0) - 1], handler);
+            else {
+                name_next(cw[h - 1], handler);
+                if (t > 0 && ev_of(t - 1) >= 0) name_next(cw[h - 2], handler);
+            }
+        }
+    }
+}
+static void make_assured(de_program *p, const uint64_t *table) {
+    p->ccode_w = p->ccode;
+    p->aids.assign(p->fbcode.size(), 0u);
+    parallel_tree_ranges(p->n_trees, [&](int, int64_t tb, int64_t te) { assured_link_trees(p, table, tb, te); });
+    p->var_stride = (int64_t)(p->bcode.size() + (size_t)p->n_trees + 2);
+    p->assured = p->assured_valid = true;
 }
 static hipError_t upload_wave_variants(de_program *p) {
     for (size_t w = 0; p->var_stride && w * p->ccode.size() < p->ccode_w.size(); w++) {
@@ -1017,7 +1083,7 @@
     }
     const size_t cbytes = (p->bcode.size() + (size_t)p->n_trees + 2) * sizeof(BoundInstr);
     {
-        const size_t nvar = p->threaded && p->var_stride ? (size_t)p->waves : 1;
+        const size_t nvar = p->threaded && p->var_stride ? (p->assured ? 2 : (size_t)p->waves) : 1;
         if (nvar > 1 && (size_t)p->var_stride * sizeof(BoundInstr) != cbytes) return fail(ctx, DE_ERR_HIP, "wave-group stream variants: stride and arena disagree");
         const size_t abytes = p->threaded ? 2 * nvar * cbytes : cbytes;
         auto al = [](size_t x) { return (x + 255) & ~(size_t)255; };
@@ -1185,6 +1251,13 @@
             if (!rpatch) p->rt_valid = false;
         } else {
             p->gcode_stale = true;
+        }
+        if (p->assured) {
+            uint64_t table[TOPX_TABLE];
+            const hipError_t hs = eval_handler_table(p->dtype, (p->options & DE_OPT_TURBO) != 0, table);
+            if (hs != hipSuccess) return fail(ctx, DE_ERR_HIP, "handler table: %s", hipGetErrorString(hs));
+            parallel_tree_ranges(p->n_trees, [&](int, int64_t tb, int64_t te) { assured_link_trees(p, table, tb, te, true); });
+            p->assured_valid = true;
         }
         const auto t4 = now();
         HIP_TRY(ctx, hipStreamSynchronize(ctx->stream));
@@ -1443,6 +1516,7 @@
             p->tab_ok_stale = false;
             p->consts_dev_ahead = true;
             p->consts_dev_path = true;
+            p->assured_valid = false;
             return DE_OK;
         }
     }
@@ -1745,12 +1819,40 @@
                 }
             }
         }
+        if (p->assured) {
+            if (p->waves != 1 || !f32 || p->ccode_w.size() != p->ccode.size() || p->aids.size() != p->fbcode.size() || (size_t)p->var_stride < p->ccode.size())
+                return bad("assured stream layout", -1, p->waves, p->ccode_w.size());
+            const BoundInstr *cw = p->ccode_w.data();
+            std::vector<AssuredInstr> info;
+            auto named = [](const BoundInstr &q) { return ((uint64_t)q.hi << 32) | q.lo; };
+            for (size_t r = 0; r < p->ccode.size(); r++)
+                if (cw[r].bop != p->ccode[r].bop || cw[r].arg != p->ccode[r].arg) return bad("assured stream: operand words differ", -1, (int64_t)r, cw[r].bop);
+            for (int64_t t = 0; t < p->n_trees; t++) {
+                const int32_t i0 = p->tcode_off[(size_t)t], i1 = p->tcode_off[(size_t)t + 1], h = p->ccode_off[(size_t)t];
+                if (i1 <= i0) continue;
+                info.resize((size_t)(i1 - i0));
+                assure_tree(p->fbcode.data() + i0, (size_t)(i1 - i0), p->n_features, p->assured_xmax, info.data(), p->assured_parts);
+                const int ev = i1 - i0 >= 2 ? topx_endv_of(p->fbcode[(size_t)i1 - 1].bop) : -1;
+                for (int32_t i = i0; i < i1; i++) {
+                    const uint32_t id = info[(size_t)(i - i0)].id;
+                    if (p->assured_valid && id != p->aids[(size_t)i]) return bad("assured stream: stale twin id", t, i - i0, p->aids[(size_t)i]);
+                    const uint32_t have = p->aids[(size_t)i];
+                    if (have >= TOPX_COUNT) return bad("assured stream: handler id", t, i - i0, have);
+                    const uint64_t want = (i == i1 - 1 && ev >= 0) ? p->endv_handler[ev]
+                                          : (have == p->fbcode[(size_t)i].bop ? p->handler_base + p->tcode[(size_t)i].bop : table[have]);
+                    if (named(cw[(size_t)(h + (i - i0) - 1)]) != want) return bad("assured stream: handler word", t, i - i0, named(cw[(size_t)(h + (i - i0) - 1)]));
+                }
+                if (ev < 0 && named(cw[(size_t)(h + (i1 - i0) - 1)]) != p->end_handler) return bad("assured stream: tree does not end in the end record", t, i1 - i0, 0);
+                if (ev >= 0 && named(cw[(size_t)(h + (i1 - i0) - 1)]) != named(cw[(size_t)(h + (i1 - i0))])) return bad("assured stream: end-fused instruction and end record disagree", t, i1 - i0, 0);
+            }
+        }
     }
     return DE_OK;
 }
 
 int64_t de_program_dump(const de_program_t *p, int64_t tree, uint32_t *words, int64_t cap, int which) {
     if (!p || tree < 0 || tree >= p->n_trees) return -DE_ERR_INVALID_ARG;
+    const bool assured_valid = p->assured && p->assured_valid;
     if (const int mrc = consts_materialise(const_cast<de_program_t *>(p))) return -mrc;
     if (which == 1) {
         if (cap < 4) return -DE_ERR_INVALID_ARG;
@@ -1760,7 +1862,19 @@
         words[3] = p->uses_params;
         if (cap < 5) return 4;
         words[4] = (uint32_t)(p->threaded ? p->waves : 1);
-        return 5;
+        if (cap < 7) return 5;
+        words[5] = p->threaded && p->assured ? 1u : 0u;
+        words[6] = p->threaded && assured_valid ? 1u : 0u;
+        return 7;
+    }
+    if (which == 4) {
+        if (!p->threaded || !p->assured) return 0;
+        const int32_t b0 = p->tcode_off[(size_t)tree], b1 = p->tcode_off[(size_t)tree + 1];
+        const int64_t nb = (int64_t)(b1 - b0) * 4;
+        if (!words || cap < nb) return nb;
+        std::memcpy(words, p->fbcode.data() + b0, (size_t)nb * 4);
+        for (int32_t i = b0; i < b1; i++) words[(size_t)(i - b0) * 4] = p->aids[(size_t)i];
+        return nb;
     }
     if (which == 2) {
         const int32_t b0 = p->bcode_off[(size_t)tree], b1 = p->bcode_off[(size_t)tree + 1];
@@ -1863,9 +1977,34 @@
     }
 }
 
+int64_t de_lower_tape_assured(const de_tape_node_t *nodes, int64_t n_nodes, const void *consts, int64_t n_consts, int32_t n_features,
+                              uint32_t options, double xmax, double *out, int64_t cap) {
+    if (!(xmax >= 0x1p-40 && xmax <= 0x1p100)) return -DE_ERR_INVALID_ARG;
+    int64_t nw = lower_tape_stage_impl(DE_F32, nodes, n_nodes, consts, n_consts, n_features, 0, options, 3, nullptr, 0);
+    if (nw < 0) return nw;
+    try {
+        std::vector<BoundInstr> f((size_t)nw / 4);
+        nw = lower_tape_stage_impl(DE_F32, nodes, n_nodes, consts, n_consts, n_features, 0, options, 3, reinterpret_cast<uint32_t *>(f.data()), nw);
+        if (nw < 0) return nw;
+        const int64_t n = (int64_t)f.size() * 6;
+        if (!out || cap < n) return n;
+        std::vector<AssuredInstr> info(f.size());
+        assure_tree(f.data(), f.size(), n_features, xmax, info.data());
+        for (size_t i = 0; i < f.size(); i++) {
+            double *o = out + 6 * i;
+            o[0] = info[i].acc.lo; o[1] = info[i].acc.hi; o[2] = info[i].acc.amin; o[3] = info[i].acc.fin ? 1.0 : 0.0;
+            o[4] = (double)info[i].id; o[5] = (double)info[i].bits;
+        }
+        return n;
+    } catch (...) {
+        return -DE_ERR_HIP;
+    }
+}
+
 static int64_t lower_tape_stage_impl(int dtype, const de_tape_node_t *nodes, int64_t n_nodes, const void *consts, int64_t n_consts,
                                      int32_t n_features, int32_t n_params, uint32_t options, int stage, uint32_t *words, int64_t cap) {
-    if (stage != 2 && stage != 3) return -DE_ERR_INVALID_ARG;
+    if (stage != 2 && stage != 3 && stage != 4) return -DE_ERR_INVALID_ARG;
+    if (stage == 4 && dtype != DE_F32) return -DE_ERR_INVALID_ARG;
     std::vector<uint32_t> g;
     int64_t nw = lower_tape_impl(dtype, nodes, n_nodes, consts, n_consts, n_features, n_params, options, nullptr, 0, nullptr);
     if (nw < 0) return nw;
@@ -1875,8 +2014,13 @@
         if (nw < 0) return nw;
         std::vector<BoundInstr> b, f;
         bind_tree(reinterpret_cast<const Instr *>(g.data()), (size_t)nw / 4, (options & DE_OPT_EARLY_EXIT) != 0, n_features, &b);
-        if (stage == 3 && dtype != DE_F16 && !is_complex_io(dtype)) fuse_tree(b.data(), b.size(), &f);
-        const std::vector<BoundInstr> &o = stage == 3 ? f : b;
+        if (stage >= 3 && dtype != DE_F16 && !is_complex_io(dtype)) fuse_tree(b.data(), b.size(), &f);
+        if (stage == 4) {
+            std::vector<AssuredInstr> info(f.size());
+            assure_tree(f.data(), f.size(), n_features, assured_xmax_env(), info.data(), assured_parts_env());
+            for (size_t i = 0; i < f.size(); i++) f[i].bop = info[i].id;
+        }
+        const std::vector<BoundInstr> &o = stage >= 3 ? f : b;
         const int64_t n = (int64_t)o.size() * 4;
         if (!words || cap < n) return n;
         std::memcpy(words, o.data(), (size_t)n * 4);
diff --git a/dynamicexpressions.jl_amd/csrc/de_bind.cpp b/dynamicexpressions.jl_amd/csrc/de_bind.cpp
--- a/dynamicexpressions.jl_amd/csrc/de_bind.cpp
+++ b/dynamicexpressions.jl_amd/csrc/de_bind.cpp
@@ -1,4 +1,9 @@
 #include "de_bind.h"
+
+#include <algorithm>
+#include <cmath>
+#include <cstring>
+#include <limits>
 
 #include "../../include/de_opcodes.h"
 
@@ -220,4 +225,165 @@
     }
 }
 
-}
+namespace {
+const double A_INF = std::numeric_limits<double>::infinity();
+AssuredVal a_unbounded() { return AssuredVal{-A_INF, A_INF, 0.0, false}; }
+AssuredVal a_make(double lo, double hi, double amin) {
+    const double W = 0x1p-20, T = 0x1p-140, BIG = 0x1p120;
+    lo -= std::fabs(lo) * W + T;
+    hi += std::fabs(hi) * W + T;
+    if (!(lo >= -BIG && hi <= BIG && lo <= hi)) return a_unbounded();
+    amin = amin * (1.0 - W) - T;
+    if (!(amin > 0.0)) amin = 0.0;
+    if (lo > 0.0) amin = std::max(amin, lo);
+    if (hi < 0.0) amin = std::max(amin, -hi);
+    return AssuredVal{lo, hi, amin, true};
+}
+AssuredVal a_const(uint32_t bits) {
+    float c;
+    std::memcpy(&c, &bits, 4);
+    if (!std::isfinite(c)) return a_unbounded();
+    return AssuredVal{(double)c, (double)c, std::fabs((double)c), true};
+}
+double a_absmax(const AssuredVal &a) { return std::max(std::fabs(a.lo), std::fabs(a.hi)); }
+AssuredVal a_div(const AssuredVal &n, const AssuredVal &d) {
+    if (!n.fin || !d.fin || !(d.amin > 0.0)) return a_unbounded();
+    const double amin = n.amin / a_absmax(d);
+    if (d.lo > 0.0 || d.hi < 0.0) {
+        const double dl = std::max(d.amin, std::min(std::fabs(d.lo), std::fabs(d.hi))), dh = a_absmax(d), s = d.lo > 0.0 ? 1.0 : -1.0;
+        const double q[4] = {s * n.lo / dl, s * n.lo / dh, s * n.hi / dl, s * n.hi / dh};
+        return a_make(std::min(std::min(q[0], q[1]), std::min(q[2], q[3])), std::max(std::max(q[0], q[1]), std::max(q[2], q[3])), amin);
+    }
+    const double m = a_absmax(n) / d.amin;
+    return a_make(-m, m, amin);
+}
+AssuredVal a_bin(int k, const AssuredVal &x, const AssuredVal &b) {
+    if (!x.fin || !b.fin) return a_unbounded();
+    switch (k) {
+    case 0: return a_make(x.lo + b.lo, x.hi + b.hi, 0.0);
+    case 1: return a_make(x.lo - b.hi, x.hi - b.lo, 0.0);
+    case 2: return a_make(b.lo - x.hi, b.hi - x.lo, 0.0);
+    case 3: {
+        const double q[4] = {x.lo * b.lo, x.lo * b.hi, x.hi * b.lo, x.hi * b.hi};
+        return a_make(std::min(std::min(q[0], q[1]), std::min(q[2], q[3])), std::max(std::max(q[0], q[1]), std::max(q[2], q[3])), x.amin * b.amin);
+    }
+    case 4: return a_div(x, b);
+    case 5: return a_div(b, x);
+    default: return a_unbounded();
+    }
+}
+AssuredVal a_un(int k, const AssuredVal &x) {
+    if (!x.fin) return a_unbounded();
+    if (k == 0) return a_make(-1.0, 1.0, 0.0);
+    if (k == 1) return a_make(std::exp(x.lo), std::exp(x.hi), 0.0);
+    return a_unbounded();
+}
+}
+
+void assure_tree(const BoundInstr *f, size_t n, int n_features, double xmax, AssuredInstr *out, uint32_t parts) {
+    static thread_local std::vector<AssuredVal> slots;
+    slots.clear();
+    const AssuredVal feature{-xmax, xmax, 0x1p-40, true};
+    auto row_val = [&](uint32_t row) -> AssuredVal {
+        if (row < (uint32_t)n_features) return feature;
+        const size_t s = row - (uint32_t)n_features;
+        return s < slots.size() ? slots[s] : a_unbounded();
+    };
+    auto push = [&](uint32_t row, const AssuredVal &v) {
+        if (row < (uint32_t)n_features) return;
+        const size_t s = row - (uint32_t)n_features;
+        if (s >= slots.size()) slots.resize(s + 1, a_unbounded());
+        slots[s] = v;
+    };
+    AssuredVal acc = a_unbounded();
+    for (size_t i = 0; i < n; i++) {
+        const BoundInstr &b = f[i];
+        const uint32_t id = b.bop, row = b.arg & 0xFFFFFFu;
+        const uint32_t prow = (uint32_t)((int32_t)row + (int32_t)(int8_t)(b.arg >> 24));
+        uint32_t twin = id, bits = 0;
+        AssuredVal un_arg = a_unbounded(), div_acc = a_unbounded(), div_row = a_unbounded();
+        const bool validity = (parts & ASSURED_PART_VALIDITY) != 0;
+        if (id == BOP_LOAD_ROW) acc = row_val(row);
+        else if (id == BOP_LOAD_CONST) acc = a_const(b.lo);
+        else if (id == BOP_PUSH) push(row, acc);
+        else if (id == BOP_CHECK_ROW || id == BOP_CHECK_ACC) ;
+        else if (id >= BOP_BIN_BASE && id < BOP_BIN_END) {
+            const uint32_t v = id - BOP_BIN_BASE;
+            div_acc = acc;
+            div_row = (v & 2) ? a_const(b.lo) : row_val(row);
+            acc = a_bin((int)(v >> 2), acc, div_row);
+            if (validity && (v & 1) && acc.fin) { twin = id - 1; bits |= ASSURED_OUT; }
+        } else if (id >= BOP_UN_BASE && id < BOP_UN_END) {
+            const uint32_t v = id - BOP_UN_BASE;
+            un_arg = (v & 2) ? row_val(row) : acc;
+            acc = a_un((int)(v >> 2), un_arg);
+            if (validity && (v & 1) && acc.fin) { twin = id - 1; bits |= ASSURED_OUT; }
+        } else if (id >= TOP_LOADROW_BASE && id < TOP_LOADCONST_PUSH) {
+            const uint32_t v = id - TOP_LOADROW_BASE;
+            if (v & 2) push(prow, acc);
+            acc = row_val(row);
+            if (validity && (v & 1) && acc.fin) { twin = top_loadrow((v & 2) != 0, false); bits |= ASSURED_ROW; }
+        } else if (id == TOP_LOADCONST_PUSH) {
+            push(b.arg & 0xFFFFFFu, acc);
+            acc = a_const(b.lo);
+        } else if (id >= TOP_UNROW_BASE && id < TOP_BINROWC_BASE) {
+            const uint32_t v = id - TOP_UNROW_BASE;
+            bool chk = (v & 1) != 0, outc = ((v >> 2) & 1) != 0;
+            const bool psh = ((v >> 1) & 1) != 0;
+            if (psh) push(prow, acc);
+            const AssuredVal x = row_val(row);
+            un_arg = x;
+            acc = a_un((int)(v >> 3), x);
+            if (validity && chk && x.fin) { chk = false; bits |= ASSURED_ROW; }
+            if (validity && outc && acc.fin) { outc = false; bits |= ASSURED_OUT; }
+            twin = top_unrow((int)(v >> 3), outc, psh, chk);
+        } else if (id >= TOP_BINROWC_BASE && id < TOP_BIN2_BASE) {
+            const uint32_t v = id - TOP_BINROWC_BASE;
+            const int k = (int)(v >> 1);
+            bool outc = (v & 1) != 0;
+            const AssuredVal x = row_val(row);
+            div_acc = acc;
+            div_row = x;
+            acc = a_bin(k, acc, x);
+            if (validity && outc && acc.fin) { outc = false; bits |= ASSURED_OUT; }
+            if (validity && x.fin) { twin = BOP_BIN_BASE + 4 * (uint32_t)k + (outc ? 1u : 0u); bits |= ASSURED_ROW; }
+            else twin = top_binrowc(k, outc);
+        } else if (id >= TOP_BIN2_BASE && id < TOP_COUNT) {
+            const uint32_t v = id - TOP_BIN2_BASE;
+            const bool psh = (v & 1) != 0, cst = ((v >> 2) & 1) != 0;
+            bool outc = ((v >> 1) & 1) != 0;
+            if (psh) push(prow, acc);
+            const AssuredVal x = row_val(row);
+            acc = a_bin((int)(v >> 3), x, cst ? a_const(b.lo) : row_val((uint32_t)((int32_t)row + (int32_t)b.lo)));
+            if (validity && outc && acc.fin) { outc = false; bits |= ASSURED_OUT; }
+            twin = top_bin2((int)(v >> 3), cst, outc, psh);
+        } else if (id == BOP_GEN_CONST && ((b.arg >> 24) == (uint32_t)DE_U_COS || (b.arg >> 24) == (uint32_t)DE_U_EXP)) {
+            acc = a_un((b.arg >> 24) == (uint32_t)DE_U_COS ? 0 : 1, a_const(b.lo));
+        } else acc = a_unbounded();
+        auto pre_idle = [](int k, const AssuredVal &x) { return x.fin && a_absmax(x) <= (k == 0 ? 9.0e4 : 125.0 / 1.4426950408889634); };
+        auto half_idle = [](const AssuredVal &x) { return x.fin && x.amin >= 0x1p-39 && a_absmax(x) <= 0x1p39; };
+        if ((parts & ASSURED_PART_PRETEST) && twin >= BOP_UN_BASE && twin < BOP_UN_BASE + 8 && pre_idle((int)((twin - BOP_UN_BASE) >> 2), un_arg)) {
+            twin = topa_un((int)((twin - BOP_UN_BASE) >> 2), (twin - BOP_UN_BASE) & 3u);
+            bits |= ASSURED_PRE;
+        } else if ((parts & ASSURED_PART_PRETEST) && twin >= TOP_UNROW_BASE && twin < TOP_UNROW_BASE + 16 && pre_idle((int)((twin - TOP_UNROW_BASE) >> 3), un_arg)) {
+            twin = TOPA_UNROW_BASE + (twin - TOP_UNROW_BASE);
+            bits |= ASSURED_PRE;
+        } else if ((parts & ASSURED_PART_DIVISION) && twin >= BOP_BIN_BASE + 16 && twin < BOP_BIN_END) {
+            const uint32_t v = twin - BOP_BIN_BASE, var = v & 3u;
+            const bool ia = half_idle(div_acc), ir = (var & 2) ? false : half_idle(div_row);
+            if (ia || ir) {
+                twin = topa_div((int)(v >> 2), var, (var & 2) ? 0u : ((ia ? 0u : 1u) | (ir ? 0u : 2u)));
+                bits |= (ia ? ASSURED_DIV_ACC : 0u) | (ir ? ASSURED_DIV_ROW : 0u);
+            }
+        }
+        out[i].acc = acc;
+        out[i].id = twin;
+        out[i].bits = bits;
+    }
+    if (n >= 2 && topx_endv_of(f[n - 1].bop) >= 0) {
+        out[n - 1].id = f[n - 1].bop;
+        out[n - 1].bits = 0;
+    }
+}
+
+}
diff --git a/dynamicexpressions.jl_amd/csrc/de_bind.h b/dynamicexpressions.jl_amd/csrc/de_bind.h
--- a/dynamicexpressions.jl_amd/csrc/de_bind.h
+++ b/dynamicexpressions.jl_amd/csrc/de_bind.h
@@ -124,7 +124,12 @@
 
 constexpr uint32_t TOPX_UN_BASE = TOP_COUNT;
 constexpr uint32_t TOPX_BIN_BASE = TOPX_UN_BASE + 2 * (GUN_K - 3);
-constexpr uint32_t TOPX_COUNT = TOPX_BIN_BASE + 4;
+constexpr uint32_t TOPA_UN_BASE = TOPX_BIN_BASE + 4;
+constexpr uint32_t TOPA_UNROW_BASE = TOPA_UN_BASE + 8;
+constexpr uint32_t TOPA_DIV_BASE = TOPA_UNROW_BASE + 16;
+constexpr uint32_t TOPX_COUNT = TOPA_DIV_BASE + 24;
+constexpr uint32_t topa_un(int k, uint32_t var) { return TOPA_UN_BASE + (uint32_t)k * 4 + var; }
+constexpr uint32_t topa_div(int k, uint32_t var, uint32_t m) { return TOPA_DIV_BASE + ((uint32_t)(k - 4) * 4 + var) * 3 + m; }
 constexpr uint32_t TOPX_END = TOPX_COUNT;
 constexpr uint32_t TOPX_ENDV_BASE = TOPX_END + 1;
 constexpr uint32_t TOPX_ENDV_COUNT = 15;
@@ -167,6 +172,25 @@
 void fuse_tree(const BoundInstr *b, size_t n, std::vector<BoundInstr> *out, const FuseRows *rows = nullptr);
 bool top_is_const_source(uint32_t top);
 
+struct AssuredVal {
+    double lo, hi;
+    double amin;
+    bool fin;
+};
+enum : uint32_t { ASSURED_OUT = 1u,
+                  ASSURED_ROW = 2u,
+                  ASSURED_PRE = 4u,
+                  ASSURED_DIV_ACC = 8u,
+                  ASSURED_DIV_ROW = 16u };
+constexpr uint32_t ASSURED_PARTS_SHIPPED = 3u;
+enum : uint32_t { ASSURED_PART_VALIDITY = 1u, ASSURED_PART_PRETEST = 2u, ASSURED_PART_DIVISION = 4u, ASSURED_PARTS_ALL = 7u };
+struct AssuredInstr {
+    AssuredVal acc;
+    uint32_t id;
+    uint32_t bits;
+};
+void assure_tree(const BoundInstr *f, size_t n, int n_features, double xmax, AssuredInstr *out, uint32_t parts = ASSURED_PARTS_ALL);
+
 void bind_tree(const Instr *code, size_t n, bool early_exit, int n_features, std::vector<BoundInstr> *out, int param_row_base = -1, int slot_shift = 0);
 
 }
diff --git a/dynamicexpressions.jl_amd/csrc/de_kernels.h b/dynamicexpressions.jl_amd/csrc/de_kernels.h
--- a/dynamicexpressions.jl_amd/csrc/de_kernels.h
+++ b/dynamicexpressions.jl_amd/csrc/de_kernels.h
@@ -69,6 +69,8 @@
     bool *compacted;
     int32_t waves, wave_slots;
     int64_t var_stride;
+    bool assured = false;
+    float assured_xmax = 0.0f;
     void *cert_max;
 };
 constexpr int DE_PRIO_MAX_F = 8;
diff --git a/dynamicexpressions.jl_amd/csrc/de_kernels.hip b/dynamicexpressions.jl_amd/csrc/de_kernels.hip
--- a/dynamicexpressions.jl_amd/csrc/de_kernels.hip
+++ b/dynamicexpressions.jl_amd/csrc/de_kernels.hip
@@ -49,7 +49,11 @@
     uint32_t list_off;
     T loss_param;
     const double *fit_ystats;
+    int32_t assured;
+    float assured_xmax;
 };
+__device__ __forceinline__ bool assured_value_ok(float v, float xmax) { return (__builtin_fabsf(v) <= xmax) & (__builtin_fabsf(v) >= 0x1p-40f); }
+__device__ __forceinline__ bool assured_value_ok(double, float) { return false; }
 
 
 __device__ __forceinline__ TileMap map_block_grouped(uint32_t bid, int32_t n_chunks, int64_t n_tiles, uint32_t grp) {
@@ -681,7 +685,7 @@
         HTREE_END_TAIL(wn, code_at(code, 2), code);                                                                                     \
     }
 #define PLANE_ADDR(A, g) ((A) + (uint32_t)(g) * DE_PLANE_BYTES)
-template <int K, int VAR, bool TB> __device__ __noinline__ HState<float> h_un_fast(HFAST_ARGS) {
+template <int K, int VAR, bool TB, bool NT = false> __device__ __noinline__ HState<float> h_un_fast(HFAST_ARGS) {
     typedef float T;
     constexpr int G = TG<T>::G;
     const U32x4 w = *code;
@@ -690,7 +694,7 @@
     UnPre p[G];
     bool slow = false;
     FOR_PLANES slow |= un_pretest<K, TB>(x[g], p[g]);
-    if (__builtin_expect(__ballot(slow) != 0ull, 0)) [[clang::musttail]] return h_chain<T, &b_un<T, K, VAR, TB>>(HFAST_PASS);
+    if constexpr (!NT) if (__builtin_expect(__ballot(slow) != 0ull, 0)) [[clang::musttail]] return h_chain<T, &b_un<T, K, VAR, TB>>(HFAST_PASS);
 #if DE_TG == 1
     FOR_PLANES {
         st.acc[g] = un_finish<K, TB>(x[g], p[g]);
@@ -721,7 +725,7 @@
 #endif
     HFAST_END_TAIL()
 }
-template <int K, bool OUT, bool PUSH, bool CHK, bool TB> __device__ __noinline__ HState<float> h_unrow_fast(HFAST_ARGS) {
+template <int K, bool OUT, bool PUSH, bool CHK, bool TB, bool NT = false> __device__ __noinline__ HState<float> h_unrow_fast(HFAST_ARGS) {
     typedef float T;
     constexpr int G = TG<T>::G;
     const U32x4 w = *code;
@@ -734,7 +738,7 @@
     UnPre p[G];
     bool slow = false;
     FOR_PLANES slow |= un_pretest<K, TB>(x[g], p[g]);
-    if (__builtin_expect(__ballot(slow) != 0ull, 0)) [[clang::musttail]] return h_chain<T, &b_unrow_f<T, K, OUT, PUSH, CHK, TB>>(HFAST_PASS);
+    if constexpr (!NT) if (__builtin_expect(__ballot(slow) != 0ull, 0)) [[clang::musttail]] return h_chain<T, &b_unrow_f<T, K, OUT, PUSH, CHK, TB>>(HFAST_PASS);
 #if DE_TG == 1
     FOR_PLANES {
         if constexpr (CHK) hpoison<T>(st.poison, x[g]);
@@ -748,16 +752,18 @@
 #endif
     HFAST_NEXT(w);
 }
-template <int K, int VAR> __device__ __noinline__ HState<float> h_div_fast(HFAST_ARGS) {
+template <int K, int VAR, int M = 3> __device__ __noinline__ HState<float> h_div_fast(HFAST_ARGS) {
     typedef float T;
     typedef VecOf<float>::type V;
     constexpr int G = TG<T>::G;
     const U32x4 w = *code;
     if constexpr (VAR & 2) {
-        bool unsafe = false;
-        FOR_PLANES unsafe |= !div_samples_safe(st.acc[g]);
         if (__builtin_expect(!div_const_in_range(w1), 0)) [[clang::musttail]] return h_chain<T, &b_bin<T, K, VAR, false>>(HFAST_PASS);
-        if (__builtin_expect(wave_any(unsafe), 0)) [[clang::musttail]] return h_chain<T, &b_bin<T, K, VAR, false>>(HFAST_PASS);
+        if constexpr (M & 1) {
+            bool unsafe = false;
+            FOR_PLANES unsafe |= !div_samples_safe(st.acc[g]);
+            if (__builtin_expect(wave_any(unsafe), 0)) [[clang::musttail]] return h_chain<T, &b_bin<T, K, VAR, false>>(HFAST_PASS);
+        }
         FOR_PLANES st.acc[g] = div_const<K>(st.acc[g], w1);
     } else {
         V num[G], den[G];
@@ -766,9 +772,11 @@
             const V b = *LDSP(T, PLANE_ADDR(lds0 + la, g));
             num[g] = K == 4 ? st.acc[g] : b;
             den[g] = K == 4 ? b : st.acc[g];
-            unsafe |= !div_operands_safe(num[g], den[g]);
-        }
-        if (__builtin_expect(__ballot(unsafe) != 0ull, 0)) [[clang::musttail]] return h_chain<T, &b_bin<T, K, VAR, false>>(HFAST_PASS);
+            if constexpr (M == 3) unsafe |= !div_operands_safe(num[g], den[g]);
+            else if constexpr (M == 1) unsafe |= !div_samples_safe(st.acc[g]);
+            else if constexpr (M == 2) unsafe |= !div_samples_safe(b);
+        }
+        if constexpr (M != 0) if (__builtin_expect(__ballot(unsafe) != 0ull, 0)) [[clang::musttail]] return h_chain<T, &b_bin<T, K, VAR, false>>(HFAST_PASS);
         FOR_PLANES st.acc[g] = div_safe(num[g], den[g]);
     }
     if constexpr (VAR & 1) FOR_PLANES hpoison<T>(st.poison, st.acc[g]);
@@ -997,6 +1005,9 @@
 #undef TBC
 #undef TB1
 #undef TBF
+    for (uint32_t k = 0; k < 2; k++) for (uint32_t v = 0; v < 4; v++) t[topa_un((int)k, v)] = t[BOP_UN_BASE + 4 * k + v];
+    for (uint32_t i = 0; i < 16; i++) t[TOPA_UNROW_BASE + i] = t[TOP_UNROW_BASE + i];
+    for (uint32_t k = 4; k < 6; k++) for (uint32_t v = 0; v < 4; v++) for (uint32_t m = 0; m < 3; m++) t[topa_div((int)k, v, m)] = t[BOP_BIN_BASE + 4 * k + v];
     if constexpr (sizeof(T) == 4) {
 #define HUF(K) t[BOP_UN_BASE + 4 * K + 0] = (uint64_t)&h_un_fast<K, 0, TB>; t[BOP_UN_BASE + 4 * K + 1] = (uint64_t)&h_un_fast<K, 1, TB>; \
                t[BOP_UN_BASE + 4 * K + 2] = (uint64_t)&h_un_fast<K, 2, TB>; t[BOP_UN_BASE + 4 * K + 3] = (uint64_t)&h_un_fast<K, 3, TB>; \
@@ -1013,6 +1024,22 @@
 #define HD2(K, C, O) t[top_bin2(K, C, O, false)] = (uint64_t)&h_div2_fast<K, C, O, false>; t[top_bin2(K, C, O, true)] = (uint64_t)&h_div2_fast<K, C, O, true>;
 #define HD2K(K) HD2(K, false, false) HD2(K, false, true) HD2(K, true, false) HD2(K, true, true)
             HDF(4) HDF(5) HD2K(4) HD2K(5)
+#define HAU(K) t[topa_un(K, 0)] = (uint64_t)&h_un_fast<K, 0, false, true>; t[topa_un(K, 1)] = (uint64_t)&h_un_fast<K, 1, false, true>; \
+               t[topa_un(K, 2)] = (uint64_t)&h_un_fast<K, 2, false, true>; t[topa_un(K, 3)] = (uint64_t)&h_un_fast<K, 3, false, true>;
+#define HAUR1(K, O, P) t[TOPA_UNROW_BASE + top_unrow(K, O, P, false) - TOP_UNROW_BASE] = (uint64_t)&h_unrow_fast<K, O, P, false, false, true>; \
+                       t[TOPA_UNROW_BASE + top_unrow(K, O, P, true) - TOP_UNROW_BASE] = (uint64_t)&h_unrow_fast<K, O, P, true, false, true>;
+#define HAUR(K) HAUR1(K, false, false) HAUR1(K, false, true) HAUR1(K, true, false) HAUR1(K, true, true)
+            HAU(0) HAU(1) HAUR(0) HAUR(1)
+#define HAD1(K, V) t[topa_div(K, V, 0)] = (uint64_t)&h_div_fast<K, V, 0>; t[topa_div(K, V, 1)] = (uint64_t)&h_div_fast<K, V, 1>; t[topa_div(K, V, 2)] = (uint64_t)&h_div_fast<K, V, 2>;
+#define HAD2(K, V) t[topa_div(K, V, 0)] = (uint64_t)&h_div_fast<K, V, 0>;
+#define HAD(K) HAD1(K, 0) HAD1(K, 1) HAD2(K, 2) HAD2(K, 3)
+            HAD(4) HAD(5)
+#undef HAD
+#undef HAD2
+#undef HAD1
+#undef HAUR
+#undef HAUR1
+#undef HAU
 #undef HD2K
 #undef HD2
 #undef HDF
@@ -1215,6 +1242,8 @@
     uint64_t *const mask_slot = reinterpret_cast<uint64_t *>(smem_raw + (size_t)BLK * G * 16);
     int32_t co_first = 0;
     if (a.skip_flagged && tA + (tid & 63) < tB) co_first = a.code_off[tA + (tid & 63)];
+    constexpr bool ASSURABLE = WW == 1 && !PARAMS && sizeof(T) == 4 && DE_TBLK == 64;
+    bool x_ok = true;
     {
         const uint32_t F = (uint32_t)a.F;
         const uint32_t total = (uint32_t)TILE * F;
@@ -1251,6 +1280,7 @@
                         uint32_t j = a.f_magic ? __umulhi(e, a.f_magic) : e;
                         uint32_t f = e - j * F;
                         DE_UNROLL for (int c = 0; c < VW; c++) {
+                            if constexpr (ASSURABLE) x_ok &= assured_value_ok(buf[u][c], a.assured_xmax);
                             rows[f * (ROWV * VW) + j] = buf[u][c];
                             ++f;
                             if (f == F) { f = 0; ++j; }
@@ -1262,14 +1292,18 @@
             const T *__restrict__ src = a.X + base * (int64_t)F;
             for (uint32_t e = stid; e < total; e += SBLK) {
                 const uint32_t j = e / F, f = e - j * F;
-                rows[f * (ROWV * VW) + j] = src[e];
+                const T v = src[e];
+                if constexpr (ASSURABLE) x_ok &= assured_value_ok(v, a.assured_xmax);
+                rows[f * (ROWV * VW) + j] = v;
             }
         } else {
             for (uint32_t e = stid; e < total; e += SBLK) {
                 const uint32_t j = e / F, f = e - j * F;
                 int64_t jj = base + j;
                 jj = jj < last ? jj : last;
-                rows[f * (ROWV * VW) + j] = a.X[f + a.ldX * jj];
+                const T v = a.X[f + a.ldX * jj];
+                if constexpr (ASSURABLE) x_ok &= assured_value_ok(v, a.assured_xmax);
+                rows[f * (ROWV * VW) + j] = v;
             }
         }
     }
@@ -1308,7 +1342,8 @@
     }
     __syncthreads();
 
-    const ConstU4Ptr code = (ConstU4Ptr)(uintptr_t)(a.code + (WW > 1 ? (int64_t)wave * a.var_stride : (int64_t)0));
+    const bool assured_tile = ASSURABLE && a.assured != 0 && __ballot(!x_ok) == 0ull;
+    const ConstU4Ptr code = (ConstU4Ptr)(uintptr_t)(a.code + (WW > 1 ? (int64_t)wave * a.var_stride : (assured_tile ? a.var_stride : (int64_t)0)));
     const uint32_t list_at = (WW > 1 && wave > 0) ? a.list_off + (uint32_t)(wave - 1) * DE_SKIPLIST_BYTES : 0u;
     const ConstI32Ptr code_off = (ConstI32Ptr)(uintptr_t)a.code_off;
     const bool full = base + TILE <= a.N;
@@ -1767,6 +1802,10 @@
     if (env_int("DE_DEBUG_NO_STORE", 0)) a.vec_store = 2;
     const int WW = (TBLK == 64 && (e.waves == 2 || e.waves == 4 || e.waves == 8) && (!e.uses_params || e.n_prows > 0)) ? e.waves : 1;
     a.var_stride = WW > 1 ? e.var_stride : 0;
+    a.assured = (WW == 1 && TBLK == 64 && sizeof(T) == 4 && e.assured && e.var_stride != 0 && !e.uses_params) ? 1 : 0;
+    a.assured_xmax = e.assured_xmax;
+    if (a.assured) a.var_stride = e.var_stride;
+    const unsigned n_variants = a.var_stride ? (a.assured ? 2u : (unsigned)WW) : 1u;
     int32_t tpc, nch, nc0;
     plan_chunks(e.n_trees, a.n_tiles, &nch, &tpc, &nc0, WW);
     a.trees_per_chunk = tpc;
@@ -1894,10 +1933,10 @@
                 }
             }
             if (sizeof(T) == 4)
-                hipLaunchKernelGGL(de_compact_live_kernel<true>, dim3(a.var_stride ? WW : 1), dim3(1024), 0, stream, reinterpret_cast<const U32x4 *>(e.code), e.code_off, e.ok,
+                hipLaunchKernelGGL(de_compact_live_kernel<true>, dim3(n_variants), dim3(1024), 0, stream, reinterpret_cast<const U32x4 *>(e.code), e.code_off, e.ok,
                                    e.n_trees, reinterpret_cast<U32x4 *>(e.compact_code), coff, live_idx, ctrl, a.n_tiles, want_blocks, tpc_max, le, a.var_stride);
             else
-                hipLaunchKernelGGL(de_compact_live_kernel<false>, dim3(a.var_stride ? WW : 1), dim3(1024), 0, stream, reinterpret_cast<const U32x4 *>(e.code), e.code_off, e.ok,
+                hipLaunchKernelGGL(de_compact_live_kernel<false>, dim3(n_variants), dim3(1024), 0, stream, reinterpret_cast<const U32x4 *>(e.code), e.code_off, e.ok,
                                    e.n_trees, reinterpret_cast<U32x4 *>(e.compact_code), coff, live_idx, ctrl, a.n_tiles, want_blocks, tpc_max, le, a.var_stride);
             const hipError_t cs = hipGetLastError();
             if (cs != hipSuccess) return cs;
diff --git a/include/de_hip.h b/include/de_hip.h
--- a/include/de_hip.h
+++ b/include/de_hip.h
@@ -107,6 +107,8 @@
                             const void *consts, int64_t n_consts, int32_t n_features,
                             int32_t n_params, uint32_t options, int stage, uint32_t *words,
                             int64_t cap);
+int64_t de_lower_tape_assured(const de_tape_node_t *nodes, int64_t n_nodes, const void *consts, int64_t n_consts,
+                              int32_t n_features, uint32_t options, double xmax, double *out, int64_t cap);
 int64_t de_lower_tape_complex(int dtype, const de_tape_node_t *nodes, int64_t n_nodes, const void *consts,
                               int64_t n_consts, int32_t n_features, int32_t n_params, uint32_t options,
                               uint32_t *words, int64_t cap, int32_t *meta);
```

After: 14870 billion (median of 6 runs). +4.2%, better.
